# als244/ResNet

Hardware: AMD Instinct MI355X
Metric: images/sec ResNet-50 fp32 224x224 batch256 (higher is better)
Workload: dtype f32

## Files before the change

include/resnet_mi.h:

```cpp
#ifndef RESNET_MI_H
#define RESNET_MI_H
#include <stddef.h>
#include <stdint.h>

#ifdef __cplusplus
extern "C" {
#endif

typedef struct {
    char **labels;
    char **synsets;
    int *counts;
    int n_classes;
} Class_Metadata;

typedef struct {
    int input;
    int init_kernel_dim;
    int init_conv_filters;
    int init_conv_stride;
    int init_maxpool_dim;
    int init_maxpool_stride;
    int n_conv_blocks;
    int *is_block_spatial_reduction;
// ... 88 lines not shown
    float *pred_cpu;
} Forward_Buffer;

typedef struct {
    float *output_layer_deriv;
    Params *param_derivs;
    Params *prev_means;
    Params *prev_vars;
    Activations *activation_derivs;
} Backprop_Buffer;

typedef struct {
    int image_dim;
    int image_size;
    int n_images;
    int cur_shard_id;
    int cur_batch_in_shard;
    int shard_n_images;
    float *full_shard_images;
    int *full_shard_correct_classes;
    float *images_float_cpu;
    float *images;
    int *correct_classes_cpu;
    int *correct_classes;
} Batch;

typedef struct {
    ResNet *model;
    Batch *cur_batch;
    Forward_Buffer *forward_buffer;
    Backprop_Buffer *backprop_buffer;
    float learning_rate;
    float weight_decay;
    float base_mean_decay;
    float base_var_decay;
    float cur_mean_decay;
    float cur_var_decay;
    float eps;
    int batch_size;
    int n_epochs;
    int cur_dump_id;
    int cur_epoch;
    float *loss_per_epoch;
    float *accuracy_per_epoch;
    int init_loaded;
    void *backend_ctx;
    const char *dump_dir;
} Train_ResNet;

typedef struct MiRng MiRng;

Dims *init_dimensions(int input, int init_kernel_dim, int init_conv_filters, int init_conv_stride,
                      int init_maxpool_dim, int init_maxpool_stride, int n_conv_blocks,
                      int *is_block_spatial_reduction, int final_depth, int output);
MiRng *mi_rng_create(uint64_t seed);
void mi_rng_destroy(MiRng *);
ResNet *init_resnet(Dims *dims, MiRng *gen);
Batch *init_general_batch(int n_images, int image_size, int image_dim, int shard_n_images);
Train_ResNet *init_trainer(ResNet *model, Batch *cur_batch, int batch_size, float learning_rate, float weight_decay,
                           float mean_decay, float var_decay, float eps, int n_epochs, const char *dump_dir);
Train_ResNet *init_trainer_cudnn_abi(ResNet *model, Batch *cur_batch, int batch_size, float learning_rate,
                                     float weight_decay, float mean_decay, float var_decay, float eps, int n_epochs,
                                     void *handle, const char *dump_dir);
Class_Metadata *populate_class_info(char *label_filename, char *synset_filename, char *class_size_filename,
                                    int n_classes);
void load_new_batch(Train_ResNet *trainer, Class_Metadata *class_metadata, Batch *batch_buffer);
void forward_pass(Train_ResNet *trainer);
void backwards_pass(Train_ResNet *trainer);
void update_parameters(Train_ResNet *trainer);
void dump_trainer(int dump_id, Train_ResNet *trainer, const char *special_dir);
void overwrite_trainer_hyperparams(Train_ResNet *trainer, int dump_id, const char *special_dir);
void overwrite_model_params(Train_ResNet *trainer, int dump_id, const char *special_dir);

int mi_device_count(void);
int mi_set_device(int device);
const char *mi_last_error(void);
void mi_device_synchronize(void);
void destroy_trainer(Train_ResNet *trainer);

enum { MI_SRC_SHARDS = 0, MI_SRC_BUFFER = 1, MI_SRC_SYNTHETIC = 2, MI_SRC_HOST = 3 };
enum { MI_LAYOUT_NHWC = 0, MI_LAYOUT_NCHW = 1 };
void mi_batch_source_shards(Batch *b, const char *shard_dir, int layout);
void mi_batch_set_prefetch(Batch *b, int on);
void mi_batch_source_buffer(Batch *b, const char *images_path, const char *labels_path, int layout);
void mi_batch_source_synthetic(Batch *b, uint64_t seed_images, uint64_t seed_labels, int n_classes, int pool_batches);
void mi_batch_source_host(Batch *b, int layout);
int mi_batch_last_status(const Batch *b);

void mi_trainer_set_full_store(Train_ResNet *t, int on);
void mi_trainer_set_dump_root(Train_ResNet *t, const char *root);
void mi_trainer_set_dump_every(Train_ResNet *t, int every);
void mi_trainer_set_input_reset(Train_ResNet *t, int on);
void mi_trainer_set_overlap(Train_ResNet *t, int mode);
float mi_host_loss(Train_ResNet *t, int *n_wrong);

void mi_copy_to_device(void *dst_dev, const void *src_host, size_t bytes);
void mi_copy_to_host(void *dst_host, const void *src_dev, size_t bytes);

int mi_dp_unique_id_bytes(void);
int mi_dp_get_unique_id(void *out, int bytes);
int mi_dp_init(Train_ResNet *t, int rank, int world, const void *unique_id, int bytes);
void mi_dp_set_bucket_bytes(Train_ResNet *t, size_t bytes);
int mi_dp_world(const Train_ResNet *t);
int mi_dp_enable_sync_bn(Train_ResNet *t, const void *unique_id, int bytes);

void mi_trainer_last_timings(Train_ResNet *t, float out_ms[5]);

void mi_prof_enable(int on);
void mi_prof_reset(void);
void mi_prof_get(int family, long *launches, double *ms, double *flops, double *bytes);

typedef void *mi_stream_t;
void *mi_malloc(size_t bytes);
void mi_free(void *p);
int mi_op_conv_fwd(const float *x, const float *w_kcrs, float *y, int N, int C, int H, int K, int k, int stride);
int mi_op_conv_dgrad(const float *w_kcrs, const float *dy, float *dx, int N, int C, int H, int K, int k, int stride,
                     int to_add);
int mi_op_conv_wgrad(const float *x, const float *dy, float *dw_kcrs, int N, int C, int H, int K, int k, int stride);
int mi_op_bn_fwd(const float *x, const float *gamma, const float *beta, float *means, float *vars, float *y, int N,
                 int C, int H, float eps, int relu);
int mi_op_bn_fwd_add_relu(const float *x, const float *gamma, const float *beta, const float *residual, float *means,
                          float *vars, float *y, int N, int C, int H, float eps);
int mi_op_bn_bwd(const float *x, const float *gamma, const float *beta, const float *means, const float *vars,
                 const float *dy, const float *mask_src, float *dx, float *dgamma, float *dbeta, int N, int C, int H,
                 float eps, int mask_mode);
int mi_op_bn_bwd_gate(const float *x, const float *gamma, const float *beta, const float *means, const float *vars,
                      const float *dy, const float *mask_src, float *gated_out, float *dx, float *dgamma, float *dbeta, int N,
                      int C, int H, float eps);
int mi_op_maxpool_fwd(const float *x, float *y, int *max_inds, int N, int C, int H, int k, int stride);
int mi_op_maxpool_bwd(const int *max_inds, const float *dy, float *dx, int N, int C, int H, int k, int stride);
int mi_op_avgpool_fwd(const float *x, float *y, int N, int C, int H);
int mi_op_avgpool_bwd(const float *dy, float *dx, int N, int C, int H);
int mi_op_relu_deriv(const float *x, const float *up, float *out, size_t n);
int mi_op_matmul(const float *A, const float *B, float *out, int m, int k, int n);
int mi_op_matmul_lt(const float *A_kxm, const float *B, float *out, int m, int k, int n);
int mi_op_matmul_rt(const float *A, const float *B_nxk, float *out, int m, int k, int n);
int mi_op_softmax(const float *x, float *out, int N, int L);
int mi_op_ce_deriv(const float *pred, const int *labels, float *d, int N, int L);
int mi_op_adam(float *p, const float *g, float *m, float *v, size_t n, float lr, float wd, float b1, float b2,
               float cur_b1, float cur_b2, float eps, int *nan_flag_dev);
int mi_op_nhwc_to_nchw(const float *in, float *out, int N, int H, int W, int C);
int mi_debug_poison_lds(void);
int mi_debug_conv_plan(int op, int N, int C, int H, int K, int k, int stride, int out[9]);
int mi_op_fill_uniform(float *out, size_t n, uint64_t seed, float lo, float hi);


enum { MI_DTYPE_F32 = 0, MI_DTYPE_BF16 = 1 };
int mi_trainer_set_dtype(Train_ResNet *t, int dtype);
int mi_trainer_get_dtype(const Train_ResNet *t);
enum { MI_STORE_FAST = 0, MI_STORE_RECOMPUTE_BN = 1, MI_STORE_FULL = 2 };
int mi_trainer_set_store_policy(Train_ResNet *t, int policy);
size_t mi_trainer_activation_bytes(const Train_ResNet *t);
size_t mi_trainer_device_bytes(const Train_ResNet *t);
void mi_clear_error(void);
int mi_trainer_check_errors(Train_ResNet *t);
int mi_trainer_stem_dtype(Train_ResNet *t);
int mi_trainer_nan_location(const Train_ResNet *t);
void mi_trainer_set_nan_exit(Train_ResNet *t, int on);
int mi_debug_bn_merge(int R, int C, float *means, float *vars, float *dgamma, float *dbeta, float *sums_out);
void mi_trainer_end_epoch(Train_ResNet *t, float epoch_loss, float epoch_n_wrong, float total_images_per_epoch);
int mi_debug_dp_plan(const Dims *d, size_t bucket_bytes, size_t *from, size_t *to, int max);
size_t mi_debug_arena_floats(const Dims *d);
int mi_debug_last_buckets(const Train_ResNet *t, size_t *from, size_t *to, int max);

int mi_build_shard(const char *partition_csv, const char *class_dir, const char *out_dir, int shard_id, int image_dim_in,
                   int image_dim_out, int layout);
void mi_batch_set_rank_slice(Batch *b, int rank, int world);

int mi_op_convert(const void *in, int in_dt, void *out, int out_dt, size_t n);
int mi_bf16_conv_supported(int op, int N, int C, int H, int K, int k, int stride);
int mi_bf16_pw_wgrad_supported(int N, int C, int H, int K);
int mi_op_conv_fwd_bf16(const void *x_bf16, const float *w_kcrs, void *y_bf16, int N, int C, int H, int K, int k, int stride);
int mi_op_conv_dgrad_bf16(const float *w_kcrs, const void *dy_bf16, void *dx_bf16, int N, int C, int H, int K, int k, int stride,
                          int to_add);
int mi_op_conv_wgrad_bf16(const void *x_bf16, const void *dy_bf16, float *dw_kcrs, int N, int C, int H, int K, int k, int stride);
int mi_op_conv_dgrad_bn_bwd_bf16(const float *w_kcrs, const void *dy, const void *addend, void *gated, int N, int C, int H, int K, int k,
                                 int stride, const void *bn_x, const void *mask, const float *gamma, const float *beta, const float *means,
                                 const float *vars, float eps, void *bn_dx, float *dgamma, float *dbeta);
int mi_op_conv_fwd_bf16_cl(const void *x_bf16, const float *w_kcrs, void *y_bf16, int N, int C, int H, int K, int stride);
int mi_op_conv_wgrad_bf16_cl(const void *x_bf16, const void *dy_bf16, float *dw_kcrs, int N, int C, int H, int K, int stride);
int mi_op_bn_fwd_cl_bf16(const void *x_bf16, const float *gamma, const float *beta, const void *residual_bf16, float *means, float *vars, void *y_bf16, void *y_cl, int N, int C, int H, float eps, int par);
int mi_op_conv1x1_fwd_bf16_cl(const void *x_bf16, const float *w_kc, void *y_bf16, int N, int C, int H, int K);
int mi_op_conv_wgrad_bf16_cl2(const void *x, const void *dy, float *dw, int N, int C, int H, int K, int stride);
int mi_op_conv_dgrad_bf16_cl(const float *w_kcrs, const void *dy_bf16, void *dx_bf16, int N, int C, int H, int K, int stride, int to_add);
int mi_op_conv_dgrad_bn_bwd_f32(const float *w_kcrs, const float *dy, const float *addend, float *gated, int N, int C, int H, int K, int k,
                                int stride, const float *bn_x, const float *mask, const float *gamma, const float *beta, const float *means,
                                const float *vars, float eps, float *bn_dx, float *dgamma, float *dbeta);
int mi_op_stem_fwd_bf16(const float *x, const float *w_kcrs, float *y, int N, int H);
int mi_op_stem_wgrad_bf16(const float *x, const float *w_kcrs, const float *dy, float *dw_kcrs, int N, int H);
int mi_op_stem_fwd_f32(const float *x, const float *w_kcrs, float *y, int N, int H);
int mi_op_stem_wgrad_f32(const float *x, const float *w_kcrs, const float *dy, float *dw_kcrs, int N, int H);
int mi_op_conv_bn_fwd_t(const void *x, const float *w_kcrs, void *conv_out, int dt, const float *gamma, const float *beta,
                        float *means, float *vars, void *y, int N, int C, int H, int K, int k, int stride, float eps, int relu);
int mi_op_bn_fwd_t(const void *x, int x_dt, const float *gamma, const float *beta, const void *residual, float *means, float *vars,
                   void *y, int a_dt, int N, int C, int H, float eps, int relu);
int mi_op_bn_apply_t(const void *x, int x_dt, const float *gamma, const float *beta, const void *residual, const float *means,
                     const float *vars, void *y, int a_dt, int N, int C, int H, float eps, int relu);
int mi_op_bn_bwd_t(const void *x, int x_dt, const float *gamma, const float *beta, const float *means, const float *vars,
                   const void *dy, const void *mask_src, void *gated_out, int a_dt, void *dx, float *dgamma, float *dbeta, int N, int C,
                   int H, float eps, int mask_mode);
int mi_op_maxpool_fwd_t(const void *x, void *y, int dt, int *max_inds, int N, int C, int H, int k, int stride);
int mi_op_maxpool_bwd_t(const int *max_inds, const void *dy, void *dx, int dt, int N, int C, int H, int k, int stride);
int mi_op_avgpool_fwd_t(const void *x, int dt, float *y, int N, int C, int H);
int mi_op_avgpool_bwd_t(const float *dy, void *dx, int dt, int N, int C, int H);

#ifdef __cplusplus
}
#endif
#endif
```

resnet_amd/binding.py:

```python
import ctypes as C
import os

_HERE = os.path.dirname(os.path.abspath(__file__))
LIB_PATH = os.environ.get("RESNET_MI_LIB") or os.path.join(_HERE, "libresnet_mi.so")

_fp = C.POINTER(C.c_float)
_ip = C.POINTER(C.c_int)


class Dims(C.Structure):
    _fields_ = [("input", C.c_int), ("init_kernel_dim", C.c_int), ("init_conv_filters", C.c_int),
                ("init_conv_stride", C.c_int), ("init_maxpool_dim", C.c_int), ("init_maxpool_stride", C.c_int),
                ("n_conv_blocks", C.c_int), ("is_block_spatial_reduction", _ip), ("final_depth", C.c_int),
                ("output", C.c_int)]


class BatchNorm(C.Structure):
    _fields_ = [("spatial_dim", C.c_int), ("depth", C.c_int), ("gamma", _fp), ("beta", _fp)]


class ConvBlock(C.Structure):
    _fields_ = [("incoming_filters", C.c_int), ("incoming_spatial_dim", C.c_int), ("reduced_depth", C.c_int),
                ("expanded_depth", C.c_int), ("stride", C.c_int), ("depth_reduction", _fp),
                ("norm_depth_reduction", C.POINTER(BatchNorm)), ("spatial", _fp), ("norm_spatial", C.POINTER(BatchNorm)),
                ("depth_expansion", _fp), ("norm_expansion", C.POINTER(BatchNorm)), ("projection", _fp),
                ("norm_projection", C.POINTER(BatchNorm))]


class Params(C.Structure):
    _fields_ = [("init_conv_layer", _fp), ("norm_init_conv", C.POINTER(BatchNorm)),
                ("conv_blocks", C.POINTER(C.POINTER(ConvBlock))), ("fully_connected", _fp),
                ("locations", C.POINTER(_fp)), ("sizes", _ip), ("n_locations", C.c_int)]


class Cache_BatchNorm(C.Structure):
    _fields_ = [("input_size", C.c_int), ("feature_size", C.c_int), ("means", _fp), ("vars", _fp),
                ("normalized_temp", _fp), ("normalized", _fp)]


_cbp = C.POINTER(Cache_BatchNorm)


class Activation_ConvBlock(C.Structure):
    _fields_ = [("incoming_filters", C.c_int), ("incoming_spatial_dim", C.c_int), ("reduced_depth", C.c_int),
                ("expanded_depth", C.c_int), ("stride", C.c_int),
                ("post_reduced", _fp), ("norm_post_reduced", _cbp), ("post_reduced_activated", _fp),
                ("post_spatial", _fp), ("norm_post_spatial", _cbp), ("post_spatial_activated", _fp),
                ("post_expanded", _fp), ("norm_post_expanded", _cbp), ("post_expanded_norm_vals", _fp),
                ("transformed_residual", _fp), ("norm_post_projection", _cbp), ("post_projection_norm_vals", _fp),
                ("output", _fp), ("output_activated", _fp)]


class Activations(C.Structure):
    _fields_ = [("init_conv_applied", _fp), ("norm_init_conv", _cbp), ("init_conv_activated", _fp),
                ("max_inds", _ip), ("init_convblock_input", _fp),
                ("activation_conv_blocks", C.POINTER(C.POINTER(Activation_ConvBlock))), ("n_conv_blocks", C.c_int),
                ("final_conv_output_pooled", _fp), ("linear_output", _fp)]


class ResNet(C.Structure):
    _fields_ = [("dims", C.POINTER(Dims)), ("params", C.POINTER(Params))]


class Forward_Buffer(C.Structure):
    _fields_ = [("activations", C.POINTER(Activations)), ("pred", _fp), ("pred_cpu", _fp)]


class Backprop_Buffer(C.Structure):
    _fields_ = [("output_layer_deriv", _fp), ("param_derivs", C.POINTER(Params)), ("prev_means", C.POINTER(Params)),
                ("prev_vars", C.POINTER(Params)), ("activation_derivs", C.POINTER(Activations))]


class Batch(C.Structure):
    _fields_ = [("image_dim", C.c_int), ("image_size", C.c_int), ("n_images", C.c_int), ("cur_shard_id", C.c_int),
                ("cur_batch_in_shard", C.c_int), ("shard_n_images", C.c_int), ("full_shard_images", _fp),
                ("full_shard_correct_classes", _ip), ("images_float_cpu", _fp), ("images", _fp),
                ("correct_classes_cpu", _ip), ("correct_classes", _ip)]


class Train_ResNet(C.Structure):
    _fields_ = [("model", C.POINTER(ResNet)), ("cur_batch", C.POINTER(Batch)),
                ("forward_buffer", C.POINTER(Forward_Buffer)), ("backprop_buffer", C.POINTER(Backprop_Buffer)),
                ("learning_rate", C.c_float), ("weight_decay", C.c_float), ("base_mean_decay", C.c_float),
                ("base_var_decay", C.c_float), ("cur_mean_decay", C.c_float), ("cur_var_decay", C.c_float),
                ("eps", C.c_float), ("batch_size", C.c_int), ("n_epochs", C.c_int), ("cur_dump_id", C.c_int),
                ("cur_epoch", C.c_int), ("loss_per_epoch", _fp), ("accuracy_per_epoch", _fp),
                ("init_loaded", C.c_int), ("backend_ctx", C.c_void_p), ("dump_dir", C.c_char_p)]


MI_SRC_SHARDS, MI_SRC_BUFFER, MI_SRC_SYNTHETIC, MI_SRC_HOST = 0, 1, 2, 3
MI_LAYOUT_NHWC, MI_LAYOUT_NCHW = 0, 1
MI_DTYPE_F32, MI_DTYPE_BF16 = 0, 1
MI_STORE_FAST, MI_STORE_RECOMPUTE_BN, MI_STORE_FULL = 0, 1, 2

_i, _f, _vp, _sz, _u64, _cp = C.c_int, C.c_float, C.c_void_p, C.c_size_t, C.c_uint64, C.c_char_p
_T = C.POINTER(Train_ResNet)
_B = C.POINTER(Batch)
PROTOTYPES = {
    "init_dimensions": (C.POINTER(Dims), [_i] * 7 + [_ip, _i, _i]),
    "mi_rng_create": (_vp, [_u64]),
    "mi_rng_destroy": (None, [_vp]),
    "init_resnet": (C.POINTER(ResNet), [C.POINTER(Dims), _vp]),
    "init_general_batch": (_B, [_i, _i, _i, _i]),
    "init_trainer": (_T, [C.POINTER(ResNet), _B, _i, _f, _f, _f, _f, _f, _i, _cp]),
    "init_trainer_cudnn_abi": (_T, [C.POINTER(ResNet), _B, _i, _f, _f, _f, _f, _f, _i, _vp, _cp]),
    "populate_class_info": (_vp, [_cp, _cp, _cp, _i]),
    "load_new_batch": (None, [_T, _vp, _B]),
    "forward_pass": (None, [_T]),
    "backwards_pass": (None, [_T]),
    "update_parameters": (None, [_T]),
    "dump_trainer": (None, [_i, _T, _cp]),
    "overwrite_trainer_hyperparams": (None, [_T, _i, _cp]),
    "overwrite_model_params": (None, [_T, _i, _cp]),
    "mi_device_count": (_i, []),
    "mi_set_device": (_i, [_i]),
    "mi_last_error": (_cp, []),
    "mi_device_synchronize": (None, []),
    "destroy_trainer": (None, [_T]),
    "mi_batch_source_shards": (None, [_B, _cp, _i]),
    "mi_batch_set_prefetch": (None, [_B, _i]),
    "mi_batch_source_buffer": (None, [_B, _cp, _cp, _i]),
    "mi_batch_source_synthetic": (None, [_B, _u64, _u64, _i, _i]),
    "mi_batch_source_host": (None, [_B, _i]),
    "mi_batch_last_status": (_i, [_B]),
    "mi_trainer_set_full_store": (None, [_T, _i]),
    "mi_trainer_set_dump_root": (None, [_T, _cp]),
    "mi_trainer_set_dump_every": (None, [_T, _i]),
    "mi_trainer_set_input_reset": (None, [_T, _i]),
    "mi_trainer_set_overlap": (None, [_T, _i]),
    "mi_host_loss": (_f, [_T, _ip]),
    "mi_copy_to_device": (None, [_vp, _vp, _sz]),
    "mi_copy_to_host": (None, [_vp, _vp, _sz]),
    "mi_dp_unique_id_bytes": (_i, []),
    "mi_dp_get_unique_id": (_i, [_vp, _i]),
    "mi_dp_init": (_i, [_T, _i, _i, _vp, _i]),
    "mi_dp_set_bucket_bytes": (None, [_T, _sz]),
    "mi_dp_world": (_i, [_T]),
    "mi_dp_enable_sync_bn": (_i, [_T, _vp, _i]),
    "mi_trainer_last_timings": (None, [_T, C.POINTER(C.c_float * 5)]),
    "mi_prof_enable": (None, [_i]),
    "mi_prof_reset": (None, []),
    "mi_prof_get": (None, [_i, C.POINTER(C.c_long), C.POINTER(C.c_double), C.POINTER(C.c_double), C.POINTER(C.c_double)]),
    "mi_malloc": (_vp, [_sz]),
    "mi_free": (None, [_vp]),
    "mi_op_conv_fwd": (_i, [_vp, _vp, _vp, _i, _i, _i, _i, _i, _i]),
    "mi_op_conv_dgrad": (_i, [_vp, _vp, _vp, _i, _i, _i, _i, _i, _i, _i]),
    "mi_op_conv_wgrad": (_i, [_vp, _vp, _vp, _i, _i, _i, _i, _i, _i]),
    "mi_op_bn_fwd": (_i, [_vp, _vp, _vp, _vp, _vp, _vp, _i, _i, _i, _f, _i]),
    "mi_op_bn_fwd_add_relu": (_i, [_vp, _vp, _vp, _vp, _vp, _vp, _vp, _i, _i, _i, _f]),
    "mi_op_bn_bwd": (_i, [_vp] * 10 + [_i, _i, _i, _f, _i]),
    "mi_op_bn_bwd_gate": (_i, [_vp] * 11 + [_i, _i, _i, _f]),
    "mi_op_maxpool_fwd": (_i, [_vp, _vp, _vp, _i, _i, _i, _i, _i]),
    "mi_op_maxpool_bwd": (_i, [_vp, _vp, _vp, _i, _i, _i, _i, _i]),
    "mi_op_avgpool_fwd": (_i, [_vp, _vp, _i, _i, _i]),
    "mi_op_avgpool_bwd": (_i, [_vp, _vp, _i, _i, _i]),
    "mi_op_relu_deriv": (_i, [_vp, _vp, _vp, _sz]),
    "mi_op_matmul": (_i, [_vp, _vp, _vp, _i, _i, _i]),
    "mi_op_matmul_lt": (_i, [_vp, _vp, _vp, _i, _i, _i]),
    "mi_op_matmul_rt": (_i, [_vp, _vp, _vp, _i, _i, _i]),
    "mi_op_softmax": (_i, [_vp, _vp, _i, _i]),
    "mi_op_ce_deriv": (_i, [_vp, _vp, _vp, _i, _i]),
    "mi_op_adam": (_i, [_vp, _vp, _vp, _vp, _sz, _f, _f, _f, _f, _f, _f, _f, _vp]),
    "mi_op_nhwc_to_nchw": (_i, [_vp, _vp, _i, _i, _i, _i]),
    "mi_op_fill_uniform": (_i, [_vp, _sz, _u64, _f, _f]),
    "mi_debug_poison_lds": (_i, []),
    "mi_debug_conv_plan": (_i, [_i] * 7 + [_vp]),
    "mi_trainer_set_dtype": (_i, [_T, _i]),
    "mi_trainer_get_dtype": (_i, [_T]),
    "mi_trainer_set_store_policy": (_i, [_T, _i]),
    "mi_trainer_activation_bytes": (_sz, [_T]),
    "mi_trainer_device_bytes": (_sz, [_T]),
    "mi_clear_error": (None, []),
    "mi_trainer_check_errors": (_i, [_T]),
    "mi_trainer_end_epoch": (None, [_T, _f, _f, _f]),
    "mi_trainer_nan_location": (_i, [_T]),
    "mi_trainer_stem_dtype": (_i, [_T]),
    "mi_trainer_set_nan_exit": (None, [_T, _i]),
    "mi_debug_bn_merge": (_i, [_i, _i, _vp, _vp, _vp, _vp, _vp]),
    "mi_debug_dp_plan": (_i, [C.POINTER(Dims), _sz, _vp, _vp, _i]),
    "mi_debug_arena_floats": (_sz, [C.POINTER(Dims)]),
    "mi_debug_last_buckets": (_i, [_T, _vp, _vp, _i]),
    "mi_build_shard": (_i, [_cp, _cp, _cp, _i, _i, _i, _i]),
    "mi_batch_set_rank_slice": (None, [_B, _i, _i]),
    "mi_op_convert": (_i, [_vp, _i, _vp, _i, _sz]),
    "mi_bf16_conv_supported": (_i, [_i] * 7),
    "mi_bf16_pw_wgrad_supported": (_i, [_i] * 4),
    "mi_op_conv_fwd_bf16": (_i, [_vp, _vp, _vp, _i, _i, _i, _i, _i, _i]),
    "mi_op_conv_dgrad_bf16": (_i, [_vp, _vp, _vp, _i, _i, _i, _i, _i, _i, _i]),
    "mi_op_conv_wgrad_bf16": (_i, [_vp, _vp, _vp, _i, _i, _i, _i, _i, _i]),
    "mi_op_conv_dgrad_bn_bwd_bf16": (_i, [_vp, _vp, _vp, _vp, _i, _i, _i, _i, _i, _i, _vp, _vp, _vp, _vp, _vp, _vp, _f, _vp, _vp, _vp]),
    "mi_op_conv_fwd_bf16_cl": (_i, [_vp, _vp, _vp, _i, _i, _i, _i, _i]),
    "mi_op_conv_wgrad_bf16_cl": (_i, [_vp, _vp, _vp, _i, _i, _i, _i, _i]),
    "mi_op_conv_wgrad_bf16_cl2": (_i, [_vp, _vp, _vp, _i, _i, _i, _i, _i]),
    "mi_op_conv1x1_fwd_bf16_cl": (_i, [_vp, _vp, _vp, _i, _i, _i, _i]),
    "mi_op_bn_fwd_cl_bf16": (_i, [_vp, _vp, _vp, _vp, _vp, _vp, _vp, _vp, _i, _i, _i, C.c_float, _i]),
    "mi_op_conv_dgrad_bf16_cl": (_i, [_vp, _vp, _vp, _i, _i, _i, _i, _i, _i]),
    "mi_op_conv_dgrad_bn_bwd_f32": (_i, [_vp, _vp, _vp, _vp, _i, _i, _i, _i, _i, _i, _vp, _vp, _vp, _vp, _vp, _vp, _f, _vp, _vp, _vp]),
    "mi_op_stem_fwd_f32": (_i, [_vp, _vp, _vp, _i, _i]),
    "mi_op_stem_wgrad_f32": (_i, [_vp, _vp, _vp, _vp, _i, _i]),
    "mi_op_stem_fwd_bf16": (_i, [_vp, _vp, _vp, _i, _i]),
    "mi_op_stem_wgrad_bf16": (_i, [_vp, _vp, _vp, _vp, _i, _i]),
    "mi_op_conv_bn_fwd_t": (_i, [_vp, _vp, _vp, _i, _vp, _vp, _vp, _vp, _vp, _i, _i, _i, _i, _i, _i, _f, _i]),
    "mi_op_bn_fwd_t": (_i, [_vp, _i, _vp, _vp, _vp, _vp, _vp, _vp, _i, _i, _i, _i, _f, _i]),
    "mi_op_bn_apply_t": (_i, [_vp, _i, _vp, _vp, _vp, _vp, _vp, _vp, _i, _i, _i, _i, _f, _i]),
    "mi_op_bn_bwd_t": (_i, [_vp, _i, _vp, _vp, _vp, _vp, _vp, _vp, _vp, _i, _vp, _vp, _vp, _i, _i, _i, _f, _i]),
    "mi_op_maxpool_fwd_t": (_i, [_vp, _vp, _i, _vp, _i, _i, _i, _i, _i]),
    "mi_op_maxpool_bwd_t": (_i, [_vp, _vp, _vp, _i, _i, _i, _i, _i, _i]),
    "mi_op_avgpool_fwd_t": (_i, [_vp, _i, _vp, _i, _i, _i]),
    "mi_op_avgpool_bwd_t": (_i, [_vp, _vp, _i, _i, _i, _i]),
}

_lib = None


def load():
    global _lib
    if _lib is not None:
        return _lib
    if not os.path.exists(LIB_PATH):
        raise RuntimeError("libresnet_mi.so is not built (run __graft_entry__.build() or make -C resnet_amd/csrc); "
                           "there is no CPU fallback")
    lib = C.CDLL(LIB_PATH, mode=C.RTLD_GLOBAL)
    for name, (res, args) in PROTOTYPES.items():
        fn = getattr(lib, name)
        fn.restype = res
        fn.argtypes = args
    _lib = lib
    return lib
```

resnet_amd/csrc/dump.c:

```c
#define _GNU_SOURCE
#include <errno.h>
#include <stdio.h>
#include <stdlib.h>
#include <string.h>
#include <sys/stat.h>
#include "mi_host.h"

static const char *root_of(Train_ResNet *t) {
    MiCtx *c = (MiCtx *)t->backend_ctx;
    return c->dump_root ? c->dump_root : "/mnt/storage/data/vision/imagenet/training_dumps";
}
static int mkdir_p(const char *path) {
    char *tmp = strdup(path);
    for (char *p = tmp + 1; *p; p++)
        if (*p == '/') { *p = 0; if (mkdir(tmp, 0777) && errno != EEXIST) { free(tmp); return -1; } *p = '/'; }
    int rc = mkdir(tmp, 0777);
    free(tmp);
    return (rc && errno != EEXIST) ? -1 : 0;
}
static int write_dev(const char *dir, const char *name, const void *dev, size_t elems) {
    if (!dev) return 0;
    char *path = NULL;
    if (mkdir_p(dir) || asprintf(&path, "%s/%s", dir, name) < 0) return -1;
    void *host = malloc(elems * 4);
    mi_copy_to_host(host, dev, elems * 4);
    FILE *f = fopen(path, "wb");
    int rc = -1;
    if (f) { rc = fwrite(host, 4, elems, f) == elems ? 0 : -1; fclose(f); }
    free(host); free(path);
    return rc;
}
static float *g_widen = NULL;
static int write_img_t(const char *dir, const char *name, const float *dev, int N, int C, int H, float *scratch, int dt) {
    if (!dev) return 0;
    if (dt == MID_BF16) {
        mid_bf16_to_f32(mi_global()->compute, dev, g_widen, (size_t)N * C * H * H);
        dev = g_widen;
    }
    mid_nchw_to_nhwc(mi_global()->compute, dev, scratch, N, C, H, H);
    return write_dev(dir, name, scratch, (size_t)N * C * H * H);
}
static int write_img(const char *dir, const char *name, const float *dev, int N, int C, int H, float *scratch) {
    return write_img_t(dir, name, dev, N, C, H, scratch, MID_F32);
}

static int dump_parameters(int dump_id, Train_ResNet *t, const char *special_dir) {
    const Params *sets[4] = {t->model->params, t->backprop_buffer->param_derivs, t->backprop_buffer->prev_means, t->backprop_buffer->prev_vars};
    const char *names[4] = {"model_params", "gradients", "means", "vars"};
    int rc = 0;
    for (int s = 0; s < 4; s++) {
        char *dir = NULL;
        if (asprintf(&dir, "%s/%s/%08d/%s", root_of(t), special_dir, dump_id, names[s]) < 0) return -1;
        for (int i = sets[s]->n_locations - 1; i >= 0 && !rc; i--) {
            char nm[32];
            snprintf(nm, sizeof nm, "%03d.buffer", i);
            rc = write_dev(dir, nm, sets[s]->locations[i], sets[s]->sizes[i]);
        }
        free(dir);
    }
    return rc;
}
static void dump_cache(const char *dir, const Cache_BatchNorm *k) {
    if (!k) return;
    write_dev(dir, "means.buffer", k->means, k->feature_size);
    write_dev(dir, "vars.buffer", k->vars, k->feature_size);
}
static void dump_activations(int dump_id, Train_ResNet *t, Activations *a, int is_deriv, const char *special_dir) {
    const Dims *d = t->model->dims;
    const int N = t->batch_size, f = d->init_conv_filters, Hs = d->input / d->init_conv_stride, Hp = Hs / d->init_maxpool_stride;
    char *base = NULL, *dir = NULL;
    if (asprintf(&base, "%s/%s/%08d/%s", root_of(t), special_dir, dump_id, is_deriv ? "activation_derivs" : "activations") < 0) return;
    size_t maxe = (size_t)N * f * Hs * Hs;
    if ((size_t)N * t->cur_batch->image_size > maxe) maxe = (size_t)N * t->cur_batch->image_size;
    const MiCtx *ctx = (const MiCtx *)t->backend_ctx;
    const int adt = ctx->dtype;
    const int imgs = !is_deriv || ctx->policy == MI_STORE_FULL;
    const int rc = !is_deriv && ctx->policy == MI_STORE_RECOMPUTE_BN;
    float *scratch = (float *)mid_malloc(maxe * sizeof(float));
    g_widen = adt == MID_BF16 ? (float *)mid_malloc(maxe * sizeof(float)) : NULL;
    if (!is_deriv) {
        write_img(base, "input.buffer", t->cur_batch->images, N, 3, d->input, scratch);
        write_dev(base, "max_inds.buffer", a->max_inds, (size_t)N * f * Hp * Hp);
        write_dev(base, "correct_classes.buffer", t->cur_batch->correct_classes, N);
        write_dev(base, "softmax.buffer", t->forward_buffer->pred, (size_t)N * d->output);
    } else {
        write_dev(base, "fc_output.buffer", t->backprop_buffer->output_layer_deriv, (size_t)N * d->output);
    }
    if (imgs) {
        write_img_t(base, "init_conv_applied.buffer", a->init_conv_applied, N, f, Hs, scratch, adt == MID_BF16 && ctx->stem_bf16 ? MID_BF16 : MID_F32);
        if (!rc) write_img_t(base, "init_conv_activated.buffer", a->init_conv_activated, N, f, Hs, scratch, adt);
        write_img_t(base, "init_convblock_input.buffer", a->init_convblock_input, N, f, Hp, scratch, adt);
    }
    if (asprintf(&dir, "%s/batch_norms/init", base) >= 0) { dump_cache(dir, a->norm_init_conv); free(dir); }
    for (int i = 0; i < a->n_conv_blocks; i++) {
        const Activation_ConvBlock *k = a->activation_conv_blocks[i];
        const int H = k->incoming_spatial_dim, Ho = H / k->stride, R = k->reduced_depth, X = k->expanded_depth;
        if (asprintf(&dir, "%s/conv_blocks/%02d", base, i) < 0) break;
        if (imgs) {
            write_img_t(dir, "reduction_applied.buffer", k->post_reduced, N, R, H, scratch, adt);
            if (!rc) write_img_t(dir, "reduction_activated.buffer", k->post_reduced_activated, N, R, H, scratch, adt);
            write_img_t(dir, "spatial_applied.buffer", k->post_spatial, N, R, Ho, scratch, adt);
            if (!rc) write_img_t(dir, "spatial_activated.buffer", k->post_spatial_activated, N, R, Ho, scratch, adt);
            write_img_t(dir, "expanded_applied.buffer", k->post_expanded, N, X, Ho, scratch, adt);
            write_img(dir, "expanded_post_norm.buffer", k->post_expanded_norm_vals, N, X, Ho, scratch);
            write_img_t(dir, "transformed_residual.buffer", k->transformed_residual, N, X, Ho, scratch, adt);
            if (k->output != k->output_activated) write_img_t(dir, "combined_output.buffer", k->output, N, X, Ho, scratch, is_deriv ? adt : MID_F32);
            write_img_t(dir, "output_activated.buffer", k->output_activated, N, X, Ho, scratch, adt);
        }
        free(dir);
        const char *bn[4] = {"reduced", "spatial", "expanded", "projected"};
        const Cache_BatchNorm *kc[4] = {k->norm_post_reduced, k->norm_post_spatial, k->norm_post_expanded, k->norm_post_projection};
        for (int j = 0; j < 4; j++)
            if (kc[j] && asprintf(&dir, "%s/batch_norms/%02d/%s", base, i, bn[j]) >= 0) { dump_cache(dir, kc[j]); free(dir); }
    }
    write_dev(base, "final_avg_pool.buffer", a->final_conv_output_pooled, (size_t)N * d->final_depth);
    if (!is_deriv) write_dev(base, "fc_output.buffer", a->linear_output, (size_t)N * d->output);
    mid_free(scratch);
    mid_free(g_widen); g_widen = NULL;
    free(base);
}
static void dump_meta_and_checkpoint(int dump_id, Train_ResNet *t, const char *special_dir) {
    char *dir = NULL, *path = NULL;
    if (asprintf(&dir, "%s/%s/%08d", root_of(t), special_dir, dump_id) < 0 || mkdir_p(dir)) { free(dir); return; }
    if (asprintf(&path, "%s/trainer_metadata.txt", dir) >= 0) {
        FILE *fp = fopen(path, "w");
        if (fp) {
            fprintf(fp, "%d\n%d\n%d\n%d\n", t->batch_size, t->cur_batch->image_size, t->cur_batch->image_dim, t->cur_batch->shard_n_images);
            fprintf(fp, "%f\n%f\n%f\n%f\n%f\n%f\n%f\n", t->learning_rate, t->weight_decay, t->base_mean_decay, t->base_var_decay,
                    t->cur_mean_decay, t->cur_var_decay, t->eps);
            fprintf(fp, "%d\n%d\n%d\n", t->n_epochs, t->cur_dump_id, t->cur_epoch);
            for (int i = 0; i < t->cur_epoch; i++) fprintf(fp, i ? ",%f" : "%f", t->loss_per_epoch[i]);
            fprintf(fp, "\n");
            for (int i = 0; i < t->cur_epoch; i++) fprintf(fp, i ? ",%f" : "%f", t->accuracy_per_epoch[i]);
            fprintf(fp, "\n");
            fclose(fp);
        }
        free(path);
    }
    if (asprintf(&path, "%s/trainer_checkpoint.txt", dir) >= 0) {
        FILE *fp = fopen(path, "w");
        if (fp) {
            fprintf(fp, "%d\n%d\n%f\n%f\n%d\n%d\n", t->cur_batch->cur_shard_id, t->cur_batch->cur_batch_in_shard,
                    t->cur_mean_decay, t->cur_var_decay, t->cur_dump_id, t->cur_epoch);
            fclose(fp);
        }
        free(path);
    }
    free(dir);
}

void dump_trainer(int dump_id, Train_ResNet *t, const char *special_dir) {
    if (!special_dir) special_dir = "default";
    if (dump_parameters(dump_id, t, special_dir)) {
        fprintf(stderr, "resnet_mi: cannot write dump %d under %s/%s (skipped)\n", dump_id, root_of(t), special_dir);
        return;
    }
    dump_activations(dump_id, t, t->forward_buffer->activations, 0, special_dir);
    dump_activations(dump_id, t, t->backprop_buffer->activation_derivs, 1, special_dir);
    dump_meta_and_checkpoint(dump_id, t, special_dir);
}

void overwrite_trainer_hyperparams(Train_ResNet *t, int dump_id, const char *special_dir) {
    char *path = NULL;
    if (asprintf(&path, "%s/%s/%08d/trainer_checkpoint.txt", root_of(t), special_dir, dump_id) < 0) return;
    FILE *fp = fopen(path, "r");
    free(path);
    if (!fp) { fprintf(stderr, "resnet_mi: no checkpoint %d\n", dump_id); return; }
    int a, b, e, f;
    float c, d;
    if (fscanf(fp, "%d %d %f %f %d %d", &a, &b, &c, &d, &e, &f) == 6) {
        t->cur_batch->cur_shard_id = a; t->cur_batch->cur_batch_in_shard = b;
        t->cur_mean_decay = c; t->cur_var_decay = d; t->cur_dump_id = e; t->cur_epoch = f;
        t->init_loaded = 1;
    }
    fclose(fp);
}
void overwrite_model_params(Train_ResNet *t, int dump_id, const char *special_dir) {
    const Params *sets[3] = {t->model->params, t->backprop_buffer->prev_means, t->backprop_buffer->prev_vars};
    const char *names[3] = {"model_params", "means", "vars"};
    for (int i = sets[0]->n_locations - 1; i >= 0; i--) {
        const size_t sz = sets[0]->sizes[i];
        float *host = (float *)malloc(sz * sizeof(float));
        for (int s = 0; s < 3; s++) {
            char *path = NULL;
            if (asprintf(&path, "%s/%s/%08d/%s/%03d.buffer", root_of(t), special_dir, dump_id, names[s], i) < 0) continue;
            FILE *fp = fopen(path, "rb");
            if (fp) {
                if (fread(host, sizeof(float), sz, fp) == sz) mi_copy_to_device(sets[s]->locations[i], host, sz * sizeof(float));
                fclose(fp);
            } else fprintf(stderr, "resnet_mi: missing %s\n", path);
            free(path);
        }
        free(host);
    }
}
```

resnet_amd/csrc/kernels_bn.hip:

```cpp
#include "mi_common.hpp"
#include "mi_device.h"

#define BN_SPLIT_MAX 64

struct Wel { float n, mean, m2; };
__device__ __forceinline__ Wel wel_merge(Wel a, Wel b) {
    Wel r;
    r.n = a.n + b.n;
    if (r.n == 0.f) { r.mean = 0.f; r.m2 = 0.f; return r; }
    const float d = b.mean - a.mean, f = b.n / r.n;
    r.mean = a.mean + d * f;
    r.m2 = a.m2 + b.m2 + d * d * a.n * f;
    return r;
}
__device__ __forceinline__ Wel wel_wave(Wel w) {
#pragma unroll
    for (int o = 32; o > 0; o >>= 1) {
        Wel b;
        b.n = __shfl_xor(w.n, o, 64); b.mean = __shfl_xor(w.mean, o, 64); b.m2 = __shfl_xor(w.m2, o, 64);
        w = wel_merge(w, b);
    }
    return w;
}
__device__ __forceinline__ void wel_add4(Wel &w, float a, float b, float c, float d) {
    const float bm = ((a + b) + (c + d)) * 0.25f;
    const float da = a - bm, db = b - bm, dc = c - bm, dd = d - bm;
    Wel t; t.n = 4.f; t.mean = bm; t.m2 = (da * da + db * db) + (dc * dc + dd * dd);
    w = wel_merge(w, t);
}
__device__ __forceinline__ void wel_add1(Wel &w, float a) {
    Wel t; t.n = 1.f; t.mean = a; t.m2 = 0.f;
    w = wel_merge(w, t);
}

__device__ __forceinline__ void wel_add_batch(Wel &w, float nb, float bmean, float bm2) {
    Wel t; t.n = nb; t.mean = bmean; t.m2 = bm2;
    w = wel_merge(w, t);
}

template <typename TX, int V>
__global__ void __launch_bounds__(256)
bn_stats_kernel(const TX *__restrict__ x, float *__restrict__ partial, int N, int C, int P, FastDiv fdPV) {
    const int c = blockIdx.x, split = blockIdx.y, nsplit = gridDim.y;
    const int cnt = (N - split + nsplit - 1) / nsplit;
    const uint32_t PV = (uint32_t)P / V;
    const uint32_t total = (uint32_t)cnt * PV;
    const size_t img_stride = (size_t)nsplit * C * P;
    const TX *base = x + ((size_t)split * C + c) * P;
    Wel w = {0.f, 0.f, 0.f};
    auto addr = [&](uint32_t idx) -> const TX * {
        const uint32_t j = fd_div(idx, fdPV), i = idx - j * PV;
        return base + (size_t)j * img_stride + (size_t)i * V;
    };
    uint32_t idx = threadIdx.x;
    for (; idx + 3 * 256 < total; idx += 4 * 256) {
        float v[4][V];
#pragma unroll
        for (int u = 0; u < 4; u++) VecIO<TX, V>::load(addr(idx + u * 256), v[u]);
        if (V == 1) {
            const float bm = ((v[0][0] + v[1][0]) + (v[2][0] + v[3][0])) * 0.25f;
            const float a = v[0][0] - bm, b = v[1][0] - bm, cc = v[2][0] - bm, d = v[3][0] - bm;
            wel_add_batch(w, 4.f, bm, (a * a + b * b) + (cc * cc + d * d));
        } else {
            float s = 0.f;
#pragma unroll
            for (int u = 0; u < 4; u++)
#pragma unroll
                for (int q = 0; q < V; q += 4) s += (v[u][q] + v[u][q + 1]) + (v[u][q + 2] + v[u][q + 3]);
            const float bm = s * (1.0f / (4.0f * V));
            float m2 = 0.f;
#pragma unroll
            for (int u = 0; u < 4; u++)
#pragma unroll
                for (int q = 0; q < V; q += 4) {
                    const float a = v[u][q] - bm, b = v[u][q + 1] - bm, cc = v[u][q + 2] - bm, d = v[u][q + 3] - bm;
                    m2 += (a * a + b * b) + (cc * cc + d * d);
                }
            wel_add_batch(w, 4.f * V, bm, m2);
        }
    }
    for (; idx < total; idx += 256) {
        float v[V];
        VecIO<TX, V>::load(addr(idx), v);
        if (V == 1) wel_add1(w, v[0]);
        else {
#pragma unroll
            for (int q = 0; q < V; q += 4) wel_add4(w, v[q], v[q + 1], v[q + 2], v[q + 3]);
        }
    }
    w = wel_wave(w);
    __shared__ Wel sh[4];
    const int lane = threadIdx.x & 63, wv = threadIdx.x >> 6;
    if (lane == 0) sh[wv] = w;
    __syncthreads();
    if (threadIdx.x == 0) {
        Wel r = sh[0];
        for (int i = 1; i < (int)(blockDim.x >> 6); i++) r = wel_merge(r, sh[i]);
        float *o = partial + ((size_t)c * BN_SPLIT_MAX + split) * 3;
        o[0] = r.n; o[1] = r.mean; o[2] = r.m2;
    }
}

__global__ void __launch_bounds__(256)
bn_parts_merge_kernel(const float *__restrict__ parts, int np, int C, float *__restrict__ partial) {
    const int cx = threadIdx.x & 63, sg = threadIdx.x >> 6;
    const int c = blockIdx.x * 64 + cx;
    const int chunk = (np + gridDim.y - 1) / gridDim.y;
    const int p0 = blockIdx.y * chunk, p1 = min(np, p0 + chunk);
    const size_t plane = (size_t)np * C;
    Wel w = {0.f, 0.f, 0.f};
    if (c < C) {
        int p = p0 + sg;
        for (; p + 7 * 4 < p1; p += 8 * 4) {
            Wel b[8];
#pragma unroll
            for (int u = 0; u < 8; u++) {
                const size_t o = (size_t)(p + 4 * u) * C + c;
                b[u].n = parts[o]; b[u].mean = parts[plane + o]; b[u].m2 = parts[2 * plane + o];
            }
#pragma unroll
            for (int u = 0; u < 8; u++) w = wel_merge(w, b[u]);
        }
        for (; p < p1; p += 4) {
            const size_t o = (size_t)p * C + c;
            Wel b = {parts[o], parts[plane + o], parts[2 * plane + o]};
            w = wel_merge(w, b);
        }
    }
    __shared__ Wel sh[4][64];
    sh[sg][cx] = w;
    __syncthreads();
    if (sg == 0 && c < C) {
        Wel r = sh[0][cx];
        for (int i = 1; i < 4; i++) r = wel_merge(r, sh[i][cx]);
        float *o = partial + ((size_t)c * BN_SPLIT_MAX + blockIdx.y) * 3;
        o[0] = r.n; o[1] = r.mean; o[2] = r.m2;
    }
}

__global__ void __launch_bounds__(256)
bn_finalize_kernel(const float *__restrict__ partial, int nsplit, int C, float *__restrict__ means, float *__restrict__ vars) {
    const int c = blockIdx.x * 4 + (threadIdx.x >> 6), lane = threadIdx.x & 63;
    if (c >= C) return;
    const float *p = partial + (size_t)c * BN_SPLIT_MAX * 3;
    Wel w = {0.f, 0.f, 0.f};
    if (lane < nsplit) { w.n = p[lane * 3]; w.mean = p[lane * 3 + 1]; w.m2 = p[lane * 3 + 2]; }
    w = wel_wave(w);
    if (lane == 0) { means[c] = w.mean; vars[c] = w.m2 / w.n; }
}

__device__ __forceinline__ float bn_xhat(float x, float mean, float sd) { return (x - mean) / sd; }
__device__ __forceinline__ float bn_y(float xh, float g, float b) { return fmaf(g, xh, b); }

template <typename TX, typename TA, int V, bool STR>
__global__ void __launch_bounds__(256)
bn_apply_kernel(const TX *__restrict__ x, const float *__restrict__ gamma, const float *__restrict__ beta,
                const float *__restrict__ means, const float *__restrict__ vars, const TA *__restrict__ residual,
                TA *__restrict__ y, float *__restrict__ xhat_out, float *__restrict__ norm_out, int C, int P,
                FastDiv fdP, FastDiv fdC, size_t total, float eps, int relu) {
    const size_t nvec = total / V;
    for (size_t i = (size_t)blockIdx.x * blockDim.x + threadIdx.x; i < nvec; i += (size_t)gridDim.x * blockDim.x) {
        const size_t e = i * V;
        const uint32_t plane = fd_div((uint32_t)e, fdP);
        const uint32_t c = plane - fd_div(plane, fdC) * C;
        const float mean0 = means[c], sd0 = sqrtf(vars[c] + eps), g0 = gamma[c], b0 = beta[c];
        int nfirst = V;
        float mean1 = mean0, sd1 = sd0, g1 = g0, b1 = b0;
        if (STR) {
            nfirst = min(V, P - (int)((uint32_t)e - plane * (uint32_t)P));
            const uint32_t c1 = c + 1 == (uint32_t)C ? 0u : c + 1;
            mean1 = means[c1]; sd1 = sqrtf(vars[c1] + eps); g1 = gamma[c1]; b1 = beta[c1];
        }
        float v[V], r[V], xh[V], nv[V];
        VecIO<TX, V>::load(x + e, v);
        if (residual) VecIO<TA, V>::load(residual + e, r);
#pragma unroll
        for (int q = 0; q < V; q++) {
            const bool nx = STR && q >= nfirst;
            const float mean = nx ? mean1 : mean0, sd = nx ? sd1 : sd0, g = nx ? g1 : g0, b = nx ? b1 : b0;
            xh[q] = bn_xhat(v[q], mean, sd);
            nv[q] = bn_y(xh[q], g, b);
            float o = nv[q];
            if (residual) o = fmaxf(o + r[q], 0.f);
            else if (relu) o = fmaxf(o, 0.f);
            v[q] = o;
        }
        VecIO<TA, V>::store(y + e, v);
        if (xhat_out) VecIO<float, V>::store(xhat_out + e, xh);
        if (norm_out) VecIO<float, V>::store(norm_out + e, nv);
    }
}

typedef uint32_t bn_u32x4 __attribute__((ext_vector_type(4)));
typedef bn_u32x4 __attribute__((aligned(2))) bn_u32x4_u2;
__global__ void __launch_bounds__(256)
bn_apply_cl_kernel(const bf16_t *__restrict__ x, const float *__restrict__ gamma, const float *__restrict__ beta, const float *__restrict__ means,
                   const float *__restrict__ vars, const bf16_t *__restrict__ residual, bf16_t *__restrict__ y, bf16_t *__restrict__ ycl, int C, int P, int W,
                   float eps, FastDiv fdW, int par) {
    __shared__ __attribute__((aligned(16))) bf16_t tile[64 * 72];
    const int c0 = blockIdx.x * 64, p0 = blockIdx.y * 64, n = blockIdx.z;
#pragma unroll
    for (int u = 0; u < 2; u++) {
        const int idx = threadIdx.x + 256 * u, cc = idx >> 3, part = idx & 7;
        const int c = c0 + cc, pp = p0 + part * 8;
        const float mean = means[c], sd = sqrtf(vars[c] + eps), g = gamma[c], b = beta[c];
        const size_t e = ((size_t)n * C + c) * P + pp;
        const int nv = min(8, P - pp);
        float v[8], r[8];
        if (nv >= 8) {
            const bn_u32x4 t = *(const bn_u32x4_u2 *)(x + e);
#pragma unroll
            for (int q = 0; q < 4; q++) { v[2 * q] = __uint_as_float(t[q] << 16); v[2 * q + 1] = __uint_as_float(t[q] & 0xffff0000u); }
            if (residual) {
                const bn_u32x4 t2 = *(const bn_u32x4_u2 *)(residual + e);
#pragma unroll
                for (int q = 0; q < 4; q++) { r[2 * q] = __uint_as_float(t2[q] << 16); r[2 * q + 1] = __uint_as_float(t2[q] & 0xffff0000u); }
            }
        } else {
#pragma unroll
            for (int q = 0; q < 8; q++) { v[q] = q < nv ? mi_bf2f(x[e + q]) : 0.f; r[q] = (residual && q < nv) ? mi_bf2f(residual[e + q]) : 0.f; }
        }
#pragma unroll
        for (int q = 0; q < 8; q++) {
            const float nvq = bn_y(bn_xhat(v[q], mean, sd), g, b);
            v[q] = residual ? fmaxf(nvq + r[q], 0.f) : fmaxf(nvq, 0.f);
        }
        const bn_u32x4 o = {mi_pack_bf2(v[0], v[1]), mi_pack_bf2(v[2], v[3]), mi_pack_bf2(v[4], v[5]), mi_pack_bf2(v[6], v[7])};
        if (nv >= 8) *(bn_u32x4_u2 *)(y + e) = o;
        else {
#pragma unroll
            for (int q = 0; q < 8; q++) if (q < nv) y[e + q] = (bf16_t)((q & 1) ? o[q >> 1] >> 16 : o[q >> 1] & 0xffffu);
        }
#pragma unroll
        for (int q = 0; q < 4; q++) {
            tile[(part * 8 + 2 * q) * 72 + cc] = (bf16_t)(o[q] & 0xffffu);
            tile[(part * 8 + 2 * q + 1) * 72 + cc] = (bf16_t)(o[q] >> 16);
        }
    }
    __syncthreads();
    const int H = W;
#pragma unroll
    for (int u = 0; u < 2; u++) {
        const int idx = threadIdx.x + 256 * u, px = idx >> 3, piece = idx & 7;
        const int p = p0 + px;
        if (p < P) {
            const uint32_t yy = fd_div((uint32_t)p, fdW), xx = (uint32_t)p - yy * W;
            const int Hp = H / 2 + 1;
            const size_t o = par ? ((((size_t)n * 4 + 2 * (yy & 1) + (xx & 1)) * Hp + (yy >> 1) + 1) * Hp + (xx >> 1) + 1) * C
                                 : (((size_t)n * (H + 2) + yy + 1) * (W + 2) + xx + 1) * C;
            *(bn_u32x4 *)(ycl + o + c0 + piece * 8) = *(const bn_u32x4 *)(tile + px * 72 + piece * 8);
        }
    }
}

template <int MASK, typename TX, typename TA, int V>
__global__ void __launch_bounds__(256)
bn_bwd_reduce_kernel(const TX *__restrict__ x, const TA *__restrict__ dy, const TA *__restrict__ mask_src,
                     const float *__restrict__ gamma, const float *__restrict__ beta, const float *__restrict__ means,
                     const float *__restrict__ vars, float *__restrict__ partial, TA *__restrict__ gated, int N, int C, int P,
                     float eps, FastDiv fdPV) {
    const int c = blockIdx.x, split = blockIdx.y, nsplit = gridDim.y;
    const float mean = means[c], sd = sqrtf(vars[c] + eps), g = gamma[c], b = beta[c];
    const int cnt = (N - split + nsplit - 1) / nsplit;
    constexpr bool EXT = MASK == 2 || MASK == 3;
    const uint32_t PV = (uint32_t)P / V;
    const uint32_t total = (uint32_t)cnt * PV;
    const size_t img_stride = (size_t)nsplit * C * P;
    const size_t base = ((size_t)split * C + c) * P;
    float s1 = 0.f, s2 = 0.f;
    auto one = [&](float xv, float d, float m) -> float {
        const float xh = bn_xhat(xv, mean, sd);
        bool on = true;
        if (MASK == 1) on = bn_y(xh, g, b) > 0.f;
        if (EXT) on = m > 0.f;
        if (on) { s1 += d; s2 = fmaf(d, xh, s2); }
        return on ? d : 0.f;
    };
    auto off = [&](uint32_t idx) -> size_t {
        const uint32_t j = fd_div(idx, fdPV), i = idx - j * PV;
        return base + (size_t)j * img_stride + (size_t)i * V;
    };
    constexpr int U = (EXT ? 2 : 4) * (V == 8 ? 1 : 1);
    uint32_t idx = threadIdx.x;
    for (; idx + (U - 1) * 256 < total; idx += U * 256) {
        float xv[U][V], dv[U][V], mv[U][V];
        size_t o[U];
#pragma unroll
        for (int u = 0; u < U; u++) {
            o[u] = off(idx + u * 256);
            VecIO<TX, V>::load(x + o[u], xv[u]);
            VecIO<TA, V>::load(dy + o[u], dv[u]);
            if (EXT) VecIO<TA, V>::load(mask_src + o[u], mv[u]);
            else {
#pragma unroll
                for (int q = 0; q < V; q++) mv[u][q] = 1.f;
            }
        }
#pragma unroll
        for (int u = 0; u < U; u++) {
            float gq[V];
#pragma unroll
            for (int q = 0; q < V; q++) gq[q] = one(xv[u][q], dv[u][q], mv[u][q]);
            if (MASK == 3) VecIO<TA, V>::store(gated + o[u], gq);
        }
    }
    for (; idx < total; idx += 256) {
        const size_t o = off(idx);
        float xv[V], dv[V], mv[V], gq[V];
        VecIO<TX, V>::load(x + o, xv);
        VecIO<TA, V>::load(dy + o, dv);
        if (EXT) VecIO<TA, V>::load(mask_src + o, mv);
        else {
#pragma unroll
            for (int q = 0; q < V; q++) mv[q] = 1.f;
        }
#pragma unroll
        for (int q = 0; q < V; q++) gq[q] = one(xv[q], dv[q], mv[q]);
        if (MASK == 3) VecIO<TA, V>::store(gated + o, gq);
    }
    s1 = wave_sum(s1); s2 = wave_sum(s2);
    __shared__ float sh[8];
    const int lane = threadIdx.x & 63, wv = threadIdx.x >> 6;
    if (lane == 0) { sh[wv * 2] = s1; sh[wv * 2 + 1] = s2; }
    __syncthreads();
    if (threadIdx.x == 0) {
        float a = 0.f, bsum = 0.f;
        for (int i = 0; i < (int)(blockDim.x >> 6); i++) { a += sh[i * 2]; bsum += sh[i * 2 + 1]; }
        float *o = partial + ((size_t)c * BN_SPLIT_MAX + split) * 3;
// ... 48 lines not shown
    if (lane == 0) { dbeta[c] = s1; dgamma[c] = s2; }
}

template <int MASK, typename TX, typename TA, int V, bool STR>
__global__ void __launch_bounds__(256)
bn_bwd_apply_kernel(const TX *__restrict__ x, const TA *__restrict__ dy, const TA *__restrict__ mask_src,
                    const float *__restrict__ gamma, const float *__restrict__ beta, const float *__restrict__ means,
                    const float *__restrict__ vars, const float *__restrict__ dgamma, const float *__restrict__ dbeta,
                    TX *__restrict__ dx, int C, int P, FastDiv fdP, FastDiv fdC, size_t total, float inv_m, float eps) {
    const size_t nvec = total / V;
    for (size_t i = (size_t)blockIdx.x * blockDim.x + threadIdx.x; i < nvec; i += (size_t)gridDim.x * blockDim.x) {
        const size_t e = i * V;
        const uint32_t plane = fd_div((uint32_t)e, fdP);
        const uint32_t c = plane - fd_div(plane, fdC) * C;
        const float mean0 = means[c], sd0 = sqrtf(vars[c] + eps), g0 = gamma[c], b0 = beta[c];
        const float k10 = dbeta[c] * inv_m, k20 = dgamma[c] * inv_m, scale0 = g0 / sd0;
        int nfirst = V;
        float mean1 = mean0, sd1 = sd0, g1 = g0, b1 = b0, k11 = k10, k21 = k20, scale1 = scale0;
        if (STR) {
            nfirst = min(V, P - (int)((uint32_t)e - plane * (uint32_t)P));
            const uint32_t c1 = c + 1 == (uint32_t)C ? 0u : c + 1;
            mean1 = means[c1]; sd1 = sqrtf(vars[c1] + eps); g1 = gamma[c1]; b1 = beta[c1];
            k11 = dbeta[c1] * inv_m; k21 = dgamma[c1] * inv_m; scale1 = g1 / sd1;
        }
        float xv[V], dv[V], mv[V];
        VecIO<TX, V>::load(x + e, xv);
        VecIO<TA, V>::load(dy + e, dv);
        if (MASK == 2) VecIO<TA, V>::load(mask_src + e, mv);
#pragma unroll
        for (int q = 0; q < V; q++) {
            const bool nx = STR && q >= nfirst;
            const float mean = nx ? mean1 : mean0, sd = nx ? sd1 : sd0, g = nx ? g1 : g0, b = nx ? b1 : b0;
            const float k1 = nx ? k11 : k10, k2 = nx ? k21 : k20, scale = nx ? scale1 : scale0;
            const float xh = bn_xhat(xv[q], mean, sd);
            bool on = true;
            if (MASK == 1) on = bn_y(xh, g, b) > 0.f;
            if (MASK == 2) on = mv[q] > 0.f;
            const float gq = on ? dv[q] : 0.f;
            xv[q] = scale * (gq - k1 - xh * k2);
        }
        VecIO<TX, V>::store(dx + e, xv);
    }
}

static int bn_nsplit(int N, int C) {
    int ns = mi_cdiv(2048, C);
    if (ns > N) ns = N;
    if (ns > BN_SPLIT_MAX) ns = BN_SPLIT_MAX;
    if (ns < 1) ns = 1;
    return ns;
}
static int ew_blocks(size_t nvec) {
    size_t b = (nvec + 255) / 256;
    if (b > (1u << 22)) b = 1u << 22;
    if (b < 1) b = 1;
    return (int)b;
}

__global__ void bn_sync_k2(const float *__restrict__ sum_means, float *__restrict__ means, const float *__restrict__ vars,
                           float *__restrict__ tmp, int C, float inv_world) {
    const int c = blockIdx.x * blockDim.x + threadIdx.x;
    if (c >= C) return;
    const float mg = sum_means[c] * inv_world, d = means[c] - mg;
    tmp[c] = vars[c] + d * d;
    means[c] = mg;
}
__global__ void bn_sync_k3(const float *__restrict__ tmp, float *__restrict__ vars, int C, float inv_world) {
    const int c = blockIdx.x * blockDim.x + threadIdx.x;
    if (c < C) vars[c] = tmp[c] * inv_world;
}
__global__ void bn_sync_pack(const float *__restrict__ a, const float *__restrict__ b, float *__restrict__ out, int C) {
    const int c = blockIdx.x * blockDim.x + threadIdx.x;
    if (c < C) { out[c] = a[c]; out[C + c] = b[c]; }
}
__global__ void bn_sync_unpack(const float *__restrict__ in, float *__restrict__ a, float *__restrict__ b, int C, float inv_world) {
    const int c = blockIdx.x * blockDim.x + threadIdx.x;
    if (c < C) { a[c] = in[c] * inv_world; b[c] = in[C + c] * inv_world; }
}

__global__ void bn_sync_emul_allreduce(float *__restrict__ bufs, int R, size_t stride, int n) {
    const int i = blockIdx.x * blockDim.x + threadIdx.x;
    if (i >= n) return;
    float s = 0.f;
    for (int r = 0; r < R; r++) s += bufs[(size_t)r * stride + i];
    for (int r = 0; r < R; r++) bufs[(size_t)r * stride + i] = s;
}

static int bn_vec(int x_dt, int a_dt, int P) {
    if (x_dt == MID_F32 && a_dt == MID_F32) return (P & 3) == 0 ? 4 : 1;
    return (P & 7) == 0 ? 8 : (P & 3) == 0 ? 4 : 1;
}
static bool bn_pair_ok(int x_dt, int a_dt) {
    return (x_dt == MID_F32 && a_dt == MID_F32) || (x_dt == MID_BF16 && a_dt == MID_BF16) || (x_dt == MID_F32 && a_dt == MID_BF16);
}
#define BN_DISPATCH(BODY)                                                                            \
    do {                                                                                             \
        if (x_dt == MID_F32 && a_dt == MID_F32) { if (vec == 4) { BODY(float, float, 4); } else { BODY(float, float, 1); } } \
        else if (x_dt == MID_BF16) { if (vec == 8) { BODY(bf16_t, bf16_t, 8); } else if (vec == 4) { BODY(bf16_t, bf16_t, 4); } else { BODY(bf16_t, bf16_t, 1); } } \
        else { if (vec == 8) { BODY(float, bf16_t, 8); } else if (vec == 4) { BODY(float, bf16_t, 4); } else { BODY(float, bf16_t, 1); } } \
    } while (0)

static int bn_vec_ew(int x_dt, int a_dt, int P, size_t total, bool *str) {
    int vec = bn_vec(x_dt, a_dt, P);
    *str = false;
    const int vmax = (x_dt == MID_F32 && a_dt == MID_F32) ? 4 : 8;
    static int on = -1;
    if (on < 0) { const char *e = getenv("RESNET_MI_BN_STRADDLE"); on = e ? atoi(e) : 1; }
    if (on && vec == 1 && P >= vmax && total % vmax == 0) { vec = vmax; *str = true; }
    return vec;
}
#define BN_DISPATCH_EW(BODY)                                                                         \
    do {                                                                                             \
        if (x_dt == MID_F32 && a_dt == MID_F32) { if (str) { BODY(float, float, 4, true); } else if (vec == 4) { BODY(float, float, 4, false); } else { BODY(float, float, 1, false); } } \
        else if (x_dt == MID_BF16) { if (str) { BODY(bf16_t, bf16_t, 8, true); } else if (vec == 8) { BODY(bf16_t, bf16_t, 8, false); } else if (vec == 4) { BODY(bf16_t, bf16_t, 4, false); } else { BODY(bf16_t, bf16_t, 1, false); } } \
        else { if (str) { BODY(float, bf16_t, 8, true); } else if (vec == 8) { BODY(float, bf16_t, 8, false); } else if (vec == 4) { BODY(float, bf16_t, 4, false); } else { BODY(float, bf16_t, 1, false); } } \
    } while (0)

static size_t dt_bytes(int dt) { return dt == MID_BF16 ? 2 : 4; }
static struct { void *comm; int world, force; float *tmp; size_t tmp_floats; } g_bn_sync;

extern "C" {
void mid_bn_set_sync(void *comm, int world, float *tmp, size_t tmp_floats, int force) {
    g_bn_sync.comm = comm; g_bn_sync.world = world; g_bn_sync.tmp = tmp; g_bn_sync.tmp_floats = tmp_floats; g_bn_sync.force = force ? 1 : 0;
}
size_t mid_bn_ws_floats(int C) { return (size_t)C * BN_SPLIT_MAX * 3; }

int mid_bn_debug_merge(mid_stream s, int R, int C, float *means, float *vars, float *dgamma, float *dbeta, float *sums_out, float *tmp) {
    hipStream_t st = (hipStream_t)s;
    if (R < 1 || C < 1) return -2;
    const float iw = 1.0f / (float)R;
    const size_t T = (size_t)2 * C;
    const dim3 gc(mi_cdiv(C, 256)), g2c(mi_cdiv(2 * C, 256)), b(256);
    if (means && vars) {
        for (int r = 0; r < R; r++) (void)hipMemcpyAsync(tmp + r * T, means + (size_t)r * C, sizeof(float) * C, hipMemcpyDeviceToDevice, st);
        hipLaunchKernelGGL(bn_sync_emul_allreduce, gc, b, 0, st, tmp, R, T, C);
        for (int r = 0; r < R; r++) hipLaunchKernelGGL(bn_sync_k2, gc, b, 0, st, tmp + r * T, means + (size_t)r * C, vars + (size_t)r * C, tmp + r * T + C, C, iw);
        hipLaunchKernelGGL(bn_sync_emul_allreduce, gc, b, 0, st, tmp + C, R, T, C);
        for (int r = 0; r < R; r++) hipLaunchKernelGGL(bn_sync_k3, gc, b, 0, st, tmp + r * T + C, vars + (size_t)r * C, C, iw);
    }
    if (dgamma && dbeta) {
        for (int r = 0; r < R; r++) hipLaunchKernelGGL(bn_sync_pack, gc, b, 0, st, dgamma + (size_t)r * C, dbeta + (size_t)r * C, tmp + r * T, C);
        hipLaunchKernelGGL(bn_sync_emul_allreduce, g2c, b, 0, st, tmp, R, T, 2 * C);
        if (sums_out) (void)hipMemcpyAsync(sums_out, tmp, sizeof(float) * R * T, hipMemcpyDeviceToDevice, st);
        for (int r = 0; r < R; r++) hipLaunchKernelGGL(bn_sync_unpack, gc, b, 0, st, tmp + r * T, dgamma + (size_t)r * C, dbeta + (size_t)r * C, C, iw);
    }
    MI_LAUNCH_CHECK("mid_bn_debug_merge");
    return 0;
}

size_t mid_bn_parts_floats(int N, int K, int Ho) { return (size_t)3 * (size_t)mi_cdiv((long)N * ((Ho * Ho + 7) / 8 * 8), 128) * 4 * K; }

static int bn_fwd_apply(hipStream_t st, const void *x, int x_dt, const float *gamma, const float *beta, const void *residual,
                        const float *means, const float *vars, void *y, int a_dt, float *xhat_out, float *norm_out, int N, int C,
                        int P, float eps, int relu, void *ycl, int Hcl) {
    const int Hab = Hcl < 0 ? -Hcl : Hcl;
    if (ycl && x_dt == MID_BF16 && a_dt == MID_BF16 && (residual || relu) && !xhat_out && !norm_out && C % 64 == 0 && Hab * Hab == P && !(Hcl < 0 && (Hab & 1))) {
        hipLaunchKernelGGL(bn_apply_cl_kernel, dim3(C / 64, mi_cdiv(P, 64), N), dim3(256), 0, st, (const bf16_t *)x, gamma, beta, means, vars,
                           (const bf16_t *)residual, (bf16_t *)y, (bf16_t *)ycl, C, P, Hab, eps, make_fastdiv(Hab), Hcl < 0);
        MI_LAUNCH_CHECK("bn_apply_cl_kernel");
        return 0;
    }
    if (ycl) { mi_record_error("bn_fwd_apply", "channel-last side output requested for a form that has none"); return -2; }
    const size_t total = (size_t)N * C * P;
    const FastDiv fdP = make_fastdiv(P), fdC = make_fastdiv(C);
    bool str;
    const int vec = bn_vec_ew(x_dt, a_dt, P, total, &str);
#define APPLY(TX, TA, V, STR)                                                                                              \
    hipLaunchKernelGGL((bn_apply_kernel<TX, TA, V, STR>), dim3(ew_blocks(total / V)), dim3(256), 0, st, (const TX *)x, gamma, beta, \
                       means, vars, (const TA *)residual, (TA *)y, xhat_out, norm_out, C, P, fdP, fdC, total, eps, relu)
    BN_DISPATCH_EW(APPLY);
#undef APPLY
    MI_LAUNCH_CHECK("bn_apply_kernel");
    return 0;
}

static int bn_stats_launch(hipStream_t st, float *ws, const void *x, int x_dt, int N, int C, int P, int ns) {
    if (x_dt == MID_F32) {
        if ((P & 3) == 0) hipLaunchKernelGGL((bn_stats_kernel<float, 4>), dim3(C, ns), dim3(256), 0, st, (const float *)x, ws, N, C, P, make_fastdiv(P / 4));
        else hipLaunchKernelGGL((bn_stats_kernel<float, 1>), dim3(C, ns), dim3(256), 0, st, (const float *)x, ws, N, C, P, make_fastdiv(P));
    } else {
        if ((P & 7) == 0) hipLaunchKernelGGL((bn_stats_kernel<bf16_t, 8>), dim3(C, ns), dim3(256), 0, st, (const bf16_t *)x, ws, N, C, P, make_fastdiv(P / 8));
        else if ((P & 3) == 0) hipLaunchKernelGGL((bn_stats_kernel<bf16_t, 4>), dim3(C, ns), dim3(256), 0, st, (const bf16_t *)x, ws, N, C, P, make_fastdiv(P / 4));
        else hipLaunchKernelGGL((bn_stats_kernel<bf16_t, 1>), dim3(C, ns), dim3(256), 0, st, (const bf16_t *)x, ws, N, C, P, make_fastdiv(P));
    }
    MI_LAUNCH_CHECK("bn_stats_kernel");
    return 0;
}

int mid_bn_stats_t(mid_stream s, float *ws, const void *x, int x_dt, float *means, float *vars, int N, int C, int P) {
    hipStream_t st = (hipStream_t)s;
    const int ns = bn_nsplit(N, C);
    if (bn_stats_launch(st, ws, x, x_dt, N, C, P, ns)) return -1;
    hipLaunchKernelGGL(bn_finalize_kernel, dim3(mi_cdiv(C, 4)), dim3(256), 0, st, ws, ns, C, means, vars);
    MI_LAUNCH_CHECK("bn_finalize_kernel");
    return 0;
}

int mid_bn_apply_t(mid_stream s, const void *x, int x_dt, const float *gamma, const float *beta, const void *residual,
                   const float *means, const float *vars, void *y, int a_dt, int N, int C, int P, float eps, int relu, void *ycl, int Hcl) {
    if (!bn_pair_ok(x_dt, a_dt)) { mi_record_error("mid_bn_apply_t", "unsupported storage types"); return -2; }
    hipStream_t st = (hipStream_t)s;
    mi_prof_begin(st, MI_FAM_BN, 0.0, (double)N * C * P * (dt_bytes(x_dt) + dt_bytes(a_dt) * (residual ? 2 : 1)));
    const int rc = bn_fwd_apply(st, x, x_dt, gamma, beta, residual, means, vars, y, a_dt, nullptr, nullptr, N, C, P, eps, relu, ycl, Hcl);
    mi_prof_end(st);
    return rc;
}

int mid_bn_fwd_t(mid_stream s, float *ws, const mid_bn_parts *parts, const void *x, int x_dt, const float *gamma, const float *beta,
                 const void *residual, float *means, float *vars, void *y, int a_dt, float *xhat_out, float *norm_out, int N, int C,
                 int P, float eps, int relu, void *ycl, int Hcl) {
    if (!bn_pair_ok(x_dt, a_dt)) { mi_record_error("mid_bn_fwd_t", "unsupported storage types"); return -2; }
    if ((xhat_out || norm_out) && !(x_dt == MID_F32 && a_dt == MID_F32)) { mi_record_error("mid_bn_fwd_t", "full-store tensors exist in fp32 only"); return -2; }
    hipStream_t st = (hipStream_t)s;
    const double xb = (double)N * C * P * dt_bytes(x_dt), ab = (double)N * C * P * dt_bytes(a_dt);
    if (!parts || parts->nparts <= 0) {
        const int ns = bn_nsplit(N, C);
        mi_prof_begin(st, MI_FAM_BN, 0.0, 2 * xb + ab * (residual ? 2 : 1));
        if (bn_stats_launch(st, ws, x, x_dt, N, C, P, ns)) return -1;
        hipLaunchKernelGGL(bn_finalize_kernel, dim3(mi_cdiv(C, 4)), dim3(256), 0, st, ws, ns, C, means, vars);
        MI_LAUNCH_CHECK("bn_finalize_kernel");
    } else {
        int G = parts->nparts / 64;
        if (G < 1) G = 1;
        if (G > BN_SPLIT_MAX) G = BN_SPLIT_MAX;
        mi_prof_begin(st, MI_FAM_BN, 0.0, xb + ab * (residual ? 2 : 1));
        hipLaunchKernelGGL(bn_parts_merge_kernel, dim3(mi_cdiv(C, 64), G), dim3(256), 0, st, parts->buf, parts->nparts, C, ws);
        MI_LAUNCH_CHECK("bn_parts_merge_kernel");
        hipLaunchKernelGGL(bn_finalize_kernel, dim3(mi_cdiv(C, 4)), dim3(256), 0, st, ws, G, C, means, vars);
        MI_LAUNCH_CHECK("bn_finalize_kernel");
    }
    if (g_bn_sync.comm && g_bn_sync.world > 1 - g_bn_sync.force) {
        const float iw = 1.0f / (float)g_bn_sync.world;
        float *tmp = g_bn_sync.tmp;
        if (C > g_bn_sync.tmp_floats / 2) { mi_record_error("sync BN", "scratch too small"); return -3; }
        (void)hipMemcpyAsync(tmp, means, sizeof(float) * C, hipMemcpyDeviceToDevice, st);
        if (mid_rccl_allreduce_sum(g_bn_sync.comm, tmp, (size_t)C, (mid_stream)st)) return -1;
        hipLaunchKernelGGL(bn_sync_k2, dim3(mi_cdiv(C, 256)), dim3(256), 0, st, tmp, means, vars, tmp + C, C, iw);
        if (mid_rccl_allreduce_sum(g_bn_sync.comm, tmp + C, (size_t)C, (mid_stream)st)) return -1;
        hipLaunchKernelGGL(bn_sync_k3, dim3(mi_cdiv(C, 256)), dim3(256), 0, st, tmp + C, vars, C, iw);
        MI_LAUNCH_CHECK("bn_sync");
    }
    const int rc = bn_fwd_apply(st, x, x_dt, gamma, beta, residual, means, vars, y, a_dt, xhat_out, norm_out, N, C, P, eps, relu, ycl, Hcl);
    mi_prof_end(st);
    return rc;
}

int mid_bn_fwd(mid_stream s, float *ws, const float *x, const float *gamma, const float *beta, const float *residual,
               float *means, float *vars, float *y, float *xhat_out, float *norm_out, int N, int C, int P, float eps,
               int relu) {
    return mid_bn_fwd_t(s, ws, nullptr, x, MID_F32, gamma, beta, residual, means, vars, y, MID_F32, xhat_out, norm_out, N, C, P, eps, relu, nullptr, 0);
}

int mid_bn_fwd_parts(mid_stream s, float *ws, const mid_bn_parts *parts, const float *x, const float *gamma, const float *beta,
                     const float *residual, float *means, float *vars, float *y, float *xhat_out, float *norm_out, int N,
                     int C, int P, float eps, int relu) {
    return mid_bn_fwd_t(s, ws, parts, x, MID_F32, gamma, beta, residual, means, vars, y, MID_F32, xhat_out, norm_out, N, C, P, eps, relu, nullptr, 0);
}

static int bn_bwd_impl(hipStream_t st, float *ws, const void *x, int x_dt, const float *gamma, const float *beta, const float *means,
                       const float *vars, const void *dy, const void *mask_src, void *gated_out, int a_dt, void *dx, float *dgamma,
                       float *dbeta, int N, int C, int P, float eps, int mask_mode, const mid_bn_bwd_parts *bparts = nullptr) {
    if (!bn_pair_ok(x_dt, a_dt)) { mi_record_error("mid_bn_bwd", "unsupported storage types"); return -2; }
    int ns = bn_nsplit(N, C);
    dim3 grid(C, ns), block(256);
    if (mask_mode >= 2 && !mask_src) { mi_record_error("mid_bn_bwd", "mask_src missing"); return -2; }
    if (mask_mode == 3 && !gated_out) { mi_record_error("mid_bn_bwd_gate", "gated_out missing"); return -2; }
    const double xb = (double)N * C * P * dt_bytes(x_dt), ab = (double)N * C * P * dt_bytes(a_dt);
    mi_prof_begin(st, MI_FAM_BN, 0.0, bparts ? 2 * xb + ab : 3 * xb + ab * (mask_mode >= 2 ? 4 : 2));
    const int vec = bn_vec(x_dt, a_dt, P);
    const FastDiv fdPV = make_fastdiv(P / vec);
    if (bparts) {
        ns = bparts->nparts >= 64 * 8 ? 64 : bparts->nparts >= 64 ? 8 : 1;
        hipLaunchKernelGGL(bn_bwd_parts_merge_kernel, dim3(mi_cdiv(C, 64), ns), dim3(256), 0, st, bparts->buf, bparts->nparts, C, vars, eps, ws);
        MI_LAUNCH_CHECK("bn_bwd_parts_merge_kernel");
    } else {
#define BWD_REDUCE_M(M_, TX, TA, V)                                                                                         \
    hipLaunchKernelGGL((bn_bwd_reduce_kernel<M_, TX, TA, V>), grid, block, 0, st, (const TX *)x, (const TA *)dy, (const TA *)mask_src, \
                       gamma, beta, means, vars, ws, (TA *)gated_out, N, C, P, eps, fdPV)
#define BWD_R0(TX, TA, V) BWD_REDUCE_M(0, TX, TA, V)
#define BWD_R1(TX, TA, V) BWD_REDUCE_M(1, TX, TA, V)
#define BWD_R2(TX, TA, V) BWD_REDUCE_M(2, TX, TA, V)
#define BWD_R3(TX, TA, V) BWD_REDUCE_M(3, TX, TA, V)
    if (mask_mode == 0) BN_DISPATCH(BWD_R0);
    else if (mask_mode == 1) BN_DISPATCH(BWD_R1);
    else if (mask_mode == 2) BN_DISPATCH(BWD_R2);
    else BN_DISPATCH(BWD_R3);
#undef BWD_R0
#undef BWD_R1
#undef BWD_R2
#undef BWD_R3
#undef BWD_REDUCE_M
    MI_LAUNCH_CHECK("bn_bwd_reduce_kernel");
    }
    hipLaunchKernelGGL(bn_bwd_finalize_kernel, dim3(mi_cdiv(C, 4)), dim3(256), 0, st, ws, ns, C, dgamma, dbeta);
    MI_LAUNCH_CHECK("bn_bwd_finalize_kernel");
    const size_t total = (size_t)N * C * P;
    const FastDiv fdP = make_fastdiv(P), fdC = make_fastdiv(C);
    float inv_m = 1.0f / (float)((size_t)N * P);
    const float *dg_apply = dgamma, *db_apply = dbeta;
    const bool sync = g_bn_sync.comm && g_bn_sync.world > 1 - g_bn_sync.force;
    if (sync) {
        if (2 * C > g_bn_sync.tmp_floats) { mi_record_error("sync BN", "scratch too small"); return -3; }
        float *tmp = g_bn_sync.tmp;
        hipLaunchKernelGGL(bn_sync_pack, dim3(mi_cdiv(C, 256)), dim3(256), 0, st, dgamma, dbeta, tmp, C);
        if (mid_rccl_allreduce_sum(g_bn_sync.comm, tmp, (size_t)2 * C, (mid_stream)st)) return -1;
        dg_apply = tmp; db_apply = tmp + C;
        inv_m = 1.0f / ((float)g_bn_sync.world * (float)((size_t)N * P));
    }
    const void *dy_apply = mask_mode == 3 ? gated_out : dy;
    {
    bool str;
    const int vec = bn_vec_ew(x_dt, a_dt, P, total, &str);
    dim3 g2(ew_blocks(total / vec));
#define BWD_APPLY_M(M_, TX, TA, V, STR)                                                                                        \
    hipLaunchKernelGGL((bn_bwd_apply_kernel<M_, TX, TA, V, STR>), g2, block, 0, st, (const TX *)x, (const TA *)dy_apply, (const TA *)mask_src, \
                       gamma, beta, means, vars, dg_apply, db_apply, (TX *)dx, C, P, fdP, fdC, total, inv_m, eps)
#define BWD_A0(TX, TA, V, STR) BWD_APPLY_M(0, TX, TA, V, STR)
#define BWD_A1(TX, TA, V, STR) BWD_APPLY_M(1, TX, TA, V, STR)
#define BWD_A2(TX, TA, V, STR) BWD_APPLY_M(2, TX, TA, V, STR)
    if (mask_mode == 0 || mask_mode == 3) BN_DISPATCH_EW(BWD_A0);
    else if (mask_mode == 1) BN_DISPATCH_EW(BWD_A1);
    else BN_DISPATCH_EW(BWD_A2);
    }
#undef BWD_A0
#undef BWD_A1
#undef BWD_A2
#undef BWD_APPLY_M
    if (sync) hipLaunchKernelGGL(bn_sync_unpack, dim3(mi_cdiv(C, 256)), dim3(256), 0, st, g_bn_sync.tmp, dgamma, dbeta, C, 1.0f / (float)g_bn_sync.world);
    mi_prof_end(st);
    MI_LAUNCH_CHECK("bn_bwd_apply_kernel");
    return 0;
}

int mid_bn_bwd_t(mid_stream s, float *ws, const void *x, int x_dt, const float *gamma, const float *beta, const float *means,
                 const float *vars, const void *dy, const void *mask_src, void *gated_out, int a_dt, void *dx, float *dgamma,
                 float *dbeta, int N, int C, int P, float eps, int mask_mode) {
    if (mask_mode < 0 || mask_mode > 3) { mi_record_error("mid_bn_bwd", "mask_mode"); return -2; }
    return bn_bwd_impl((hipStream_t)s, ws, x, x_dt, gamma, beta, means, vars, dy, mask_src, gated_out, a_dt, dx, dgamma, dbeta, N, C, P, eps, mask_mode);
}
int mid_bn_bwd_parts_t(mid_stream s, float *ws, const mid_bn_bwd_parts *parts, const void *x, int x_dt, const float *gamma, const float *beta,
                       const float *means, const float *vars, const void *dy_gated, int a_dt, void *dx, float *dgamma, float *dbeta, int N,
                       int C, int P, float eps) {
    if (!parts || parts->nparts <= 0) { mi_record_error("mid_bn_bwd_parts_t", "no partials"); return -2; }
    return bn_bwd_impl((hipStream_t)s, ws, x, x_dt, gamma, beta, means, vars, dy_gated, nullptr, nullptr, a_dt, dx, dgamma, dbeta, N, C, P, eps, 0, parts);
}
int mid_bn_bwd(mid_stream s, float *ws, const float *x, const float *gamma, const float *beta, const float *means,
               const float *vars, const float *dy, const float *mask_src, float *dx, float *dgamma, float *dbeta, int N,
               int C, int P, float eps, int mask_mode) {
    if (mask_mode < 0 || mask_mode > 2) { mi_record_error("mid_bn_bwd", "mask_mode"); return -2; }
    return bn_bwd_impl((hipStream_t)s, ws, x, MID_F32, gamma, beta, means, vars, dy, mask_src, nullptr, MID_F32, dx, dgamma, dbeta, N, C, P, eps, mask_mode);
}
int mid_bn_bwd_gate(mid_stream s, float *ws, const float *x, const float *gamma, const float *beta, const float *means,
                    const float *vars, const float *dy, const float *mask_src, float *gated_out, float *dx, float *dgamma,
                    float *dbeta, int N, int C, int P, float eps) {
    return bn_bwd_impl((hipStream_t)s, ws, x, MID_F32, gamma, beta, means, vars, dy, mask_src, gated_out, MID_F32, dx, dgamma, dbeta, N, C, P, eps, 3);
}
}
```

resnet_amd/csrc/mi_device.h:

```cpp
#ifndef MI_DEVICE_H
#define MI_DEVICE_H
#include <stddef.h>
#include <stdint.h>
#ifdef __cplusplus
extern "C" {
#endif

typedef void *mid_stream;
typedef void *mid_event;

enum { MID_F32 = 0, MID_BF16 = 1 };

int mid_device_count(void);
int mid_set_device(int dev);
const char *mid_last_error(void);
void mid_clear_error(void);
void *mid_malloc(size_t bytes);
void mid_free(void *p);
void *mid_malloc_host(size_t bytes);
void mid_free_host(void *p);
void mid_memcpy_h2d(void *dst, const void *src, size_t bytes, mid_stream s);
void mid_memcpy_d2h(void *dst, const void *src, size_t bytes, mid_stream s);
void mid_memcpy_d2d(void *dst, const void *src, size_t bytes, mid_stream s);
void mid_memset(void *dst, int byte, size_t bytes, mid_stream s);
mid_stream mid_stream_create(void);
mid_stream mid_stream_create_low_priority(void);
void mid_stream_destroy(mid_stream s);
void mid_stream_sync(mid_stream s);
void mid_device_sync(void);
mid_event mid_event_create(void);
void mid_event_destroy(mid_event e);
void mid_event_record(mid_event e, mid_stream s);
void mid_stream_wait_event(mid_stream s, mid_event e);
float mid_event_elapsed_ms(mid_event a, mid_event b);
void mid_event_sync(mid_event e);

void mid_prof_enable(int on);
void mid_prof_reset(void);
void mid_prof_get(int family, long *launches, double *ms, double *flops, double *bytes);

typedef struct {
    float *wt;
    size_t wt_floats;
    float *part;
    size_t part_floats;
    const float *pre_fwd, *pre_dgrad;
    void *s2d;
    size_t s2d_bytes;
    int s2d_valid;
} mid_workspace;

typedef struct {
    const float *w;
    float *fwd, *dgrad;
    int K, C, T, tile0;
} mid_wt_entry;
int mid_conv_prelayout_all(mid_stream s, const mid_wt_entry *entries_dev, const int *tile_entry_dev, int ntiles);
void mid_conv_prelayout_needs(int N, int C, int H, int K, int k, int stride, int *need_fwd, int *need_dgrad);

int mid_conv_fwd(mid_stream s, mid_workspace *ws, const float *x, const float *w, float *y, int N, int C, int H, int K,
                 int k, int stride);
typedef struct {
    float *buf;
    size_t floats;
    int nparts;
} mid_bn_parts;
size_t mid_bn_parts_floats(int N, int K, int Ho);
int mid_conv_fwd_stats(mid_stream s, mid_workspace *ws, const float *x, const float *w, float *y, int N, int C, int H, int K,
                       int k, int stride, mid_bn_parts *parts);
int mid_conv_dgrad(mid_stream s, mid_workspace *ws, const float *w, const float *dy, float *dx, const float *addend,
                   int N, int C, int H, int K, int k, int stride);
int mid_conv_wgrad(mid_stream s, mid_workspace *ws, const float *x, const float *dy, float *dw, int N, int C, int H,
                   int K, int k, int stride);
size_t mid_conv_ws_wt_floats(int C, int K, int k);
size_t mid_conv_ws_part_floats(int N, int C, int H, int K, int k, int stride);

int mid_bf16_supported(int op, int N, int C, int H, int K, int k, int stride);
size_t mid_bf16_part_floats(int N, int C, int H, int K, int k, int stride);
int mid_conv_prelayout_all_bf16(mid_stream s, const mid_wt_entry *entries_dev, const int *tile_entry_dev, int ntiles);
int mid_conv_fwd_bf16(mid_stream s, mid_workspace *ws, const void *x, const float *w, void *y, int N, int C, int H, int K, int k,
                      int stride, mid_bn_parts *parts);
typedef struct {
    const void *x;
    const void *mask;
    const float *means;
    float *buf;
    size_t floats;
    int nparts;
} mid_bn_bwd_parts;
int mid_conv_dgrad_bn_bf16(mid_stream s, mid_workspace *ws, const float *w, const void *dy, void *dx, const void *addend, int N, int C,
                           int H, int K, int k, int stride, mid_bn_bwd_parts *fz);
int mid_conv_dgrad_bn_f32(mid_stream s, mid_workspace *ws, const float *w, const float *dy, float *dx, const float *addend, int N, int C,
                          int H, int K, int k, int stride, mid_bn_bwd_parts *fz);
int mid_bn_bwd_parts_t(mid_stream s, float *stats_ws, const mid_bn_bwd_parts *parts, const void *x, int x_dt, const float *gamma,
                       const float *beta, const float *means, const float *vars, const void *dy_gated, int a_dt, void *dx, float *dgamma,
                       float *dbeta, int N, int C, int P, float eps);
int mid_conv_dgrad_bf16(mid_stream s, mid_workspace *ws, const float *w, const void *dy, void *dx, const void *addend, int N, int C,
                        int H, int K, int k, int stride);
int mid_conv_wgrad_bf16(mid_stream s, mid_workspace *ws, const void *x, const void *dy, float *dw, int N, int C, int H, int K, int k,
                        int stride);
int mid_bf16_prelayout_fwd(mid_stream s, const float *w, void *out, int K, int C, int k);
int mid_bf16_prelayout_dgrad(mid_stream s, const float *w, void *out, int K, int C, int k);
int mid_cl_supported(int op, int N, int C, int H, int K, int stride);
size_t mid_cl_operand_bytes(int op, int N, int C, int H, int K, int stride);
int mid_cl_relayout(mid_stream s, const void *x, void *xp, int N, int C, int H, int parity);
int mid_cl_fwd(mid_stream s, const void *xp, const void *a_tiles, void *y, int N, int C, int H, int K, int stride, mid_bn_parts *parts);
int mid_cl_dgrad(mid_stream s, const void *dyp, const void *a_tiles, void *dx, const void *addend, int N, int C, int H, int K);
int mid_cl_wgrad_supported(int N, int C, int H, int K, int stride);
size_t mid_cl_wgrad_part_floats(int N, int C, int H, int K, int stride);
int mid_cl_pw_supported(int N, int C, int H, int K);
int mid_cl_relayout_dense(mid_stream s, const void *x, void *xp, int N, int C, int H);
int mid_cl_pw_fwd(mid_stream s, const void *xc, const void *a_tiles, void *y, int N, int C, int H, int K, mid_bn_parts *parts);
int mid_cl_wgrad2_supported(int N, int C, int H, int K, int stride);
size_t mid_cl_wgrad2_part_floats(int N, int C, int H, int K, int stride);
int mid_cl_wgrad2(mid_stream s, const void *xp, const void *dyp, float *dw, float *part, size_t part_floats, int N, int C, int H, int K, int stride);
int mid_pw_wgrad_supported(int N, int C, int H, int K);
size_t mid_pw_wgrad_part_floats(int N, int C, int H, int K);
int mid_pw_wgrad(mid_stream s, const void *x, const void *dy, float *dw, float *part, size_t part_floats, int N, int C, int H, int K);
int mid_cl_wgrad(mid_stream s, const void *xp, const void *dy, float *dw, float *part, size_t part_floats, int N, int C, int H, int K, int stride);
int mid_cl_dgrad2_supported(int N, int C, int H, int K);
size_t mid_cl_dgrad2_operand_bytes(int N, int K, int Ho);
int mid_cl_relayout_end(mid_stream s, const void *dy, void *dyp, int N, int K, int Ho);
int mid_cl_dgrad2(mid_stream s, const void *dyp, const void *a_tiles, void *dx, int N, int C, int H, int K);
int mid_igemm_mode(void);
size_t mid_stem_f32_xp_bytes(int N, int H);
int mid_stem_fwd_f32(mid_stream s, const float *x, const float *w, float *y, void *xp, size_t xp_bytes, float *scratch, size_t scratch_floats,
                     int N, int H, mid_bn_parts *parts);
int mid_stem_wgrad_f32(mid_stream s, const void *xp, const float *dy, float *dw, float *scratch, size_t scratch_floats, int N, int H);
int mid_stem_bf16_supported(int C, int H, int K, int k, int stride);
size_t mid_stem_bf16_xp_bytes(int N, int H);
size_t mid_stem_bf16_part_floats(int N, int H);
int mid_stem_fwd_bf16(mid_stream s, const float *x, const float *w, void *y, int y_dt, void *xp, size_t xp_bytes, float *scratch, size_t scratch_floats,
                      int N, int H, mid_bn_parts *parts);
int mid_stem_wgrad_bf16(mid_stream s, const void *xp, const void *dy, int dy_dt, float *dw, float *scratch, size_t scratch_floats, int N, int H);
int mid_f32_to_bf16(mid_stream s, const float *in, void *out, size_t n);
int mid_bf16_to_f32(mid_stream s, const void *in, float *out, size_t n);

int mid_igemm_plan(int op, int N, int C, int H, int K, int k, int stride, int out[9]);

int mid_gemm_nn(mid_stream s, const float *A, const float *B, float *out, int m, int k, int n);
int mid_gemm_tn(mid_stream s, const float *At, const float *B, float *out, int m, int k, int n);
int mid_gemm_nt(mid_stream s, const float *A, const float *Bt, float *out, int m, int k, int n);

size_t mid_bn_ws_floats(int C);
int mid_bn_fwd(mid_stream s, float *stats_ws, const float *x, const float *gamma, const float *beta,
               const float *residual, float *means, float *vars, float *y, float *xhat_out, float *norm_out, int N,
               int C, int P, float eps, int relu);
int mid_bn_fwd_parts(mid_stream s, float *stats_ws, const mid_bn_parts *parts, const float *x, const float *gamma,
                     const float *beta, const float *residual, float *means, float *vars, float *y, float *xhat_out,
                     float *norm_out, int N, int C, int P, float eps, int relu);
int mid_bn_bwd(mid_stream s, float *stats_ws, const float *x, const float *gamma, const float *beta,
               const float *means, const float *vars, const float *dy, const float *mask_src, float *dx,
               float *dgamma, float *dbeta, int N, int C, int P, float eps, int mask_mode);

int mid_bn_bwd_gate(mid_stream s, float *stats_ws, const float *x, const float *gamma, const float *beta,
                    const float *means, const float *vars, const float *dy, const float *mask_src, float *gated_out,
                    float *dx, float *dgamma, float *dbeta, int N, int C, int P, float eps);

int mid_bn_fwd_t(mid_stream s, float *stats_ws, const mid_bn_parts *parts, const void *x, int x_dt, const float *gamma,
                 const float *beta, const void *residual, float *means, float *vars, void *y, int a_dt, float *xhat_out,
                 float *norm_out, int N, int C, int P, float eps, int relu, void *ycl, int Hcl);
void mid_bn_set_sync(void *comm, int world, float *tmp, size_t tmp_floats, int force);
int mid_bn_debug_merge(mid_stream s, int R, int C, float *means, float *vars, float *dgamma, float *dbeta, float *sums_out, float *tmp);
int mid_bn_stats_t(mid_stream s, float *stats_ws, const void *x, int x_dt, float *means, float *vars, int N, int C, int P);
int mid_bn_apply_t(mid_stream s, const void *x, int x_dt, const float *gamma, const float *beta, const void *residual,
                   const float *means, const float *vars, void *y, int a_dt, int N, int C, int P, float eps, int relu, void *ycl, int Hcl);
int mid_bn_bwd_t(mid_stream s, float *stats_ws, const void *x, int x_dt, const float *gamma, const float *beta, const float *means,
                 const float *vars, const void *dy, const void *mask_src, void *gated_out, int a_dt, void *dx, float *dgamma,
                 float *dbeta, int N, int C, int P, float eps, int mask_mode);
int mid_maxpool_fwd_t(mid_stream s, const void *x, void *y, int dt, int *max_inds, int N, int C, int H, int k, int stride);
int mid_maxpool_bwd_t(mid_stream s, const int *max_inds, const void *dy, void *dx, int dt, int N, int C, int H, int k, int stride);
int mid_avgpool_fwd_t(mid_stream s, const void *x, int dt, float *y, int N, int C, int P);
int mid_avgpool_bwd_t(mid_stream s, const float *dy, void *dx, int dt, int N, int C, int P);

int mid_maxpool_fwd(mid_stream s, const float *x, float *y, int *max_inds, int N, int C, int H, int k, int stride);
int mid_maxpool_bwd(mid_stream s, const int *max_inds, const float *dy, float *dx, int N, int C, int H, int k,
                    int stride);
int mid_avgpool_fwd(mid_stream s, const float *x, float *y, int N, int C, int P);
int mid_avgpool_bwd(mid_stream s, const float *dy, float *dx, int N, int C, int P);
int mid_relu_deriv(mid_stream s, const float *x, const float *up, float *out, size_t n);
int mid_add_relu(mid_stream s, const float *a, const float *b, float *sum_out, float *act_out, size_t n);
int mid_softmax(mid_stream s, const float *x, float *out, int N, int L);
int mid_ce_deriv(mid_stream s, const float *pred, const int *labels, float *d, int N, int L);
int mid_adam(mid_stream s, float *p, float *g, float *m, float *v, size_t n, float lr, float wd, float b1,
             float b2, float cur_b1, float cur_b2, float eps, int *nan_flag, int zero_grads, const size_t *loc_off_dev, int n_loc,
             size_t base);
int mid_nhwc_to_nchw(mid_stream s, const float *in, float *out, int N, int H, int W, int C);
int mid_nchw_to_nhwc(mid_stream s, const float *in, float *out, int N, int C, int H, int W);
int mid_fill_uniform(mid_stream s, float *out, size_t n, uint64_t seed, uint64_t offset, float lo, float hi);
int mid_lds_poison(mid_stream s);
int mid_fill_labels(mid_stream s, int *out, size_t n, uint64_t seed, uint64_t offset, int n_classes);

int mid_rccl_unique_id_bytes(void);
int mid_rccl_get_unique_id(void *out, int bytes);
void *mid_rccl_comm_init(int rank, int world, const void *unique_id, int bytes);
int mid_rccl_allreduce_sum(void *comm, float *buf, size_t count, mid_stream s);
void mid_rccl_comm_destroy(void *comm);
void mid_rccl_comm_abort(void *comm);

#ifdef __cplusplus
}
#endif
#endif
```

resnet_amd/csrc/mi_host.h:

```cpp
#ifndef MI_HOST_H
#define MI_HOST_H
#include "mi_device.h"
#include "resnet_mi.h"

struct MiRng { uint64_t seed; uint64_t counter; };

uint64_t mi_splitmix64_at(uint64_t seed, uint64_t i);
void mi_synth_uniform(float *out, size_t n, uint64_t seed, uint64_t offset, float lo, float hi);
void mi_synth_normal(float *out, size_t n, uint64_t seed, uint64_t offset, double var);
void mi_synth_labels(int *out, size_t n, uint64_t seed, uint64_t offset, int n_classes);

typedef struct {
    int ready;
    mid_stream compute, comm, copy, aux;
} MiGlobal;
MiGlobal *mi_global(void);

typedef struct BatchExt {
    Batch *batch;
    int source, layout, status;
    int rank, world;
    char *shard_dir, *images_path, *labels_path;
    uint64_t seed_images, seed_labels;
    int n_classes, pool_batches, pool_next;
    float *pool_images;
    int *pool_labels;
    int *pool_labels_host;
    float *stage_dev;
    int prefetch, have_next, next_shard_id, next_batch_in_shard;
    float *images_next, *stage_next, *pinned_next;
    int *labels_next, *labels_next_host;
    mid_event ev_next, ev_compute;
    uint64_t synth_step;
    struct BatchExt *next;
} BatchExt;
BatchExt *mi_batch_ext(Batch *b);
void mi_batch_ext_free(Batch *b);

typedef struct {
    int cl_s1, cl_s1_dgrad;
    int cl_s2, cl_dgrad2;
    int stem_mfma, bf16_stem;
    int stem_tensors_f32;
    int bnfuse_bwd;
    int bnfuse_bwd_f32;
    int overlap, overlap_given;
    int bnfuse;
    int prelayout;
} MiOptions;

enum { MI_FWD_F32, MI_FWD_BF16, MI_FWD_CL, MI_FWD_STEM_F32, MI_FWD_STEM_BF16 };
enum { MI_DG_F32, MI_DG_BF16, MI_DG_CL, MI_DG_CL2 };
enum { MI_WG_F32, MI_WG_BF16, MI_WG_CL, MI_WG_CL2, MI_WG_STEM_F32, MI_WG_STEM_BF16 };
typedef struct {
    const float *w;
    int C, H, K, k, stride;
    const mid_wt_entry *we;
    int fwd, dgrad, wgrad;
    int fz;
    void *cl; int cl_by_bn;
    void *dye;
    void *par; size_t par_bytes; int par_valid;
    void *xp; size_t xp_bytes; float *scratch; size_t scratch_floats;
} MiLayer;
typedef struct { MiLayer red, spa, exp, proj; } MiBlockLayers;

typedef struct MiCtx {
    mid_workspace ws;
    float *bn_ws;
    mid_bn_parts bn_parts;
    mid_wt_entry *wt_tab;
    int wt_n, wt_tiles;
    mid_wt_entry *wt_tab_dev;
    int *wt_tile_entry_dev;
    MiOptions opt;
    MiLayer stem;
    MiBlockLayers *blk;
    int *nan_flag_dev, *nan_flag_host;
    int nan_check_pending;
    mid_event ev_nan;
    size_t *loc_off_dev; int n_loc;
    int nan_location, nan_no_exit;
    struct MiCtx *next_live;
    int full_store, dump_every, input_reset;
    int dtype;
    int policy;
    int n_persist;
    size_t act_bytes, dev_bytes;
    size_t *alloc_bytes;
    float *rc_buf[2];
    int stem_bf16;
    float *stem_dx;
    int counting_act;
    int overlap_set;
    int params_dirty;
    unsigned long host_epoch_seen;
    char *dump_root;
    void **allocs;
    int n_allocs, cap_allocs;
    size_t arena_floats;
    float *g_arena, *m_arena, *v_arena;
    void *comm;
    int rank, world;
    size_t bucket_bytes;
    size_t dp_cursor;
    mid_event ev_grads, ev_reduced;
    int dp_pending;
#define MI_MAX_BUCKETS 64
    size_t bk_from[MI_MAX_BUCKETS], bk_to[MI_MAX_BUCKETS];
    mid_event bk_ev[MI_MAX_BUCKETS];
    int n_buckets;
    int sync_bn;
    void *sync_bn_comm;
    float *sync_bn_tmp;
    int overlap_wgrad, wgrad_pending;
    mid_event ev_bn_done, ev_wgrad_done;
#define MI_RING 10
    float *ring_buf[MI_RING];
    mid_event ring_ev[MI_RING];
    int ring_busy[MI_RING], ring_next;
    float *dpool[6];
    mid_event ev_t[6];
    float last_ms[5];
} MiCtx;

#define MI_GUARD 256
void *mi_ctx_alloc(MiCtx *c, size_t bytes);
void mi_params_mark_dirty(void);
int mi_dp_plan_buckets(const Dims *d, size_t bucket_bytes, size_t *from, size_t *to, int max);
size_t mi_params_arena_floats(const Params *p);
float *mi_params_arena_base(const Params *p);
void mi_dp_reduce_ready(Train_ResNet *t, size_t from_float_offset, int force);
void mi_trainer_poll_errors(Train_ResNet *t);

#endif
```

resnet_amd/csrc/ops.c:

```c
#include <stdlib.h>
#include "mi_host.h"

void *mi_malloc(size_t bytes) {
    char *p = (char *)mid_malloc(bytes + 2 * MI_GUARD);
    return p ? p + MI_GUARD : NULL;
}
void mi_free(void *p) { if (p) mid_free((char *)p - MI_GUARD); }

static int finish(int rc) {
    mid_stream_sync(mi_global()->compute);
    if (rc) return rc;
    return mid_last_error()[0] ? -1 : 0;
}
static int ws_make(mid_workspace *ws, size_t wt, size_t part) {
    ws->wt_floats = wt; ws->part_floats = part;
    ws->pre_fwd = ws->pre_dgrad = NULL;
    ws->s2d = NULL; ws->s2d_bytes = 0; ws->s2d_valid = 0;
    ws->wt = wt ? (float *)mid_malloc(wt * sizeof(float)) : NULL;
    ws->part = part ? (float *)mid_malloc(part * sizeof(float)) : NULL;
    return (wt && !ws->wt) || (part && !ws->part);
}
static void ws_free(mid_workspace *ws) { mid_free(ws->wt); mid_free(ws->part); }

int mi_op_conv_fwd(const float *x, const float *w, float *y, int N, int C, int H, int K, int k, int stride) {
// ... 105 lines not shown
}
int mi_op_conv_dgrad_bn_bwd_bf16(const float *w, const void *dy, const void *addend, void *gated, int N, int C, int H, int K, int k, int stride,
                                 const void *bn_x, const void *mask, const float *gamma, const float *beta, const float *means,
                                 const float *vars, float eps, void *bn_dx, float *dgamma, float *dbeta) {
    mid_workspace ws;
    if (ws_make(&ws, (size_t)k * k * C * K, 0)) return -3;
    mid_bn_bwd_parts fz = {bn_x, mask, means, NULL, mid_bn_parts_floats(N, C, H), 0};
    fz.buf = (float *)mid_malloc(fz.floats * sizeof(float));
    float *bws = (float *)mid_malloc(mid_bn_ws_floats(C) * sizeof(float));
    if (addend) mid_memcpy_d2d(gated, addend, (size_t)N * C * H * H * 2, mi_global()->compute);
    int rc = mid_conv_dgrad_bn_bf16(mi_global()->compute, &ws, w, dy, gated, addend ? gated : NULL, N, C, H, K, k, stride, &fz);
    if (!rc) {
        if (fz.nparts > 0)
            rc = mid_bn_bwd_parts_t(mi_global()->compute, bws, &fz, bn_x, MID_BF16, gamma, beta, means, vars, gated, MID_BF16, bn_dx, dgamma, dbeta, N, C, H * H, eps);
        else {
            void *tmp = mi_malloc((size_t)N * C * H * H * 2);
            rc = mid_bn_bwd_t(mi_global()->compute, bws, bn_x, MID_BF16, gamma, beta, means, vars, gated, mask, tmp, MID_BF16, bn_dx, dgamma, dbeta, N, C, H * H, eps, 3);
            if (!rc) mid_memcpy_d2d(gated, tmp, (size_t)N * C * H * H * 2, mi_global()->compute);
            rc = finish(rc);
            mi_free(tmp);
        }
    }
    rc = finish(rc);
    mid_free(bws);
    mid_free(fz.buf);
    ws_free(&ws);
    return rc < 0 ? rc : fz.nparts;
}
int mi_op_conv_dgrad_bn_bwd_f32(const float *w, const float *dy, const float *addend, float *gated, int N, int C, int H, int K, int k, int stride,
                                const float *bn_x, const float *mask, const float *gamma, const float *beta, const float *means,
                                const float *vars, float eps, float *bn_dx, float *dgamma, float *dbeta) {
    mid_workspace ws;
    if (ws_make(&ws, mid_conv_ws_wt_floats(C, K, k), 0)) return -3;
    mid_bn_bwd_parts fz = {bn_x, mask, means, NULL, mid_bn_parts_floats(N, C, H), 0};
    fz.buf = (float *)mid_malloc(fz.floats * sizeof(float));
    float *bws = (float *)mid_malloc(mid_bn_ws_floats(C) * sizeof(float));
    const size_t bytes = (size_t)N * C * H * H * 4;
    if (addend) mid_memcpy_d2d(gated, addend, bytes, mi_global()->compute);
    int rc = mid_conv_dgrad_bn_f32(mi_global()->compute, &ws, w, dy, gated, addend ? gated : NULL, N, C, H, K, k, stride, &fz);
    if (!rc) {
        if (fz.nparts > 0)
            rc = mid_bn_bwd_parts_t(mi_global()->compute, bws, &fz, bn_x, MID_F32, gamma, beta, means, vars, gated, MID_F32, bn_dx, dgamma, dbeta, N, C, H * H, eps);
        else {
            float *tmp = (float *)mid_malloc(bytes);
            rc = mid_bn_bwd_t(mi_global()->compute, bws, bn_x, MID_F32, gamma, beta, means, vars, gated, mask, tmp, MID_F32, bn_dx, dgamma, dbeta, N, C, H * H, eps, 3);
            if (!rc) mid_memcpy_d2d(gated, tmp, bytes, mi_global()->compute);
            rc = finish(rc);
            mid_free(tmp);
        }
    }
    rc = finish(rc);
    mid_free(bws);
    mid_free(fz.buf);
    ws_free(&ws);
    return rc < 0 ? rc : fz.nparts;
}
int mi_op_stem_fwd_bf16(const float *x, const float *w, float *y, int N, int H) {
    if (!mid_stem_bf16_supported(3, H, 64, 7, 2)) return -2;
    const size_t xb = mid_stem_bf16_xp_bytes(N, H), sf = mid_stem_bf16_part_floats(N, H);
    void *xp = mi_malloc(xb);
    float *sc = (float *)mid_malloc(sf * sizeof(float));
    int rc = (!xp || !sc) ? -3 : finish(mid_stem_fwd_bf16(mi_global()->compute, x, w, y, MID_F32, xp, xb, sc, sf, N, H, NULL));
    mid_free(sc);
    mi_free(xp);
    return rc;
}
int mi_op_stem_wgrad_bf16(const float *x, const float *w, const float *dy, float *dw, int N, int H) {
    if (!mid_stem_bf16_supported(3, H, 64, 7, 2)) return -2;
    const size_t xb = mid_stem_bf16_xp_bytes(N, H), sf = mid_stem_bf16_part_floats(N, H);
    void *xp = mi_malloc(xb);
    float *sc = (float *)mid_malloc(sf * sizeof(float));
    float *y = (float *)mid_malloc((size_t)N * 64 * (H / 2) * (H / 2) * sizeof(float));
    int rc = (!xp || !sc || !y) ? -3 : mid_stem_fwd_bf16(mi_global()->compute, x, w, y, MID_F32, xp, xb, sc, sf, N, H, NULL);
    if (!rc) rc = mid_stem_wgrad_bf16(mi_global()->compute, xp, dy, MID_F32, dw, sc, sf, N, H);
    rc = finish(rc);
    mid_free(y);
    mid_free(sc);
    mi_free(xp);
    return rc;
}
int mi_op_stem_fwd_f32(const float *x, const float *w, float *y, int N, int H) {
    if (!mid_stem_bf16_supported(3, H, 64, 7, 2)) return -2;
    const size_t xb = mid_stem_f32_xp_bytes(N, H), sf = mid_stem_bf16_part_floats(N, H);
    void *xp = mi_malloc(xb);
    float *sc = (float *)mid_malloc(sf * sizeof(float));
    int rc = (!xp || !sc) ? -3 : finish(mid_stem_fwd_f32(mi_global()->compute, x, w, y, xp, xb, sc, sf, N, H, NULL));
    mid_free(sc);
    mi_free(xp);
    return rc;
}
int mi_op_stem_wgrad_f32(const float *x, const float *w, const float *dy, float *dw, int N, int H) {
    if (!mid_stem_bf16_supported(3, H, 64, 7, 2)) return -2;
    const size_t xb = mid_stem_f32_xp_bytes(N, H), sf = mid_stem_bf16_part_floats(N, H);
    void *xp = mi_malloc(xb);
    float *sc = (float *)mid_malloc(sf * sizeof(float));
    float *y = (float *)mid_malloc((size_t)N * 64 * (H / 2) * (H / 2) * sizeof(float));
    int rc = (!xp || !sc || !y) ? -3 : mid_stem_fwd_f32(mi_global()->compute, x, w, y, xp, xb, sc, sf, N, H, NULL);
    if (!rc) rc = mid_stem_wgrad_f32(mi_global()->compute, xp, dy, dw, sc, sf, N, H);
    rc = finish(rc);
    mid_free(y);
    mid_free(sc);
    mi_free(xp);
    return rc;
}
int mi_op_conv_bn_fwd_t(const void *x, const float *w, void *conv_out, int dt, const float *gamma, const float *beta, float *means,
                        float *vars, void *y, int N, int C, int H, int K, int k, int stride, float eps, int relu) {
    mid_workspace ws;
    const int Ho = H / stride;
    if (ws_make(&ws, dt == MID_BF16 ? (size_t)k * k * C * K : mid_conv_ws_wt_floats(C, K, k), 0)) return -3;
    mid_bn_parts parts = {NULL, mid_bn_parts_floats(N, K, Ho), 0};
    parts.buf = (float *)mid_malloc(parts.floats * sizeof(float));
    float *bws = (float *)mid_malloc(mid_bn_ws_floats(K) * sizeof(float));
    void *par = NULL;
    int rc;
    if (dt == MID_BF16) {
        if (stride == 2) { ws.s2d_bytes = (size_t)N * C * H * H * 2; par = mi_malloc(ws.s2d_bytes); ws.s2d = par; }
        rc = mid_conv_fwd_bf16(mi_global()->compute, &ws, x, w, conv_out, N, C, H, K, k, stride, &parts);
    } else rc = mid_conv_fwd_stats(mi_global()->compute, &ws, (const float *)x, w, (float *)conv_out, N, C, H, K, k, stride, &parts);
    if (!rc) rc = mid_bn_fwd_t(mi_global()->compute, bws, &parts, conv_out, dt, gamma, beta, NULL, means, vars, y, dt, NULL, NULL, N, K, Ho * Ho, eps, relu, NULL, 0);
    rc = finish(rc);
    mi_free(par);
    mid_free(bws);
    mid_free(parts.buf);
    ws_free(&ws);
    return rc < 0 ? rc : parts.nparts;
}
int mi_op_bn_fwd_t(const void *x, int x_dt, const float *gamma, const float *beta, const void *residual, float *means, float *vars,
                   void *y, int a_dt, int N, int C, int H, float eps, int relu) {
    float *ws = (float *)mid_malloc(mid_bn_ws_floats(C) * sizeof(float));
    int rc = finish(mid_bn_fwd_t(mi_global()->compute, ws, NULL, x, x_dt, gamma, beta, residual, means, vars, y, a_dt, NULL, NULL, N, C, H * H, eps, relu, NULL, 0));
    mid_free(ws);
    return rc;
}
int mi_op_bn_fwd_cl_bf16(const void *x, const float *gamma, const float *beta, const void *residual, float *means, float *vars, void *y, void *ycl,
                         int N, int C, int H, float eps, int par) {
    float *ws = (float *)mid_malloc(mid_bn_ws_floats(C) * sizeof(float));
    int rc = finish(mid_bn_fwd_t(mi_global()->compute, ws, NULL, x, MID_BF16, gamma, beta, residual, means, vars, y, MID_BF16, NULL, NULL, N, C, H * H, eps,
                                 residual ? 0 : 1, ycl, par ? -H : H));
    mid_free(ws);
    return rc;
}
int mi_op_bn_bwd_t(const void *x, int x_dt, const float *gamma, const float *beta, const float *means, const float *vars,
                   const void *dy, const void *mask_src, void *gated_out, int a_dt, void *dx, float *dgamma, float *dbeta, int N, int C,
                   int H, float eps, int mask_mode) {
    float *ws = (float *)mid_malloc(mid_bn_ws_floats(C) * sizeof(float));
    int rc = finish(mid_bn_bwd_t(mi_global()->compute, ws, x, x_dt, gamma, beta, means, vars, dy, mask_src, gated_out, a_dt, dx, dgamma, dbeta, N, C, H * H, eps, mask_mode));
    mid_free(ws);
    return rc;
}
int mi_op_bn_apply_t(const void *x, int x_dt, const float *gamma, const float *beta, const void *residual, const float *means,
                     const float *vars, void *y, int a_dt, int N, int C, int H, float eps, int relu) {
    return finish(mid_bn_apply_t(mi_global()->compute, x, x_dt, gamma, beta, residual, means, vars, y, a_dt, N, C, H * H, eps, relu, NULL, 0));
}
int mi_op_maxpool_fwd_t(const void *x, void *y, int dt, int *max_inds, int N, int C, int H, int k, int stride) {
    return finish(mid_maxpool_fwd_t(mi_global()->compute, x, y, dt, max_inds, N, C, H, k, stride));
}
int mi_op_maxpool_bwd_t(const int *max_inds, const void *dy, void *dx, int dt, int N, int C, int H, int k, int stride) {
    return finish(mid_maxpool_bwd_t(mi_global()->compute, max_inds, dy, dx, dt, N, C, H, k, stride));
}
int mi_op_avgpool_fwd_t(const void *x, int dt, float *y, int N, int C, int H) { return finish(mid_avgpool_fwd_t(mi_global()->compute, x, dt, y, N, C, H * H)); }
int mi_op_avgpool_bwd_t(const float *dy, void *dx, int dt, int N, int C, int H) { return finish(mid_avgpool_bwd_t(mi_global()->compute, dy, dx, dt, N, C, H * H)); }
int mi_bf16_conv_supported(int op, int N, int C, int H, int K, int k, int stride) { return mid_bf16_supported(op, N, C, H, K, k, stride); }
int mi_bf16_pw_wgrad_supported(int N, int C, int H, int K) { return mid_pw_wgrad_supported(N, C, H, K); }
void mi_clear_error(void) { mid_clear_error(); }

int mi_debug_bn_merge(int R, int C, float *means, float *vars, float *dgamma, float *dbeta, float *sums_out) {
    float *tmp = (float *)mid_malloc((size_t)R * 2 * C * sizeof(float));
    if (!tmp) return -3;
    int rc = finish(mid_bn_debug_merge(mi_global()->compute, R, C, means, vars, dgamma, dbeta, sums_out, tmp));
    mid_free(tmp);
    return rc;
}

int mi_op_conv_fwd_bf16_cl(const void *x, const float *w, void *y, int N, int C, int H, int K, int stride) {
    if (!mid_cl_supported(0, N, C, H, K, stride)) return -2;
    mid_stream st = mi_global()->compute;
    const size_t xb = mid_cl_operand_bytes(0, N, C, H, K, stride);
    void *xp = mid_malloc(xb), *at = mid_malloc((size_t)9 * C * K * 2);
    if (!xp || !at) { mid_free(xp); mid_free(at); return -3; }
    mid_memset(xp, 0, xb, st);
    int rc = mid_bf16_prelayout_fwd(st, w, at, K, C, 3);
    if (!rc) rc = mid_cl_relayout(st, x, xp, N, C, H, stride == 2);
    if (!rc) rc = mid_cl_fwd(st, xp, at, y, N, C, H, K, stride, NULL);
    rc = finish(rc);
    mid_free(xp); mid_free(at);
    return rc;
}
int mi_op_conv1x1_fwd_bf16_cl(const void *x, const float *w, void *y, int N, int C, int H, int K) {
    if (!mid_cl_pw_supported(N, C, H, K)) return -2;
    mid_stream st = mi_global()->compute;
    const size_t xb = (size_t)N * H * H * C * 2 + 4096;
    void *xp = mid_malloc(xb), *at = mid_malloc((size_t)C * K * 2);
    if (!xp || !at) { mid_free(xp); mid_free(at); return -3; }
    int rc = mid_bf16_prelayout_fwd(st, w, at, K, C, 1);
    if (!rc) rc = mid_cl_relayout_dense(st, x, xp, N, C, H);
    if (!rc) rc = mid_cl_pw_fwd(st, xp, at, y, N, C, H, K, NULL);
    rc = finish(rc);
    mid_free(xp); mid_free(at);
    return rc;
}
int mi_op_conv_dgrad_bf16_cl(const float *w, const void *dy, void *dx, int N, int C, int H, int K, int stride, int to_add) {
    if (stride == 2) {
        if (to_add || !mid_cl_dgrad2_supported(N, C, H, K)) return -2;
        mid_stream st2 = mi_global()->compute;
        const size_t yb2 = mid_cl_dgrad2_operand_bytes(N, K, H / 2);
        void *dyp2 = mid_malloc(yb2), *at2 = mid_malloc((size_t)9 * C * K * 2);
        if (!dyp2 || !at2) { mid_free(dyp2); mid_free(at2); return -3; }
        mid_memset(dyp2, 0, yb2, st2);
        int rc2 = mid_bf16_prelayout_dgrad(st2, w, at2, K, C, 3);
        if (!rc2) rc2 = mid_cl_relayout_end(st2, dy, dyp2, N, K, H / 2);
        if (!rc2) rc2 = mid_cl_dgrad2(st2, dyp2, at2, dx, N, C, H, K);
        rc2 = finish(rc2);
        mid_free(dyp2); mid_free(at2);
        return rc2;
    }
    if (!mid_cl_supported(1, N, C, H, K, 1)) return -2;
    mid_stream st = mi_global()->compute;
    const size_t yb = mid_cl_operand_bytes(1, N, C, H, K, 1);
    void *dyp = mid_malloc(yb), *at = mid_malloc((size_t)9 * C * K * 2);
    if (!dyp || !at) { mid_free(dyp); mid_free(at); return -3; }
    mid_memset(dyp, 0, yb, st);
    int rc = mid_bf16_prelayout_dgrad(st, w, at, K, C, 3);
    if (!rc) rc = mid_cl_relayout(st, dy, dyp, N, K, H, 0);
    if (!rc) rc = mid_cl_dgrad(st, dyp, at, dx, to_add ? dx : NULL, N, C, H, K);
    rc = finish(rc);
    mid_free(dyp); mid_free(at);
    return rc;
}

int mi_op_conv_wgrad_bf16_cl2(const void *x, const void *dy, float *dw, int N, int C, int H, int K, int stride) {
    if (!mid_cl_wgrad2_supported(N, C, H, K, stride)) return -2;
    mid_stream st = mi_global()->compute;
    const int Ho = H / stride;
    const size_t xb = mid_cl_operand_bytes(0, N, C, H, K, stride), yb = stride == 2 ? mid_cl_dgrad2_operand_bytes(N, K, Ho) : mid_cl_operand_bytes(1, N, C, H, K, 1),
                 pf = mid_cl_wgrad2_part_floats(N, C, H, K, stride);
    void *xp = mid_malloc(xb), *dyp = mid_malloc(yb);
    float *part = (float *)mid_malloc(pf * sizeof(float));
    if (!xp || !dyp || !part) { mid_free(xp); mid_free(dyp); mid_free(part); return -3; }
    mid_memset(xp, 0, xb, st);
    mid_memset(dyp, 0, yb, st);
    int rc = mid_cl_relayout(st, x, xp, N, C, H, stride == 2);
    if (!rc) rc = stride == 2 ? mid_cl_relayout_end(st, dy, dyp, N, K, Ho) : mid_cl_relayout(st, dy, dyp, N, K, H, 0);
    if (!rc) rc = mid_cl_wgrad2(st, xp, dyp, dw, part, pf, N, C, H, K, stride);
    rc = finish(rc);
    mid_free(xp); mid_free(dyp); mid_free(part);
    return rc;
}
int mi_op_conv_wgrad_bf16_cl(const void *x, const void *dy, float *dw, int N, int C, int H, int K, int stride) {
    if (!mid_cl_wgrad_supported(N, C, H, K, stride)) return -2;
    mid_stream st = mi_global()->compute;
    const size_t xb = mid_cl_operand_bytes(0, N, C, H, K, stride), pf = mid_cl_wgrad_part_floats(N, C, H, K, stride);
    void *xp = mid_malloc(xb);
    float *part = (float *)mid_malloc(pf * sizeof(float));
    if (!xp || !part) { mid_free(xp); mid_free(part); return -3; }
    mid_memset(xp, 0, xb, st);
    int rc = mid_cl_relayout(st, x, xp, N, C, H, stride == 2);
    if (!rc) rc = mid_cl_wgrad(st, xp, dy, dw, part, pf, N, C, H, K, stride);
    rc = finish(rc);
    mid_free(xp); mid_free(part);
    return rc;
}
```

resnet_amd/csrc/trainer.c:

```c
#include <math.h>
#include <stdio.h>
#include <stdlib.h>
#include <string.h>
#include "mi_host.h"

static MiGlobal G;
MiGlobal *mi_global(void) {
    if (!G.ready) {
        G.compute = mid_stream_create();
        G.comm = mid_stream_create();
        G.copy = mid_stream_create();
        G.aux = mid_stream_create_low_priority();
        G.ready = 1;
    }
    return &G;
}

int mi_device_count(void) { return mid_device_count(); }
int mi_set_device(int device) { return mid_set_device(device); }
const char *mi_last_error(void) { return mid_last_error(); }
void mi_device_synchronize(void) { mid_device_sync(); }
static unsigned long g_host_write_epoch = 0;
void mi_params_mark_dirty(void) { g_host_write_epoch++; }
void mi_copy_to_device(void *d, const void *s, size_t n) { MiGlobal *g = mi_global(); mid_memcpy_h2d(d, s, n, g->compute); mid_stream_sync(g->compute); g_host_write_epoch++; }
// ... 203 lines not shown
    } else {
        a->init_conv_applied = c->dtype == MID_BF16 ? c->stem_dx : pool[3];
        a->norm_init_conv = make_cache(c, (int)stem, f, 0);
        a->init_conv_activated = pool[2];
        a->init_convblock_input = pool[0];
    }
    for (int i = 0; i < d->n_conv_blocks; i++) {
        const ConvBlock *b = blocks[i];
        Activation_ConvBlock *k = (Activation_ConvBlock *)calloc(1, sizeof(Activation_ConvBlock));
        k->incoming_filters = b->incoming_filters; k->incoming_spatial_dim = b->incoming_spatial_dim;
        k->reduced_depth = b->reduced_depth; k->expanded_depth = b->expanded_depth; k->stride = b->stride;
        const int H = b->incoming_spatial_dim, Ho = H / b->stride;
        const size_t rsz = (size_t)N * b->reduced_depth * H * H, ssz = (size_t)N * b->reduced_depth * Ho * Ho,
                     osz = (size_t)N * b->expanded_depth * Ho * Ho;
        const int has_proj = b->projection != NULL;
        k->norm_post_reduced = make_cache(c, (int)rsz, b->reduced_depth, mode == 0);
        k->norm_post_spatial = make_cache(c, (int)ssz, b->reduced_depth, mode == 0);
        k->norm_post_expanded = make_cache(c, (int)osz, b->expanded_depth, mode == 0);
        if (has_proj) k->norm_post_projection = make_cache(c, (int)osz, b->expanded_depth, mode == 0);
        if (mode == 0) {
            k->post_reduced = aalloc(c, rsz); k->post_reduced_activated = rc ? c->rc_buf[0] : aalloc(c, rsz);
            k->post_spatial = aalloc(c, ssz); k->post_spatial_activated = rc ? c->rc_buf[1] : aalloc(c, ssz);
            k->post_expanded = aalloc(c, osz);
            if (has_proj) { k->transformed_residual = aalloc(c, osz); k->post_projection_norm_vals = rc ? c->rc_buf[0] : aalloc(c, osz); }
            k->output_activated = aalloc(c, osz);
            k->output = k->output_activated;
        } else if (mode == 2) {
            k->output_activated = aalloc(c, osz); k->output = aalloc(c, osz);
            k->transformed_residual = has_proj ? aalloc(c, osz) : NULL;
            k->post_expanded = aalloc(c, osz);
            k->post_spatial_activated = aalloc(c, ssz); k->post_spatial = aalloc(c, ssz);
            k->post_reduced_activated = aalloc(c, rsz); k->post_reduced = aalloc(c, rsz);
        } else {
            k->output_activated = pool[(i + 1) & 1];
            k->output = pool[5];
            k->transformed_residual = has_proj ? pool[2] : NULL;
            k->post_expanded = pool[3];
            k->post_spatial_activated = pool[4];
            k->post_spatial = pool[2];
            k->post_reduced_activated = pool[3];
            k->post_reduced = pool[4];
        }
        a->activation_conv_blocks[i] = k;
    }
    if (mode == 0) {
        a->final_conv_output_pooled = falloc(c, (size_t)N * d->final_depth);
        a->linear_output = falloc(c, (size_t)N * d->output);
    } else a->final_conv_output_pooled = falloc(c, (size_t)N * d->final_depth);
    return a;
}

static size_t max_tensor_elems(const Dims *d, ConvBlock **blocks, int N) {
    const int f = d->init_conv_filters, Hs = d->input / d->init_conv_stride;
    size_t m = (size_t)N * f * Hs * Hs;
    for (int i = 0; i < d->n_conv_blocks; i++) {
        const ConvBlock *b = blocks[i];
        const int H = b->incoming_spatial_dim, Ho = H / b->stride;
        size_t v[3] = {(size_t)N * b->reduced_depth * H * H, (size_t)N * b->expanded_depth * Ho * Ho,
                       (size_t)N * b->incoming_filters * H * H};
        for (int j = 0; j < 3; j++) if (v[j] > m) m = v[j];
    }
    return m;
}

static void *zalloc(MiCtx *c, size_t bytes) {
    void *p = mi_ctx_alloc(c, bytes);
    mid_memset(p, 0, bytes, G.compute);
    return p;
}
static void layer_init(MiLayer *L, const float *w, int C, int H, int K, int k, int stride) {
    memset(L, 0, sizeof *L);
    L->w = w; L->C = C; L->H = H; L->K = K; L->k = k; L->stride = stride;
}
static void plan_conv(MiCtx *c, MiLayer *L, int N, int site) {
    const MiOptions *o = &c->opt;
    const int C = L->C, H = L->H, K = L->K, s = L->stride;
    if (c->dtype == MID_BF16) {
        L->fwd = MI_FWD_BF16; L->dgrad = MI_DG_BF16; L->wgrad = MI_WG_BF16;
        if (L->k == 3 && s == 1 && o->cl_s1 && mid_cl_supported(0, N, C, H, K, 1)) {
            L->cl = zalloc(c, mid_cl_operand_bytes(0, N, C, H, K, 1));
            L->fwd = MI_FWD_CL;
            if (o->cl_s1_dgrad && mid_cl_supported(1, N, C, H, K, 1)) {
                L->dye = zalloc(c, mid_cl_operand_bytes(1, N, C, H, K, 1));
                L->dgrad = MI_DG_CL;
            }
        }
        if (s == 2) {
            if (o->cl_s2 && mid_cl_supported(0, N, C, H, K, 2)) {
                L->cl = zalloc(c, mid_cl_operand_bytes(0, N, C, H, K, 2));
                L->fwd = MI_FWD_CL;
            }
            if (o->cl_dgrad2 && mid_cl_dgrad2_supported(N, C, H, K)) {
                L->dye = zalloc(c, mid_cl_dgrad2_operand_bytes(N, K, H / 2));
                L->dgrad = MI_DG_CL2;
            }
        }
        const int P = (H / s) * (H / s);
        const int wg = L->cl && mid_cl_wgrad_supported(N, C, H, K, s), wg2 = L->cl && mid_cl_wgrad2_supported(N, C, H, K, s);
        if (L->dye && wg2 && (P % 64 != 0 || !wg)) L->wgrad = MI_WG_CL2;
        else if (wg) L->wgrad = MI_WG_CL;
        if (s == 2 && (L->fwd == MI_FWD_BF16 || (!wg && !wg2))) {
            const size_t e = (size_t)N * C * H * H;
            L->par_bytes = e * 2;
            L->par = (char *)mi_ctx_alloc(c, e * 2 + 2 * MI_GUARD) + MI_GUARD;
        }
    }
    const int f32_sites = mid_igemm_mode() >= 2 ? o->bnfuse_bwd_f32 : 0;
    L->fz = site && o->bnfuse_bwd &&
            (L->dgrad == MI_DG_BF16 || (L->dgrad == MI_DG_F32 && (f32_sites & site) && c->policy != MI_STORE_FULL));
}
static void plan_layers(MiCtx *c, const Params *p, const Dims *d, int N) {
    const MiOptions *o = &c->opt;
    ConvBlock **blocks = p->conv_blocks;
    const int f = d->init_conv_filters;
    MiLayer *S = &c->stem;
    layer_init(S, p->init_conv_layer, 3, d->input, f, d->init_kernel_dim, d->init_conv_stride);
    c->stem_bf16 = 0;
    const int stem_mc = mid_stem_bf16_supported(3, d->input, f, d->init_kernel_dim, d->init_conv_stride);
    if (c->dtype == MID_F32 && mid_igemm_mode() > 0 && stem_mc && o->stem_mfma) {
        S->xp_bytes = mid_stem_f32_xp_bytes(N, d->input);
        S->scratch_floats = mid_stem_bf16_part_floats(N, d->input);
        S->xp = falloc(c, (S->xp_bytes + 3) / 4);
        S->scratch = falloc(c, S->scratch_floats);
        S->fwd = MI_FWD_STEM_F32; S->wgrad = MI_WG_STEM_F32;
    }
    if (c->dtype == MID_BF16 && stem_mc && o->bf16_stem) {
        S->xp_bytes = mid_stem_bf16_xp_bytes(N, d->input);
        S->scratch_floats = mid_stem_bf16_part_floats(N, d->input);
        S->xp = aalloc(c, (S->xp_bytes + 1) / 2);
        S->scratch = falloc(c, S->scratch_floats);
        S->fwd = MI_FWD_STEM_BF16; S->wgrad = MI_WG_STEM_BF16;
        c->stem_bf16 = !o->stem_tensors_f32;
    }
    free(c->blk);
    c->blk = (MiBlockLayers *)calloc((size_t)(d->n_conv_blocks > 0 ? d->n_conv_blocks : 1), sizeof(MiBlockLayers));
    free(c->wt_tab);
    c->wt_tab = (mid_wt_entry *)calloc((size_t)(4 * d->n_conv_blocks + 1), sizeof(mid_wt_entry));
    c->wt_n = 0; c->wt_tiles = 0;
    for (int i = 0; i < d->n_conv_blocks; i++) {
        const ConvBlock *b = blocks[i];
        MiBlockLayers *B = &c->blk[i];
        const int H = b->incoming_spatial_dim, s = b->stride;
        layer_init(&B->red, b->depth_reduction, b->incoming_filters, H, b->reduced_depth, 1, 1);
        layer_init(&B->spa, b->spatial, b->reduced_depth, H, b->reduced_depth, 3, s);
        layer_init(&B->exp, b->depth_expansion, b->reduced_depth, H / s, b->expanded_depth, 1, 1);
        plan_conv(c, &B->red, N, i > 0 && !blocks[i - 1]->projection ? 4 : 0);
        plan_conv(c, &B->spa, N, 2);
        plan_conv(c, &B->exp, N, 1);
        if (B->spa.cl) B->spa.cl_by_bn = s == 1 || !(H & 1);
        if (b->projection) {
            layer_init(&B->proj, b->projection, b->incoming_filters, H, b->expanded_depth, s == 2 ? 3 : 1, s);
            plan_conv(c, &B->proj, N, 0);
            if (B->proj.cl) B->proj.cl_by_bn = i > 0 && !(H & 1);
        }
        MiLayer *Ls[4] = {&B->red, &B->spa, &B->exp, &B->proj};
        for (int j = 0; j < 4; j++) {
            MiLayer *L = Ls[j];
            int nf = 0, nd = 0;
            if (L->w && c->dtype == MID_BF16) nf = nd = 1;
            else if (L->w && o->prelayout) mid_conv_prelayout_needs(N, L->C, L->H, L->K, L->k, L->stride, &nf, &nd);
            if (!nf && !nd) continue;
            mid_wt_entry *e = &c->wt_tab[c->wt_n++];
            const size_t n = ((size_t)L->k * L->k * L->C * L->K) / (c->dtype == MID_BF16 ? 2 : 1);
            e->w = L->w; e->K = L->K; e->C = L->C; e->T = L->k * L->k;
            e->fwd = nf ? falloc(c, n) : NULL; e->dgrad = nd ? falloc(c, n) : NULL;
            e->tile0 = c->wt_tiles; c->wt_tiles += (L->C / 32) * (L->K / 32);
            L->we = e;
        }
    }
    c->wt_tab_dev = NULL; c->wt_tile_entry_dev = NULL;
    if (c->wt_n) {
        int *te = (int *)malloc((size_t)c->wt_tiles * sizeof(int));
        for (int e = 0; e < c->wt_n; e++) {
            const int nt = (c->wt_tab[e].C / 32) * (c->wt_tab[e].K / 32);
            for (int q = 0; q < nt; q++) te[c->wt_tab[e].tile0 + q] = e;
        }
        c->wt_tab_dev = (mid_wt_entry *)mi_ctx_alloc(c, (size_t)c->wt_n * sizeof(mid_wt_entry));
        c->wt_tile_entry_dev = (int *)mi_ctx_alloc(c, (size_t)c->wt_tiles * sizeof(int));
        mid_memcpy_h2d(c->wt_tab_dev, c->wt_tab, (size_t)c->wt_n * sizeof(mid_wt_entry), G.compute);
        mid_memcpy_h2d(c->wt_tile_entry_dev, te, (size_t)c->wt_tiles * sizeof(int), G.compute);
        mid_stream_sync(G.compute);
        free(te);
    }
}
static void size_layer_ws(const MiCtx *c, const MiLayer *L, int N, size_t *wt, size_t *part, int *maxc) {
    const int C = L->C, H = L->H, K = L->K, k = L->k, s = L->stride;
    size_t a = mid_conv_ws_wt_floats(C, K, k), b = mid_conv_ws_part_floats(N, C, H, K, k, s);
    if (c->dtype == MID_BF16 && k <= 3) { size_t e = mid_bf16_part_floats(N, C, H, K, k, s); if (e > b) b = e; }
    if (c->dtype == MID_BF16 && k == 3 && mid_cl_wgrad_supported(N, C, H, K, s)) { size_t e = mid_cl_wgrad_part_floats(N, C, H, K, s); if (e > b) b = e; }
    if (c->dtype == MID_BF16 && k == 3 && mid_cl_wgrad2_supported(N, C, H, K, s)) { size_t e = mid_cl_wgrad2_part_floats(N, C, H, K, s); if (e > b) b = e; }
    if (a > *wt) *wt = a;
    if (b > *part) *part = b;
    if (K > *maxc) *maxc = K;
}
static void size_workspaces(MiCtx *c, const Dims *d, int N) {
    size_t wt = 0, part = 0, pf = 0;
    int maxc = d->init_conv_filters;
    size_layer_ws(c, &c->stem, N, &wt, &part, &maxc);
    for (int i = 0; i < d->n_conv_blocks; i++) {
        const MiBlockLayers *B = &c->blk[i];
        size_layer_ws(c, &B->red, N, &wt, &part, &maxc);
        size_layer_ws(c, &B->spa, N, &wt, &part, &maxc);
        size_layer_ws(c, &B->exp, N, &wt, &part, &maxc);
        if (B->proj.w) size_layer_ws(c, &B->proj, N, &wt, &part, &maxc);
        const size_t a = mid_bn_parts_floats(N, B->red.K, B->red.H), e = mid_bn_parts_floats(N, B->exp.K, B->exp.H);
        if (a > pf) pf = a;
        if (e > pf) pf = e;
    }
    c->ws.s2d = NULL; c->ws.s2d_bytes = 0; c->ws.s2d_valid = 0;
    c->ws.wt_floats = wt; c->ws.part_floats = part;
    c->ws.wt = wt ? falloc(c, wt) : NULL;
    c->ws.part = part ? falloc(c, part) : NULL;
    c->bn_ws = falloc(c, mid_bn_ws_floats(maxc));
    c->bn_parts.floats = pf;
    c->bn_parts.buf = pf ? falloc(c, pf) : NULL;
    c->bn_parts.nparts = 0;
}

static MiCtx *ctx_of(Train_ResNet *t) { return (MiCtx *)t->backend_ctx; }
static void free_activations_host(Activations *a);
static void add_full_store_extras(Train_ResNet *t);
static void build_buffers(Train_ResNet *t) {
    MiCtx *c = (MiCtx *)t->backend_ctx;
    Dims *d = t->model->dims;
    ConvBlock **blocks = t->model->params->conv_blocks;
    const int N = t->batch_size;
    const size_t maxe = max_tensor_elems(d, blocks, N);
    c->act_bytes = 0;
    c->rc_buf[0] = c->rc_buf[1] = NULL;
    if (c->policy == MI_STORE_RECOMPUTE_BN) { c->rc_buf[0] = aalloc(c, maxe); c->rc_buf[1] = aalloc(c, maxe); }
    c->counting_act = 1;
    t->forward_buffer->activations = build_activations(c, d, blocks, N, NULL, 0);
    c->counting_act = 0;
    c->full_store = 0;
    if (c->policy == MI_STORE_FULL) add_full_store_extras(t);
    const int f = d->init_conv_filters, Hs = d->input / d->init_conv_stride;
    c->stem_dx = c->dtype == MID_BF16 ? falloc(c, (size_t)N * f * Hs * Hs) : NULL;
    float *pool[6];
    for (int i = 0; i < 6; i++) pool[i] = aalloc(c, maxe);
    for (int i = 0; i < 6; i++) c->dpool[i] = pool[i];
    for (int i = 0; i < MI_RING; i++) { c->ring_buf[i] = i < 4 ? pool[2 + i] : aalloc(c, maxe); c->ring_busy[i] = 0; }
    c->ring_next = 0;
    t->backprop_buffer->activation_derivs = build_activations(c, d, blocks, N, pool, c->policy == MI_STORE_FULL ? 2 : 1);
    if ((c->policy != MI_STORE_FAST || c->dtype != MID_F32) && c->overlap_wgrad > 1) c->overlap_wgrad = 1;
    if (c->dtype == MID_BF16 && !c->opt.overlap_given && !c->overlap_set) c->overlap_wgrad = 0;
    plan_layers(c, t->model->params, d, N);
    size_workspaces(c, d, N);
    mid_stream_sync(G.compute);
}
static void drop_buffers(Train_ResNet *t) {
    MiCtx *c = (MiCtx *)t->backend_ctx;
    mid_device_sync();
    ctx_free_from(c, c->n_persist);
    free_activations_host(t->forward_buffer->activations);
    free_activations_host(t->backprop_buffer->activation_derivs);
    t->forward_buffer->activations = NULL; t->backprop_buffer->activation_derivs = NULL;
    c->wt_n = 0; c->wt_tiles = 0; c->wt_tab_dev = NULL; c->wt_tile_entry_dev = NULL;
    c->wgrad_pending = 0;
}

static void read_options(MiOptions *o) {
#define ENV_INT(name_, default_) (getenv(name_) ? atoi(getenv(name_)) : (default_))
    o->cl_s1 = ENV_INT("RESNET_MI_BF16_CL_S1", 1) != 0;
    o->cl_s1_dgrad = ENV_INT("RESNET_MI_BF16_CL_S1_DGRAD", 1) != 0;
    o->cl_s2 = ENV_INT("RESNET_MI_BF16_CL_S2", 1) != 0;
    o->cl_dgrad2 = ENV_INT("RESNET_MI_BF16_CL_DGRAD2", 1) != 0;
    o->stem_mfma = ENV_INT("RESNET_MI_STEM_MFMA", 1) != 0;
    o->bf16_stem = ENV_INT("RESNET_MI_BF16_STEM", 1) != 0;
    o->stem_tensors_f32 = getenv("RESNET_MI_BF16_STEM_TENSORS") && !strcmp(getenv("RESNET_MI_BF16_STEM_TENSORS"), "f32");
    o->bnfuse_bwd = ENV_INT("RESNET_MI_BF16_BNFUSE_BWD", 1) != 0;
    o->bnfuse_bwd_f32 = ENV_INT("RESNET_MI_F32_BNFUSE_BWD", 4);
    o->overlap = ENV_INT("RESNET_MI_OVERLAP", 1);
    o->overlap_given = getenv("RESNET_MI_OVERLAP") != NULL;
    o->bnfuse = ENV_INT("RESNET_MI_BNFUSE", 1);
    o->prelayout = ENV_INT("RESNET_MI_PRELAYOUT", 1);
#undef ENV_INT
}
Train_ResNet *init_trainer(ResNet *model, Batch *cur_batch, int batch_size, float learning_rate, float weight_decay,
                           float mean_decay, float var_decay, float eps, int n_epochs, const char *dump_dir) {
    Train_ResNet *t = (Train_ResNet *)calloc(1, sizeof(Train_ResNet));
    MiCtx *c = (MiCtx *)calloc(1, sizeof(MiCtx));
    Dims *d = model->dims;
    mi_global();
    t->backend_ctx = c;
    t->model = model; t->cur_batch = cur_batch; t->batch_size = batch_size;
    c->dump_every = 1000;
    c->input_reset = 1;
    c->world = 1; c->bucket_bytes = (size_t)32 << 20;
    c->dtype = MID_F32; c->policy = MI_STORE_FAST;
    read_options(&c->opt);
    c->overlap_wgrad = c->opt.overlap;
    c->ev_bn_done = mid_event_create(); c->ev_wgrad_done = mid_event_create();

    Forward_Buffer *fb = (Forward_Buffer *)calloc(1, sizeof(Forward_Buffer));
    fb->pred = falloc(c, (size_t)batch_size * d->output);
    fb->pred_cpu = (float *)mid_malloc_host((size_t)batch_size * d->output * sizeof(float));
    t->forward_buffer = fb;
    Backprop_Buffer *bb = (Backprop_Buffer *)calloc(1, sizeof(Backprop_Buffer));
    bb->output_layer_deriv = falloc(c, (size_t)batch_size * d->output);
    bb->param_derivs = build_params(d, NULL, c);
    bb->prev_means = build_params(d, NULL, c);
    bb->prev_vars = build_params(d, NULL, c);
    t->backprop_buffer = bb;
    c->arena_floats = mi_params_arena_floats(model->params);
    c->g_arena = mi_params_arena_base(bb->param_derivs);
    c->m_arena = mi_params_arena_base(bb->prev_means);
// ... 38 lines not shown
Train_ResNet *init_trainer_cudnn_abi(ResNet *model, Batch *cur_batch, int batch_size, float learning_rate,
                                     float weight_decay, float mean_decay, float var_decay, float eps, int n_epochs,
                                     void *handle, const char *dump_dir) {
    (void)handle;
    return init_trainer(model, cur_batch, batch_size, learning_rate, weight_decay, mean_decay, var_decay, eps, n_epochs, dump_dir);
}

static void add_full_store_extras(Train_ResNet *t) {
    MiCtx *c = ctx_of(t);
    Activations *a = t->forward_buffer->activations;
    c->counting_act = 1;
#define EXTRA(cache) do { (cache)->normalized_temp = falloc(c, (cache)->input_size); (cache)->normalized = falloc(c, (cache)->input_size); } while (0)
    EXTRA(a->norm_init_conv);
    for (int i = 0; i < a->n_conv_blocks; i++) {
        Activation_ConvBlock *k = a->activation_conv_blocks[i];
        EXTRA(k->norm_post_reduced); EXTRA(k->norm_post_spatial); EXTRA(k->norm_post_expanded);
        if (k->norm_post_projection) EXTRA(k->norm_post_projection);
        k->post_expanded_norm_vals = falloc(c, k->norm_post_expanded->input_size);
        k->output = falloc(c, k->norm_post_expanded->input_size);
    }
#undef EXTRA
    c->counting_act = 0;
    c->full_store = 1;
}
static int bf16_net_supported(const Train_ResNet *t, char *why, size_t whylen) {
    const Dims *d = t->model->dims;
    ConvBlock **blocks = t->model->params->conv_blocks;
    const int N = t->batch_size;
    for (int i = 0; i < d->n_conv_blocks; i++) {
        const ConvBlock *b = blocks[i];
        const int H = b->incoming_spatial_dim;
        const int L[4][5] = {{b->incoming_filters, H, b->reduced_depth, 1, 1},
                             {b->reduced_depth, H, b->reduced_depth, 3, b->stride},
                             {b->reduced_depth, H / b->stride, b->expanded_depth, 1, 1},
                             {b->incoming_filters, H, b->expanded_depth, b->stride == 2 ? 3 : 1, b->stride}};
        for (int j = 0; j < (b->projection ? 4 : 3); j++)
            for (int op = 0; op < 3; op++)
                if (!mid_bf16_supported(op, N, L[j][0], L[j][1], L[j][2], L[j][3], L[j][4])) {
                    snprintf(why, whylen, "block %d conv %d (C=%d H=%d K=%d k=%d s=%d) op %d does not tile for the bf16 kernels", i, j,
                             L[j][0], L[j][1], L[j][2], L[j][3], L[j][4], op);
                    return 0;
                }
    }
    return 1;
}
void mi_record_host_error(const char *what, const char *detail);
int mi_trainer_set_store_policy(Train_ResNet *t, int policy) {
    MiCtx *c = ctx_of(t);
    if (policy < MI_STORE_FAST || policy > MI_STORE_FULL) { mi_record_host_error("mi_trainer_set_store_policy", "unknown policy"); return -1; }
    if (policy == MI_STORE_FULL && c->dtype != MID_F32) { mi_record_host_error("mi_trainer_set_store_policy", "the FULL policy (x-hat / BN-out / pre-ReLU sums) exists in fp32 only"); return -1; }
    if (policy == c->policy) return 0;
    drop_buffers(t);
    c->policy = policy;
    build_buffers(t);
    return 0;
}
void mi_trainer_set_full_store(Train_ResNet *t, int on) { (void)mi_trainer_set_store_policy(t, on ? MI_STORE_FULL : MI_STORE_FAST); }
int mi_trainer_set_dtype(Train_ResNet *t, int dtype) {
    MiCtx *c = ctx_of(t);
    if (dtype != MID_F32 && dtype != MID_BF16) { mi_record_host_error("mi_trainer_set_dtype", "unknown dtype"); return -1; }
    if (dtype == c->dtype) return 0;
    if (dtype == MID_BF16) {
        char why[256];
        if (c->policy == MI_STORE_FULL) { mi_record_host_error("mi_trainer_set_dtype", "the FULL store policy exists in fp32 only"); return -1; }
        if (!bf16_net_supported(t, why, sizeof why)) { mi_record_host_error("mi_trainer_set_dtype", why); return -1; }
    }
    drop_buffers(t);
    c->dtype = dtype;
    build_buffers(t);
    return 0;
}
int mi_trainer_get_dtype(const Train_ResNet *t) { return ((MiCtx *)t->backend_ctx)->dtype; }
size_t mi_trainer_activation_bytes(const Train_ResNet *t) { return ((MiCtx *)t->backend_ctx)->act_bytes; }
size_t mi_trainer_device_bytes(const Train_ResNet *t) {
    const MiCtx *c = (MiCtx *)t->backend_ctx;
    return c->dev_bytes + c->arena_floats * sizeof(float);
}
void mi_trainer_set_dump_every(Train_ResNet *t, int every) { ctx_of(t)->dump_every = every; }
void mi_trainer_set_overlap(Train_ResNet *t, int mode) {
    MiCtx *c = ctx_of(t);
    mid_stream_sync(G.aux); mid_stream_sync(G.compute);
    c->overlap_wgrad = mode < 0 ? 0 : mode > 2 ? 2 : mode;
    c->overlap_set = 1;
    if ((c->policy != MI_STORE_FAST || c->dtype != MID_F32) && c->overlap_wgrad > 1) c->overlap_wgrad = 1;
    c->wgrad_pending = 0;
    for (int i = 0; i < MI_RING; i++) c->ring_busy[i] = 0;
    if (c->overlap_wgrad != 2) {
        Activations *da = t->backprop_buffer->activation_derivs;
        float **pool = c->dpool;
        if (c->policy == MI_STORE_FULL) return;
        da->init_conv_applied = c->dtype == MID_BF16 ? c->stem_dx : pool[3]; da->init_conv_activated = pool[2];
        for (int i = 0; i < da->n_conv_blocks; i++) {
            Activation_ConvBlock *k = da->activation_conv_blocks[i];
            k->output = pool[5];
            if (k->transformed_residual) k->transformed_residual = pool[2];
            k->post_expanded = pool[3]; k->post_spatial_activated = pool[4]; k->post_spatial = pool[2];
            k->post_reduced_activated = pool[3]; k->post_reduced = pool[4];
        }
    }
}
void mi_trainer_set_input_reset(Train_ResNet *t, int on) { ctx_of(t)->input_reset = on; }
void mi_trainer_set_dump_root(Train_ResNet *t, const char *root) {
    MiCtx *c = ctx_of(t);
    free(c->dump_root);
    c->dump_root = root ? strdup(root) : NULL;
}
void mi_trainer_last_timings(Train_ResNet *t, float out_ms[5]) {
    MiCtx *c = ctx_of(t);
    mid_stream_sync(G.compute);
    out_ms[0] = 0;
    out_ms[1] = mid_event_elapsed_ms(c->ev_t[0], c->ev_t[1]);
    out_ms[2] = mid_event_elapsed_ms(c->ev_t[2], c->ev_t[3]);
    out_ms[3] = mid_event_elapsed_ms(c->ev_t[4], c->ev_t[5]);
    out_ms[4] = c->last_ms[4];
}

static void relayout_weights(MiCtx *c) {
    if (c->dtype == MID_BF16) ck(mid_conv_prelayout_all_bf16(G.compute, c->wt_tab_dev, c->wt_tile_entry_dev, c->wt_tiles), "weight re-layout (bf16)");
    else ck(mid_conv_prelayout_all(G.compute, c->wt_tab_dev, c->wt_tile_entry_dev, c->wt_tiles), "weight re-layout");
    c->params_dirty = 0;
    c->host_epoch_seen = g_host_write_epoch;
}
static int weights_stale(const MiCtx *c) { return c->params_dirty || c->host_epoch_seen != g_host_write_epoch; }
void dump_trainer(int dump_id, Train_ResNet *trainer, const char *special_dir);
static void poll_nan_flag(Train_ResNet *t) {
    MiCtx *c = ctx_of(t);
    if (!c->nan_check_pending) return;
    c->nan_check_pending = 0;
    if (*c->nan_flag_host) {
        printf("ERROR: nan or inf found at location: %d\n", *c->nan_flag_host - 1);
        printf("Dumping data to id=99999999 and exiting...\n");
        c->nan_location = *c->nan_flag_host - 1;
        if (c->dp_pending) mid_stream_sync(G.comm);
        dump_trainer(99999999, t, t->dump_dir);
        if (c->nan_no_exit) {
            mid_memset(c->nan_flag_dev, 0, sizeof(int), G.compute);
            mid_stream_sync(G.compute);
            *c->nan_flag_host = 0;
            return;
        }
        abort_all_comms();
        exit(1);
    }
}
void mi_trainer_poll_errors(Train_ResNet *t) {
    MiCtx *c = ctx_of(t);
    if (!c || !c->nan_check_pending) return;
    mid_event_sync(c->ev_nan);
    poll_nan_flag(t);
}

static int conv_out_dt(const MiCtx *c, const MiLayer *L) { return L == &c->stem ? (c->stem_bf16 ? MID_BF16 : MID_F32) : c->dtype; }
static void unit_fwd(Train_ResNet *t, MiLayer *L, const float *in, const BatchNorm *bn, Cache_BatchNorm *cache, float *conv_out,
                     float *act_out, const float *residual, int relu, const MiLayer *cl_reader) {
    MiCtx *c = ctx_of(t);
    const int N = t->batch_size, C = L->C, H = L->H, K = L->K, Ho = H / L->stride;
    const int bf_ops = L->fwd == MI_FWD_BF16 || L->fwd == MI_FWD_CL || L->fwd == MI_FWD_STEM_BF16;
    mid_bn_parts *parts = (c->opt.bnfuse || bf_ops) ? &c->bn_parts : NULL;
    c->ws.s2d = L->par; c->ws.s2d_bytes = L->par_bytes; c->ws.s2d_valid = 0;
    c->ws.pre_fwd = L->we ? L->we->fwd : NULL;
    switch (L->fwd) {
    case MI_FWD_STEM_F32:
        ck(mid_stem_fwd_f32(G.compute, in, L->w, conv_out, L->xp, L->xp_bytes, L->scratch, L->scratch_floats, N, H, parts),
           "stem convolution forward (fp32 matrix cores)");
        break;
    case MI_FWD_STEM_BF16:
        ck(mid_stem_fwd_bf16(G.compute, in, L->w, conv_out, conv_out_dt(c, L), L->xp, L->xp_bytes, L->scratch, L->scratch_floats, N, H, parts),
           "stem convolution forward (bf16 operands)");
        break;
    case MI_FWD_CL:
        if (!L->cl_by_bn) ck(mid_cl_relayout(G.compute, in, L->cl, N, C, H, L->stride == 2), "input re-layout (channel-last parity planes)");
        ck(mid_cl_fwd(G.compute, L->cl, L->we->fwd, conv_out, N, C, H, K, L->stride, parts), "convolution forward (bf16, channel-last)");
        L->par_valid = 0;
        break;
    case MI_FWD_BF16:
        ck(mid_conv_fwd_bf16(G.compute, &c->ws, in, L->w, conv_out, N, C, H, K, L->k, L->stride, parts), "convolution forward (bf16)");
        L->par_valid = c->ws.s2d_valid;
        break;
    default: ck(mid_conv_fwd_stats(G.compute, &c->ws, in, L->w, conv_out, N, C, H, K, L->k, L->stride, parts), "convolution forward");
    }
    c->ws.pre_fwd = NULL;
    void *ycl = cl_reader && cl_reader->cl_by_bn ? cl_reader->cl : NULL;
    const int Hcl = ycl ? (cl_reader->stride == 2 ? -cl_reader->H : cl_reader->H) : 0;
    ck(mid_bn_fwd_t(G.compute, c->bn_ws, parts, conv_out, conv_out_dt(c, L), bn->gamma, bn->beta, residual, cache->means, cache->vars,
                    act_out, c->dtype, cache->normalized_temp, cache->normalized, N, K, Ho * Ho, t->eps, relu, ycl, Hcl), "batch norm forward");
}

#define MI_SYNC_BN_TMP_FLOATS (2 * 4096)
static void bind_sync_bn(const MiCtx *c) {
    if (c->sync_bn && c->sync_bn_comm) mid_bn_set_sync(c->sync_bn_comm, c->world, c->sync_bn_tmp, MI_SYNC_BN_TMP_FLOATS, 1);
    else mid_bn_set_sync(NULL, 1, NULL, 0, 0);
}
void forward_pass(Train_ResNet *t) {
    MiCtx *c = ctx_of(t);
    const Dims *d = t->model->dims;
    const Params *p = t->model->params;
    Activations *a = t->forward_buffer->activations;
    const int N = t->batch_size, f = d->init_conv_filters;
    mid_event_record(c->ev_t[0], G.compute);
    bind_sync_bn(c);
    relayout_weights(c);
    unit_fwd(t, &c->stem, t->cur_batch->images, p->norm_init_conv, a->norm_init_conv, a->init_conv_applied, a->init_conv_activated,
             NULL, 1, NULL);
    const int Hs = d->input / d->init_conv_stride;
    ck(mid_maxpool_fwd_t(G.compute, a->init_conv_activated, a->init_convblock_input, c->dtype, a->max_inds, N, f, Hs, d->init_maxpool_dim,
                         d->init_maxpool_stride), "max-pool forward");
    const float *bin = a->init_convblock_input;
    for (int i = 0; i < d->n_conv_blocks; i++) {
        const ConvBlock *b = p->conv_blocks[i];
        MiBlockLayers *B = &c->blk[i];
        Activation_ConvBlock *k = a->activation_conv_blocks[i];
        const int Ho = b->incoming_spatial_dim / b->stride;
        unit_fwd(t, &B->red, bin, b->norm_depth_reduction, k->norm_post_reduced, k->post_reduced, k->post_reduced_activated, NULL, 1, &B->spa);
        unit_fwd(t, &B->spa, k->post_reduced_activated, b->norm_spatial, k->norm_post_spatial, k->post_spatial, k->post_spatial_activated,
                 NULL, 1, NULL);
        const float *res = bin;
        if (b->projection) {
            unit_fwd(t, &B->proj, bin, b->norm_projection, k->norm_post_projection, k->transformed_residual, k->post_projection_norm_vals,
                     NULL, 0, NULL);
            res = k->post_projection_norm_vals;
        }
        if (!c->full_store) {
            unit_fwd(t, &B->exp, k->post_spatial_activated, b->norm_expansion, k->norm_post_expanded, k->post_expanded, k->output_activated,
                     res, 0, i + 1 < d->n_conv_blocks ? &c->blk[i + 1].proj : NULL);
        } else {
            unit_fwd(t, &B->exp, k->post_spatial_activated, b->norm_expansion, k->norm_post_expanded, k->post_expanded,
                     k->post_expanded_norm_vals, NULL, 0, NULL);
            ck(mid_add_relu(G.compute, k->post_expanded_norm_vals, res, k->output, k->output_activated,
                            (size_t)N * b->expanded_depth * Ho * Ho), "add + ReLU");
        }
        bin = k->output_activated;
    }
    const ConvBlock *last = p->conv_blocks[d->n_conv_blocks - 1];
    const int Hl = last->incoming_spatial_dim;
    ck(mid_avgpool_fwd_t(G.compute, bin, c->dtype, a->final_conv_output_pooled, N, d->final_depth, Hl * Hl), "average pool");
    ck(mid_gemm_nn(G.compute, a->final_conv_output_pooled, p->fully_connected, a->linear_output, N, d->final_depth, d->output), "FC forward");
    ck(mid_softmax(G.compute, a->linear_output, t->forward_buffer->pred, N, d->output), "soft-max");
    mid_event_record(c->ev_t[1], G.compute);
    mid_memcpy_d2h(t->forward_buffer->pred_cpu, t->forward_buffer->pred, (size_t)N * d->output * sizeof(float), G.compute);
    mid_stream_sync(G.compute);
    poll_nan_flag(t);
}

float mi_host_loss(Train_ResNet *t, int *n_wrong) {
    const int N = t->batch_size, L = t->model->dims->output;
    const float *pred = t->forward_buffer->pred_cpu;
    const int *lab = t->cur_batch->correct_classes_cpu;
    float loss = 0;
    int wrong = 0;
    for (int s = 0; s < N; s++) loss += -1 * logf(pred[(size_t)s * L + lab[s]]);
    for (int s = 0; s < N; s++) {
        const float pc = pred[(size_t)s * L + lab[s]];
        for (int cc = 0; cc < L; cc++)
            if (cc != lab[s] && pred[(size_t)s * L + cc] >= pc) { wrong++; break; }
    }
    if (n_wrong) *n_wrong = wrong;
    return loss;
}

static void join_wgrad(MiCtx *c) {
    if (c->wgrad_pending) { mid_stream_wait_event(G.compute, c->ev_wgrad_done); c->wgrad_pending = 0; }
}
static float *ring_take(MiCtx *c, int *slot) {
    const int i = c->ring_next;
    c->ring_next = (i + 1) % MI_RING;
    if (c->ring_busy[i]) { mid_stream_wait_event(G.compute, c->ring_ev[i]); c->ring_busy[i] = 0; }
    if (slot) *slot = i;
    return c->ring_buf[i];
}
static void conv_dgrad_t(Train_ResNet *t, const MiLayer *L, const float *dy, float *dx, const float *addend, const mid_bn_bwd_parts *req,
                         mid_bn_bwd_parts *fz) {
    MiCtx *c = ctx_of(t);
    const int N = t->batch_size, C = L->C, H = L->H, K = L->K, k = L->k, s = L->stride;
    if (L->dgrad == MI_DG_CL) {
        ck(mid_cl_dgrad(G.compute, L->dye, L->we->dgrad, dx, addend, N, C, H, K), "convolution dgrad (bf16, channel-last)");
        return;
    }
    if (L->dgrad == MI_DG_CL2) {
        ck(mid_cl_dgrad2(G.compute, L->dye, L->we->dgrad, dx, N, C, H, K), "convolution dgrad (bf16, channel-last, stride 2)");
        return;
    }
    c->ws.pre_dgrad = L->we ? L->we->dgrad : NULL;
    if (req) *fz = *req;
    if (L->dgrad == MI_DG_BF16 && req)
        ck(mid_conv_dgrad_bn_bf16(G.compute, &c->ws, L->w, dy, dx, addend, N, C, H, K, k, s, fz), "convolution dgrad + BN' reduction (bf16)");
    else if (req)
        ck(mid_conv_dgrad_bn_f32(G.compute, &c->ws, L->w, dy, dx, addend, N, C, H, K, k, s, fz), "convolution dgrad + BN' reduction");
    else if (L->dgrad == MI_DG_BF16) ck(mid_conv_dgrad_bf16(G.compute, &c->ws, L->w, dy, dx, addend, N, C, H, K, k, s), "convolution dgrad (bf16)");
    else ck(mid_conv_dgrad(G.compute, &c->ws, L->w, dy, dx, addend, N, C, H, K, k, s), "convolution dgrad");
    c->ws.pre_dgrad = NULL;
}
static void conv_wgrad_t(Train_ResNet *t, const MiLayer *L, mid_stream st, const float *x, const float *dy, float *dw) {
    MiCtx *c = ctx_of(t);
    const int N = t->batch_size, C = L->C, H = L->H, K = L->K, k = L->k, s = L->stride;
    c->ws.s2d = L->par; c->ws.s2d_bytes = L->par_bytes; c->ws.s2d_valid = L->par && L->par_valid;
    switch (L->wgrad) {
    case MI_WG_STEM_F32:
        ck(mid_stem_wgrad_f32(st, L->xp, dy, dw, L->scratch, L->scratch_floats, N, H), "stem convolution wgrad (fp32 matrix cores)");
        break;
    case MI_WG_STEM_BF16:
        ck(mid_stem_wgrad_bf16(st, L->xp, dy, conv_out_dt(c, L), dw, L->scratch, L->scratch_floats, N, H), "stem convolution wgrad (bf16 operands)");
        break;
    case MI_WG_CL2:
        ck(mid_cl_wgrad2(st, L->cl, L->dye, dw, c->ws.part, c->ws.part_floats, N, C, H, K, s), "convolution wgrad (bf16, both operands channel-last)");
        break;
    case MI_WG_CL:
        ck(mid_cl_wgrad(st, L->cl, dy, dw, c->ws.part, c->ws.part_floats, N, C, H, K, s), "convolution wgrad (bf16, channel-last input)");
        break;
    case MI_WG_BF16: ck(mid_conv_wgrad_bf16(st, &c->ws, x, dy, dw, N, C, H, K, k, s), "convolution wgrad (bf16)"); break;
    default: ck(mid_conv_wgrad(st, &c->ws, x, dy, dw, N, C, H, K, k, s), "convolution wgrad");
    }
}
static void unit_bwd(Train_ResNet *t, MiLayer *L, const float *in, const BatchNorm *bn, const Cache_BatchNorm *cache,
                     const BatchNorm *dbn, const float *conv_out, const float *dy, const float *mask_src, int mask_mode,
                     float *gated_out, float *d_conv_out, int d_slot, float *dx, const float *addend, float *dw, mid_bn_bwd_parts *fz,
                     const mid_bn_bwd_parts *fz_req) {
    MiCtx *c = ctx_of(t);
    const int N = t->batch_size, K = L->K, Ho = L->H / L->stride;
    const int x_dt = conv_out_dt(c, L);
    if (fz->nparts > 0) {
        ck(mid_bn_bwd_parts_t(G.compute, c->bn_ws, fz, conv_out, x_dt, bn->gamma, bn->beta, cache->means, cache->vars, dy, c->dtype,
                              d_conv_out, dbn->gamma, dbn->beta, N, K, Ho * Ho, t->eps), "batch norm backward (reduction done by the dgrad)");
        fz->nparts = 0;
    } else
    ck(mid_bn_bwd_t(G.compute, c->bn_ws, conv_out, x_dt, bn->gamma, bn->beta, cache->means, cache->vars, dy, mask_src, gated_out, c->dtype,
                    d_conv_out, dbn->gamma, dbn->beta, N, K, Ho * Ho, t->eps, mask_mode), "batch norm backward");
    if (L->dgrad == MI_DG_CL)
        ck(mid_cl_relayout(G.compute, d_conv_out, L->dye, N, K, Ho, 0), "dY re-layout (channel-last)");
    else if (L->dgrad == MI_DG_CL2)
        ck(mid_cl_relayout_end(G.compute, d_conv_out, L->dye, N, K, Ho), "dY re-layout (channel-last)");
    if (c->overlap_wgrad == 2 && d_slot >= 0) {
        mid_event_record(c->ev_bn_done, G.compute);
        mid_stream_wait_event(G.aux, c->ev_bn_done);
        conv_wgrad_t(t, L, G.aux, in, d_conv_out, dw);
        mid_event_record(c->ring_ev[d_slot], G.aux);
        c->ring_busy[d_slot] = 1;
        mid_event_record(c->ev_wgrad_done, G.aux);
        c->wgrad_pending = 1;
        if (dx) conv_dgrad_t(t, L, d_conv_out, dx, addend, fz_req, fz);
        return;
    }
    join_wgrad(c);
    if (dx) conv_dgrad_t(t, L, d_conv_out, dx, addend, fz_req, fz);
    if (c->overlap_wgrad) {
        mid_event_record(c->ev_bn_done, G.compute);
        mid_stream_wait_event(G.aux, c->ev_bn_done);
        conv_wgrad_t(t, L, G.aux, in, d_conv_out, dw);
        mid_event_record(c->ev_wgrad_done, G.aux);
        c->wgrad_pending = 1;
    } else conv_wgrad_t(t, L, G.compute, in, d_conv_out, dw);
}
static const mid_bn_bwd_parts *fz_request(const MiCtx *c, mid_bn_bwd_parts *r, const MiLayer *L, const void *x, const void *mask,
                                          const float *means) {
    if (!L->fz) return NULL;
    r->x = x; r->mask = mask; r->means = means;
    r->buf = c->bn_parts.buf; r->floats = c->bn_parts.floats; r->nparts = 0;
    return r;
}

void backwards_pass(Train_ResNet *t) {
    MiCtx *c = ctx_of(t);
    const Dims *d = t->model->dims;
    const Params *p = t->model->params;
    Activations *a = t->forward_buffer->activations;
    Backprop_Buffer *bb = t->backprop_buffer;
    const Params *dp = bb->param_derivs;
    Activations *da = bb->activation_derivs;
    const int N = t->batch_size, L = d->output, D = d->final_depth, nb = d->n_conv_blocks;
    const int recompute = c->policy == MI_STORE_RECOMPUTE_BN;
    mid_event_record(c->ev_t[2], G.compute);
    bind_sync_bn(c);
    if (weights_stale(c)) relayout_weights(c);
    c->dp_cursor = c->arena_floats;
    c->n_buckets = 0;
    ck(mid_ce_deriv(G.compute, t->forward_buffer->pred, t->cur_batch->correct_classes, bb->output_layer_deriv, N, L), "cross-entropy derivative");
    ck(mid_gemm_tn(G.compute, a->final_conv_output_pooled, bb->output_layer_deriv, dp->fully_connected, D, N, L), "FC wgrad");
    ck(mid_gemm_nt(G.compute, bb->output_layer_deriv, p->fully_connected, da->final_conv_output_pooled, N, L, D), "FC dgrad");
    mi_dp_reduce_ready(t, (size_t)(dp->fully_connected - c->g_arena), 0);
    const ConvBlock *last = p->conv_blocks[nb - 1];
    const int Hl = last->incoming_spatial_dim;
    ck(mid_avgpool_bwd_t(G.compute, da->final_conv_output_pooled, da->activation_conv_blocks[nb - 1]->output_activated, c->dtype, N, D, Hl * Hl),
       "average pool backward");
    const int ring = c->overlap_wgrad == 2;
    mid_bn_bwd_parts fz = {NULL}, req;
    for (int i = nb - 1; i >= 0; i--) {
        const ConvBlock *b = p->conv_blocks[i];
        const ConvBlock *db = dp->conv_blocks[i];
        MiBlockLayers *B = &c->blk[i];
        const Activation_ConvBlock *k = a->activation_conv_blocks[i];
        const Activation_ConvBlock *kb = i == 0 ? NULL : a->activation_conv_blocks[i - 1];
        Activation_ConvBlock *dk = da->activation_conv_blocks[i];
        const float *bin = i == 0 ? a->init_convblock_input : kb->output_activated;
        float *dbin = i == 0 ? da->init_convblock_input : da->activation_conv_blocks[i - 1]->output_activated;
        const int H = b->incoming_spatial_dim, Ho = H / b->stride;
// ... 244 lines not shown
```

resnet_amd/ops.py:

```python
import ctypes as C

import numpy as np

from . import binding as B


class DeviceArray:
    def __init__(self, lib, arr=None, shape=None, dtype=np.float32):
        self.L = lib
        if arr is not None:
            arr = np.ascontiguousarray(arr)
            shape, dtype = arr.shape, arr.dtype
        self.shape, self.dtype = tuple(shape), np.dtype(dtype)
        self.nbytes = int(np.prod(self.shape)) * self.dtype.itemsize
        self.ptr = lib.mi_malloc(max(self.nbytes, 4))
        if not self.ptr:
            raise MemoryError(lib.mi_last_error().decode())
        if arr is not None:
            lib.mi_copy_to_device(self.ptr, arr.ctypes.data, self.nbytes)

    def get(self):
        out = np.empty(self.shape, self.dtype)
        self.L.mi_copy_to_host(out.ctypes.data, self.ptr, self.nbytes)
        return out
# ... 170 lines not shown
        self._chk(self.L.mi_op_conv_fwd_bf16(dx.ptr, dw.ptr, dy.ptr, N, Cc, H, K, k, stride), "conv_fwd_bf16")
        return self.get_t(dy, BF)

    def conv_fwd_bf16_cl(self, x, w, stride):
        N, Cc, H, _ = x.shape
        K = w.shape[0]
        BF = B.MI_DTYPE_BF16
        dx, dw = self.dev_t(x, BF), self.dev(w)
        dy = self.new_t((N, K, H // stride, H // stride), BF)
        self._chk(self.L.mi_op_conv_fwd_bf16_cl(dx.ptr, dw.ptr, dy.ptr, N, Cc, H, K, stride), "conv_fwd_bf16_cl")
        return self.get_t(dy, BF)

    def conv_wgrad_bf16_cl(self, x, dy, stride):
        N, Cc, H, _ = x.shape
        K = dy.shape[1]
        BF = B.MI_DTYPE_BF16
        dx, ddy = self.dev_t(x, BF), self.dev_t(dy, BF)
        dw = self.dev(shape=(K, Cc, 3, 3))
        self._chk(self.L.mi_op_conv_wgrad_bf16_cl(dx.ptr, ddy.ptr, dw.ptr, N, Cc, H, K, stride), "conv_wgrad_bf16_cl")
        return dw.get()

    def bn_fwd_cl_bf16(self, x, gamma, beta, eps, residual=None, par=False):
        N, Cc, H, _ = x.shape
        BF = B.MI_DTYPE_BF16
        dx, dg, db = self.dev_t(x, BF), self.dev(gamma), self.dev(beta)
        dr = self.dev_t(residual, BF) if residual is not None else None
        dm, dv, dy = self.dev(shape=(Cc,)), self.dev(shape=(Cc,)), self.new_t(x.shape, BF)
        shp = (N, 4, H // 2 + 1, H // 2 + 1, Cc) if par else (N, H + 2, H + 2, Cc)
        ycl = self.dev_t(np.zeros(shp, np.float32), BF)
        self._chk(self.L.mi_op_bn_fwd_cl_bf16(dx.ptr, dg.ptr, db.ptr, dr.ptr if dr else None, dm.ptr, dv.ptr, dy.ptr, ycl.ptr, N, Cc, H, eps, int(par)),
                  "bn_fwd_cl_bf16")
        return dm.get(), dv.get(), self.get_t(dy, BF), self.get_t(ycl, BF)

    def conv1x1_fwd_bf16_cl(self, x, w):
        N, Cc, H, _ = x.shape
        K = w.shape[0]
        BF = B.MI_DTYPE_BF16
        dx, dw = self.dev_t(x, BF), self.dev(w)
        dy = self.new_t((N, K, H, H), BF)
        self._chk(self.L.mi_op_conv1x1_fwd_bf16_cl(dx.ptr, dw.ptr, dy.ptr, N, Cc, H, K), "conv1x1_fwd_bf16_cl")
        return self.get_t(dy, BF)

    def conv_wgrad_bf16_cl2(self, x, dy, stride=2):
        N, Cc, H, _ = x.shape
        K = dy.shape[1]
        BF = B.MI_DTYPE_BF16
        dx, ddy = self.dev_t(x, BF), self.dev_t(dy, BF)
        dw = self.dev(shape=(K, Cc, 3, 3))
        self._chk(self.L.mi_op_conv_wgrad_bf16_cl2(dx.ptr, ddy.ptr, dw.ptr, N, Cc, H, K, stride), "conv_wgrad_bf16_cl2")
        return dw.get()

    def conv_dgrad_bf16_cl(self, w, dy, H, dx_init=None, stride=1):
        K, Cc, k, _ = w.shape
        N = dy.shape[0]
        BF = B.MI_DTYPE_BF16
        dw_, ddy = self.dev(w), self.dev_t(dy, BF)
        ddx = self.dev_t(dx_init, BF) if dx_init is not None else self.new_t((N, Cc, H, H), BF)
        self._chk(self.L.mi_op_conv_dgrad_bf16_cl(dw_.ptr, ddy.ptr, ddx.ptr, N, Cc, H, K, stride, 0 if dx_init is None else 1), "conv_dgrad_bf16_cl")
        return self.get_t(ddx, BF)

    def conv_dgrad_bf16(self, w, dy, H, stride, dx_init=None):
        K, Cc, k, _ = w.shape
        N = dy.shape[0]
        BF = B.MI_DTYPE_BF16
        dw_, ddy = self.dev(w), self.dev_t(dy, BF)
        ddx = self.dev_t(dx_init, BF) if dx_init is not None else self.new_t((N, Cc, H, H), BF)
        self._chk(self.L.mi_op_conv_dgrad_bf16(dw_.ptr, ddy.ptr, ddx.ptr, N, Cc, H, K, k, stride, 0 if dx_init is None else 1), "conv_dgrad_bf16")
        return self.get_t(ddx, BF)

    def conv_wgrad_bf16(self, x, dy, k, stride):
        N, Cc, H, _ = x.shape
        K = dy.shape[1]
        BF = B.MI_DTYPE_BF16
        dx, ddy = self.dev_t(x, BF), self.dev_t(dy, BF)
        dw = self.dev(shape=(K, Cc, k, k))
        self._chk(self.L.mi_op_conv_wgrad_bf16(dx.ptr, ddy.ptr, dw.ptr, N, Cc, H, K, k, stride), "conv_wgrad_bf16")
        return dw.get()

    def bn_fwd_t(self, x, gamma, beta, eps, relu, x_dt, a_dt, residual=None):
        N, Cc, H, _ = x.shape
        dx, dg, db = self.dev_t(x, x_dt), self.dev(gamma), self.dev(beta)
        dm, dv, dy = self.dev(shape=(Cc,)), self.dev(shape=(Cc,)), self.new_t(x.shape, a_dt)
        dr = self.dev_t(residual, a_dt) if residual is not None else None
        self._chk(self.L.mi_op_bn_fwd_t(dx.ptr, x_dt, dg.ptr, db.ptr, dr.ptr if dr else None, dm.ptr, dv.ptr, dy.ptr, a_dt, N, Cc, H, eps,
                                        int(relu)), "bn_fwd_t")
        return dm.get(), dv.get(), self.get_t(dy, a_dt)

    def conv_dgrad_bn_bwd_bf16(self, w, dy, H, stride, bn_x, mask, gamma, beta, means, vars_, eps, addend=None):
        N = dy.shape[0]
        K, Cc, k, _ = w.shape
        BF = B.MI_DTYPE_BF16
        dw, ddy = self.dev(w), self.dev_t(dy, BF)
        dadd = self.dev_t(addend, BF) if addend is not None else None
        dxb, dmask = self.dev_t(bn_x, BF), self.dev_t(mask, BF)
        dg, db, dm, dv = (self.dev(a) for a in (gamma, beta, means, vars_))
        gated, bdx = self.new_t((N, Cc, H, H), BF), self.new_t((N, Cc, H, H), BF)
        og, ob = self.dev(shape=(Cc,)), self.dev(shape=(Cc,))
        rc = self.L.mi_op_conv_dgrad_bn_bwd_bf16(dw.ptr, ddy.ptr, dadd.ptr if dadd else None, gated.ptr, N, Cc, H, K, k, stride, dxb.ptr, dmask.ptr,
                                                 dg.ptr, db.ptr, dm.ptr, dv.ptr, eps, bdx.ptr, og.ptr, ob.ptr)
        if rc < 0:
            self._chk(rc, "conv_dgrad_bn_bwd_bf16")
        return self.get_t(gated, BF), self.get_t(bdx, BF), og.get(), ob.get(), rc > 0

    def conv_dgrad_bn_bwd_f32(self, w, dy, H, stride, bn_x, mask, gamma, beta, means, vars_, eps, addend=None):
        N = dy.shape[0]
        K, Cc, k, _ = w.shape
        dw, ddy = self.dev(w), self.dev(dy)
        dadd = self.dev(addend) if addend is not None else None
        dxb, dmask = self.dev(bn_x), self.dev(mask)
        dg, db, dm, dv = (self.dev(a) for a in (gamma, beta, means, vars_))
        gated, bdx = self.dev(shape=(N, Cc, H, H)), self.dev(shape=(N, Cc, H, H))
        og, ob = self.dev(shape=(Cc,)), self.dev(shape=(Cc,))
        rc = self.L.mi_op_conv_dgrad_bn_bwd_f32(dw.ptr, ddy.ptr, dadd.ptr if dadd else None, gated.ptr, N, Cc, H, K, k, stride, dxb.ptr, dmask.ptr,
                                                dg.ptr, db.ptr, dm.ptr, dv.ptr, eps, bdx.ptr, og.ptr, ob.ptr)
        if rc < 0:
            self._chk(rc, "conv_dgrad_bn_bwd_f32")
        return gated.get(), bdx.get(), og.get(), ob.get(), rc > 0

    def stem_fwd_bf16(self, x, w, exact=False):
        N, _, H, _ = x.shape
        dx, dw, dy = self.dev(x), self.dev(w), self.dev(shape=(N, 64, H // 2, H // 2))
        fn = self.L.mi_op_stem_fwd_f32 if exact else self.L.mi_op_stem_fwd_bf16
        self._chk(fn(dx.ptr, dw.ptr, dy.ptr, N, H), "stem_fwd")
        return dy.get()

    def stem_wgrad_bf16(self, x, w, dy, exact=False):
        N, _, H, _ = x.shape
        dx, dw, ddy, out = self.dev(x), self.dev(w), self.dev(dy), self.dev(shape=w.shape)
        fn = self.L.mi_op_stem_wgrad_f32 if exact else self.L.mi_op_stem_wgrad_bf16
        self._chk(fn(dx.ptr, dw.ptr, ddy.ptr, out.ptr, N, H), "stem_wgrad")
        return out.get()

    def conv_bn_fwd_t(self, x, w, gamma, beta, stride, eps, relu, dt):
        N, Cc, H, _ = x.shape
        K, _, k, _ = w.shape
        Ho = H // stride
        dx, dw, dg, db = self.dev_t(x, dt), self.dev(w), self.dev(gamma), self.dev(beta)
        dc, dy = self.new_t((N, K, Ho, Ho), dt), self.new_t((N, K, Ho, Ho), dt)
        dm, dv = self.dev(shape=(K,)), self.dev(shape=(K,))
        rc = self.L.mi_op_conv_bn_fwd_t(dx.ptr, dw.ptr, dc.ptr, dt, dg.ptr, db.ptr, dm.ptr, dv.ptr, dy.ptr, N, Cc, H, K, k, stride, eps, int(relu))
        if rc < 0:
            self._chk(rc, "conv_bn_fwd_t")
        return self.get_t(dc, dt), dm.get(), dv.get(), self.get_t(dy, dt), rc > 0

    def bn_apply_t(self, x, gamma, beta, means, vars_, eps, relu, x_dt, a_dt, residual=None):
        N, Cc, H, _ = x.shape
        dx, dg, db, dm, dv = self.dev_t(x, x_dt), self.dev(gamma), self.dev(beta), self.dev(means), self.dev(vars_)
        dy = self.new_t(x.shape, a_dt)
        dr = self.dev_t(residual, a_dt) if residual is not None else None
        self._chk(self.L.mi_op_bn_apply_t(dx.ptr, x_dt, dg.ptr, db.ptr, dr.ptr if dr else None, dm.ptr, dv.ptr, dy.ptr, a_dt, N, Cc, H, eps,
                                          int(relu)), "bn_apply_t")
        return self.get_t(dy, a_dt)

    def bn_bwd_t(self, x, gamma, beta, means, vars_, dy, eps, mask_mode, x_dt, a_dt, mask_src=None):
        N, Cc, H, _ = x.shape
        dx, ddy = self.dev_t(x, x_dt), self.dev_t(dy, a_dt)
        dg, db, dm, dv = (self.dev(a) for a in (gamma, beta, means, vars_))
        dmask = self.dev_t(mask_src, a_dt) if mask_src is not None else None
        gated = self.new_t(x.shape, a_dt) if mask_mode == 3 else None
        out, ogam, obet = self.new_t(x.shape, x_dt), self.dev(shape=(Cc,)), self.dev(shape=(Cc,))
        self._chk(self.L.mi_op_bn_bwd_t(dx.ptr, x_dt, dg.ptr, db.ptr, dm.ptr, dv.ptr, ddy.ptr, dmask.ptr if dmask else None,
                                        gated.ptr if gated else None, a_dt, out.ptr, ogam.ptr, obet.ptr, N, Cc, H, eps, mask_mode), "bn_bwd_t")
        res = (self.get_t(out, x_dt), ogam.get(), obet.get())
        return res + (self.get_t(gated, a_dt),) if gated else res

    def maxpool_fwd_t(self, x, k, stride, dt):
        N, Cc, H, _ = x.shape
        Ho = H // stride
        dx, dy, di = self.dev_t(x, dt), self.new_t((N, Cc, Ho, Ho), dt), self.dev(shape=(N, Cc, Ho, Ho), dtype=np.int32)
        self._chk(self.L.mi_op_maxpool_fwd_t(dx.ptr, dy.ptr, dt, di.ptr, N, Cc, H, k, stride), "maxpool_fwd_t")
        return self.get_t(dy, dt), di.get()

    def maxpool_bwd_t(self, idx, dy, H, k, stride, dt):
        N, Cc = dy.shape[:2]
        di, ddy, dx = self.dev(idx.astype(np.int32)), self.dev_t(dy, dt), self.new_t((N, Cc, H, H), dt)
        self._chk(self.L.mi_op_maxpool_bwd_t(di.ptr, ddy.ptr, dx.ptr, dt, N, Cc, H, k, stride), "maxpool_bwd_t")
        return self.get_t(dx, dt)

    def avgpool_fwd_t(self, x, dt):
        N, Cc, H, _ = x.shape
        dx, dy = self.dev_t(x, dt), self.dev(shape=(N, Cc))
        self._chk(self.L.mi_op_avgpool_fwd_t(dx.ptr, dt, dy.ptr, N, Cc, H), "avgpool_fwd_t")
        return dy.get()

    def avgpool_bwd_t(self, dy, H, dt):
        N, Cc = dy.shape
        ddy, dx = self.dev(dy), self.new_t((N, Cc, H, H), dt)
        self._chk(self.L.mi_op_avgpool_bwd_t(ddy.ptr, dx.ptr, dt, N, Cc, H), "avgpool_bwd_t")
        return self.get_t(dx, dt)
```

resnet_amd/trainer.py:

```python
import ctypes as C

import numpy as np

from . import binding as B


def resnet_dims(input=224, n_conv_blocks=16, reductions=(3, 7, 13), final_depth=2048, output=1000,
                init_conv_filters=64):
    return dict(input=input, init_kernel_dim=7, init_conv_filters=init_conv_filters, init_conv_stride=2,
                init_maxpool_dim=3, init_maxpool_stride=2, n_conv_blocks=n_conv_blocks,
                is_block_spatial_reduction=[1 if i in reductions else 0 for i in range(n_conv_blocks)],
                final_depth=final_depth, output=output)


class Trainer:
    def __init__(self, dims, batch, lr=1e-4, wd=0.0, b1=0.9, b2=0.999, eps=1e-7, seed=1234, n_epochs=1,
                 dump_dir="default", shard_n_images=None, device=None):
        self.L = L = B.load()
        if device is not None:
            if L.mi_set_device(int(device)) != 0:
                raise RuntimeError(self.error())
        self.dims, self.batch = dict(dims), batch
        nb = dims["n_conv_blocks"]
        self._flags = (C.c_int * max(nb, 1))(*dims["is_block_spatial_reduction"])
        self.c_dims = L.init_dimensions(dims["input"], dims["init_kernel_dim"], dims["init_conv_filters"],
                                        dims["init_conv_stride"], dims["init_maxpool_dim"], dims["init_maxpool_stride"],
                                        nb, self._flags, dims["final_depth"], dims["output"])
        rng = L.mi_rng_create(seed)
        self.model = L.init_resnet(self.c_dims, rng)
        L.mi_rng_destroy(rng)
        image_size = dims["input"] * dims["input"] * 3
        self.c_batch = L.init_general_batch(batch, image_size, dims["input"], shard_n_images or batch)
        self._dump_dir = dump_dir.encode()
        self.t = L.init_trainer(self.model, self.c_batch, batch, lr, wd, b1, b2, eps, n_epochs, self._dump_dir)
        self.check()
        p = self.t.contents.model.contents.params.contents
        self.n_locations = p.n_locations
        self.sizes = [p.sizes[i] for i in range(p.n_locations)]
        L.mi_trainer_set_dump_every(self.t, 0)
        self.dtype = B.MI_DTYPE_F32

    def set_dtype(self, dtype):
        if self.L.mi_trainer_set_dtype(self.t, int(dtype)) != 0:
            e = self.error()
            self.L.mi_clear_error()
            raise RuntimeError("mi_trainer_set_dtype: " + e)
        self.dtype = int(dtype)

    def set_store_policy(self, policy):
        if self.L.mi_trainer_set_store_policy(self.t, int(policy)) != 0:
            e = self.error()
            self.L.mi_clear_error()
            raise RuntimeError("mi_trainer_set_store_policy: " + e)

    def activation_bytes(self):
        return int(self.L.mi_trainer_activation_bytes(self.t))

    def device_bytes(self):
        return int(self.L.mi_trainer_device_bytes(self.t))

    def check_errors(self):
        return int(self.L.mi_trainer_check_errors(self.t))

    def error(self):
        return self.L.mi_last_error().decode()

    def check(self):
        e = self.error()
        if e:
            raise RuntimeError("libresnet_mi: " + e)

    def close(self):
        if self.t:
            self.L.destroy_trainer(self.t)
            self.t = None

    def _to_host(self, ptr, n, dtype=np.float32):
        out = np.empty(n, dtype)
        self.L.mi_copy_to_host(out.ctypes.data, C.cast(ptr, C.c_void_p), n * 4)
        return out

    def _act_to_host(self, ptr, n):
        if self.dtype == B.MI_DTYPE_F32:
            return self._to_host(ptr, n)
        raw = np.empty(n, np.uint16)
        self.L.mi_copy_to_host(raw.ctypes.data, C.cast(ptr, C.c_void_p), n * 2)
        return (raw.astype(np.uint32) << 16).view(np.float32)

    def _to_dev(self, ptr, arr):
        arr = np.ascontiguousarray(arr)
        self.L.mi_copy_to_device(C.cast(ptr, C.c_void_p), arr.ctypes.data, arr.nbytes)

    def _pset(self, which):
        t = self.t.contents
        if which == "params":
            return t.model.contents.params.contents
        bb = t.backprop_buffer.contents
        return {"grads": bb.param_derivs, "means": bb.prev_means, "vars": bb.prev_vars}[which].contents

    def get(self, which, i):
        p = self._pset(which)
        return self._to_host(p.locations[i], p.sizes[i])

    def set(self, which, i, arr):
        p = self._pset(which)
        assert arr.size == p.sizes[i]
        self._to_dev(p.locations[i], arr.astype(np.float32).ravel())

    def set_params(self, arrays):
        for i, a in enumerate(arrays):
            self.set("params", i, a)

    def source_synthetic(self, seed_images=1234, seed_labels=1235, pool_batches=2):
        self.L.mi_batch_source_synthetic(self.c_batch, seed_images, seed_labels, self.dims["output"], pool_batches)
        self.check()

    def source_host(self, layout=B.MI_LAYOUT_NHWC):
        self.L.mi_batch_source_host(self.c_batch, layout)

    def source_buffer(self, images_path, labels_path, layout=B.MI_LAYOUT_NHWC):
        self.L.mi_batch_source_buffer(self.c_batch, images_path.encode(), labels_path.encode(), layout)

    def source_shards(self, shard_dir, layout=B.MI_LAYOUT_NCHW, prefetch=False):
        self.L.mi_batch_source_shards(self.c_batch, shard_dir.encode(), layout)
        if prefetch:
            self.L.mi_batch_set_prefetch(self.c_batch, 1)

    def fill_host_batch(self, images, labels):
        b = self.c_batch.contents
        n = b.n_images * b.image_size
        np.ctypeslib.as_array(b.images_float_cpu, shape=(n,))[:] = np.ascontiguousarray(images, np.float32).ravel()
        np.ctypeslib.as_array(b.correct_classes_cpu, shape=(b.n_images,))[:] = np.asarray(labels, np.int32)

    def load_new_batch(self):
        self.L.load_new_batch(self.t, None, self.c_batch)

    def forward(self):
        self.L.forward_pass(self.t)

    def loss(self):
        nw = C.c_int(0)
        return float(self.L.mi_host_loss(self.t, C.byref(nw))), nw.value

    def backward(self):
        self.L.backwards_pass(self.t)

    def update(self):
        self.L.update_parameters(self.t)

    def step(self):
        self.load_new_batch()
        self.forward()
        loss = self.loss()
        self.backward()
        self.update()
        return loss

    def pred(self):
        t = self.t.contents
        n = self.batch * self.dims["output"]
        return np.ctypeslib.as_array(t.forward_buffer.contents.pred_cpu, shape=(n,)).reshape(self.batch, -1).copy()

    def stem_dtype(self):
        return self.L.mi_trainer_stem_dtype(self.t)

    def labels(self):
        return np.ctypeslib.as_array(self.c_batch.contents.correct_classes_cpu, shape=(self.batch,)).copy()

    def timings(self):
        out = (C.c_float * 5)()
        self.L.mi_trainer_last_timings(self.t, C.byref(out))
        return list(out)

    def activation(self, name, deriv=False):
        t = self.t.contents
        a = (t.backprop_buffer.contents.activation_derivs if deriv else t.forward_buffer.contents.activations).contents
        d, N = self.dims, self.batch
        f = d["init_conv_filters"]
        Hs = d["input"] // d["init_conv_stride"]
        Hp = Hs // d["init_maxpool_stride"]
        if name == "input":
            return self._to_host(self.c_batch.contents.images, N * 3 * d["input"] ** 2).reshape(N, 3, d["input"], d["input"])
        if name == "init_conv_applied":
            get = self._act_to_host if self.stem_dtype() == B.MI_DTYPE_BF16 else self._to_host
            return get(a.init_conv_applied, N * f * Hs * Hs).reshape(N, f, Hs, Hs)
        if name == "init_conv_activated":
            return self._act_to_host(a.init_conv_activated, N * f * Hs * Hs).reshape(N, f, Hs, Hs)
        if name == "init_convblock_input":
            return self._act_to_host(a.init_convblock_input, N * f * Hp * Hp).reshape(N, f, Hp, Hp)
        if name == "max_inds":
            return self._to_host(a.max_inds, N * f * Hp * Hp, np.int32).reshape(N, f, Hp, Hp)
        if name == "final_avg_pool":
            return self._to_host(a.final_conv_output_pooled, N * d["final_depth"]).reshape(N, -1)
        if name == "fc_output":
            if deriv:
                return self._to_host(t.backprop_buffer.contents.output_layer_deriv, N * d["output"]).reshape(N, -1)
            return self._to_host(a.linear_output, N * d["output"]).reshape(N, -1)
        if name == "softmax":
            return self._to_host(t.forward_buffer.contents.pred, N * d["output"]).reshape(N, -1)
        if name.startswith("conv_blocks/"):
            _, idx, leaf = name.split("/")
            k = a.activation_conv_blocks[int(idx)].contents
            H, Ho, R, X = k.incoming_spatial_dim, k.incoming_spatial_dim // k.stride, k.reduced_depth, k.expanded_depth
            table = {"reduction_applied": ("post_reduced", R, H), "reduction_activated": ("post_reduced_activated", R, H),
                     "spatial_applied": ("post_spatial", R, Ho), "spatial_activated": ("post_spatial_activated", R, Ho),
                     "expanded_applied": ("post_expanded", X, Ho), "expanded_post_norm": ("post_expanded_norm_vals", X, Ho),
                     "transformed_residual": ("transformed_residual", X, Ho),
                     "post_projection_norm_vals": ("post_projection_norm_vals", X, Ho),
                     "combined_output": ("output", X, Ho), "output_activated": ("output_activated", X, Ho)}
            field, ch, hh = table[leaf]
            ptr = getattr(k, field)
            if not ptr:
                raise KeyError(name + " is not stored (fast path); enable full-store")
            return self._act_to_host(ptr, N * ch * hh * hh).reshape(N, ch, hh, hh)
        if name.startswith("batch_norms/"):
            parts = name.split("/")
            if parts[1] == "init":
                cache = a.norm_init_conv.contents
            else:
                k = a.activation_conv_blocks[int(parts[1])].contents
                cache = {"reduced": k.norm_post_reduced, "spatial": k.norm_post_spatial,
                         "expanded": k.norm_post_expanded, "projected": k.norm_post_projection}[parts[2]].contents
            return self._to_host(getattr(cache, parts[-1]), cache.feature_size)
        raise KeyError(name)
```

Baseline: 2452.

## Fold projection batch norm into expansion BN apply with deferred materialisation

For fp32 without full-store, the projection shortcut's batch-norm apply is no longer run as its own pass. Its statistics are still computed, but the normalisation of the raw projection output is fused into the expansion BN apply kernel, which normalises the residual on the fly before the add. This removes one full read and write of the projection activation per downsampling block. A gamma/beta snapshot is saved, and a materialise routine rebuilds the normalised projection tensor on demand for dumps and inspection, which adds bookkeeping and extra per-element sqrt and loads in the fused kernel.

```diff
diff --git a/include/resnet_mi.h b/include/resnet_mi.h
--- a/include/resnet_mi.h
+++ b/include/resnet_mi.h
@@ -264,6 +264,7 @@
 int mi_trainer_set_store_policy(Train_ResNet *t, int policy);
 size_t mi_trainer_activation_bytes(const Train_ResNet *t);
 size_t mi_trainer_device_bytes(const Train_ResNet *t);
+void mi_trainer_materialize_activations(Train_ResNet *t);
 void mi_clear_error(void);
 int mi_trainer_check_errors(Train_ResNet *t);
 int mi_trainer_stem_dtype(Train_ResNet *t);
@@ -308,6 +309,8 @@
                    void *y, int a_dt, int N, int C, int H, float eps, int relu);
 int mi_op_bn_apply_t(const void *x, int x_dt, const float *gamma, const float *beta, const void *residual, const float *means,
                      const float *vars, void *y, int a_dt, int N, int C, int H, float eps, int relu);
+int mi_op_bn_fwd_rbn(const float *x, const float *gamma, const float *beta, const float *r, const float *rgamma, const float *rbeta,
+                     const float *rmeans, const float *rvars, float *snap, float *means, float *vars, float *y, int N, int C, int H, float eps);
 int mi_op_bn_bwd_t(const void *x, int x_dt, const float *gamma, const float *beta, const float *means, const float *vars,
                    const void *dy, const void *mask_src, void *gated_out, int a_dt, void *dx, float *dgamma, float *dbeta, int N, int C,
                    int H, float eps, int mask_mode);
diff --git a/resnet_amd/binding.py b/resnet_amd/binding.py
--- a/resnet_amd/binding.py
+++ b/resnet_amd/binding.py
@@ -170,6 +170,7 @@
     "mi_trainer_set_store_policy": (_i, [_T, _i]),
     "mi_trainer_activation_bytes": (_sz, [_T]),
     "mi_trainer_device_bytes": (_sz, [_T]),
+    "mi_trainer_materialize_activations": (None, [_T]),
     "mi_clear_error": (None, []),
     "mi_trainer_check_errors": (_i, [_T]),
     "mi_trainer_end_epoch": (None, [_T, _f, _f, _f]),
@@ -203,6 +204,7 @@
     "mi_op_conv_bn_fwd_t": (_i, [_vp, _vp, _vp, _i, _vp, _vp, _vp, _vp, _vp, _i, _i, _i, _i, _i, _i, _f, _i]),
     "mi_op_bn_fwd_t": (_i, [_vp, _i, _vp, _vp, _vp, _vp, _vp, _vp, _i, _i, _i, _i, _f, _i]),
     "mi_op_bn_apply_t": (_i, [_vp, _i, _vp, _vp, _vp, _vp, _vp, _vp, _i, _i, _i, _i, _f, _i]),
+    "mi_op_bn_fwd_rbn": (_i, [_vp] * 12 + [_i, _i, _i, _f]),
     "mi_op_bn_bwd_t": (_i, [_vp, _i, _vp, _vp, _vp, _vp, _vp, _vp, _vp, _i, _vp, _vp, _vp, _i, _i, _i, _f, _i]),
     "mi_op_maxpool_fwd_t": (_i, [_vp, _vp, _i, _vp, _i, _i, _i, _i, _i]),
     "mi_op_maxpool_bwd_t": (_i, [_vp, _vp, _vp, _i, _i, _i, _i, _i, _i]),
diff --git a/resnet_amd/csrc/dump.c b/resnet_amd/csrc/dump.c
--- a/resnet_amd/csrc/dump.c
+++ b/resnet_amd/csrc/dump.c
@@ -151,6 +151,7 @@
 
 void dump_trainer(int dump_id, Train_ResNet *t, const char *special_dir) {
     if (!special_dir) special_dir = "default";
+    mi_trainer_materialize_activations(t);
     if (dump_parameters(dump_id, t, special_dir)) {
         fprintf(stderr, "resnet_mi: cannot write dump %d under %s/%s (skipped)\n", dump_id, root_of(t), special_dir);
         return;
diff --git a/resnet_amd/csrc/kernels_bn.hip b/resnet_amd/csrc/kernels_bn.hip
--- a/resnet_amd/csrc/kernels_bn.hip
+++ b/resnet_amd/csrc/kernels_bn.hip
@@ -152,13 +152,15 @@
 __device__ __forceinline__ float bn_xhat(float x, float mean, float sd) { return (x - mean) / sd; }
 __device__ __forceinline__ float bn_y(float xh, float g, float b) { return fmaf(g, xh, b); }
 
-template <typename TX, typename TA, int V, bool STR>
+template <typename TX, typename TA, int V, bool STR, bool RBN = false>
 __global__ void __launch_bounds__(256)
 bn_apply_kernel(const TX *__restrict__ x, const float *__restrict__ gamma, const float *__restrict__ beta,
                 const float *__restrict__ means, const float *__restrict__ vars, const TA *__restrict__ residual,
                 TA *__restrict__ y, float *__restrict__ xhat_out, float *__restrict__ norm_out, int C, int P,
-                FastDiv fdP, FastDiv fdC, size_t total, float eps, int relu) {
+                FastDiv fdP, FastDiv fdC, size_t total, float eps, int relu, const mid_bn_res rb) {
     const size_t nvec = total / V;
+    if (RBN && rb.snap && blockIdx.x == 0)
+        for (int c = threadIdx.x; c < C; c += blockDim.x) { rb.snap[c] = rb.gamma[c]; rb.snap[C + c] = rb.beta[c]; }
     for (size_t i = (size_t)blockIdx.x * blockDim.x + threadIdx.x; i < nvec; i += (size_t)gridDim.x * blockDim.x) {
         const size_t e = i * V;
         const uint32_t plane = fd_div((uint32_t)e, fdP);
@@ -174,6 +176,19 @@
         float v[V], r[V], xh[V], nv[V];
         VecIO<TX, V>::load(x + e, v);
         if (residual) VecIO<TA, V>::load(residual + e, r);
+        if (RBN) {
+            const float rm0 = rb.means[c], rs0 = sqrtf(rb.vars[c] + eps), rg0 = rb.gamma[c], rbb0 = rb.beta[c];
+            float rm1 = rm0, rs1 = rs0, rg1 = rg0, rbb1 = rbb0;
+            if (STR) {
+                const uint32_t c1 = c + 1 == (uint32_t)C ? 0u : c + 1;
+                rm1 = rb.means[c1]; rs1 = sqrtf(rb.vars[c1] + eps); rg1 = rb.gamma[c1]; rbb1 = rb.beta[c1];
+            }
+#pragma unroll
+            for (int q = 0; q < V; q++) {
+                const bool nx = STR && q >= nfirst;
+                r[q] = bn_y(bn_xhat(r[q], nx ? rm1 : rm0, nx ? rs1 : rs0), nx ? rg1 : rg0, nx ? rbb1 : rbb0);
+            }
+        }
 #pragma unroll
         for (int q = 0; q < V; q++) {
             const bool nx = STR && q >= nfirst;
@@ -528,7 +543,7 @@
 
 static int bn_fwd_apply(hipStream_t st, const void *x, int x_dt, const float *gamma, const float *beta, const void *residual,
                         const float *means, const float *vars, void *y, int a_dt, float *xhat_out, float *norm_out, int N, int C,
-                        int P, float eps, int relu, void *ycl, int Hcl) {
+                        int P, float eps, int relu, void *ycl, int Hcl, const mid_bn_res *rb = nullptr) {
     const int Hab = Hcl < 0 ? -Hcl : Hcl;
     if (ycl && x_dt == MID_BF16 && a_dt == MID_BF16 && (residual || relu) && !xhat_out && !norm_out && C % 64 == 0 && Hab * Hab == P && !(Hcl < 0 && (Hab & 1))) {
         hipLaunchKernelGGL(bn_apply_cl_kernel, dim3(C / 64, mi_cdiv(P, 64), N), dim3(256), 0, st, (const bf16_t *)x, gamma, beta, means, vars,
@@ -541,9 +556,23 @@
     const FastDiv fdP = make_fastdiv(P), fdC = make_fastdiv(C);
     bool str;
     const int vec = bn_vec_ew(x_dt, a_dt, P, total, &str);
+    const mid_bn_res rb0 = {nullptr, nullptr, nullptr, nullptr, nullptr};
+    if (rb) {
+        if (!(x_dt == MID_F32 && a_dt == MID_F32) || !residual || relu || xhat_out || norm_out) {
+            mi_record_error("bn_fwd_apply", "a normalised residual needs fp32 tensors, a residual and no full-store output");
+            return -2;
+        }
+#define APPLY_RBN(V, STR)                                                                                                       \
+    hipLaunchKernelGGL((bn_apply_kernel<float, float, V, STR, true>), dim3(ew_blocks(total / V)), dim3(256), 0, st, (const float *)x, \
+                       gamma, beta, means, vars, (const float *)residual, (float *)y, nullptr, nullptr, C, P, fdP, fdC, total, eps, 0, *rb)
+        if (str) { APPLY_RBN(4, true); } else if (vec == 4) { APPLY_RBN(4, false); } else { APPLY_RBN(1, false); }
+#undef APPLY_RBN
+        MI_LAUNCH_CHECK("bn_apply_kernel");
+        return 0;
+    }
 #define APPLY(TX, TA, V, STR)                                                                                              \
     hipLaunchKernelGGL((bn_apply_kernel<TX, TA, V, STR>), dim3(ew_blocks(total / V)), dim3(256), 0, st, (const TX *)x, gamma, beta, \
-                       means, vars, (const TA *)residual, (TA *)y, xhat_out, norm_out, C, P, fdP, fdC, total, eps, relu)
+                       means, vars, (const TA *)residual, (TA *)y, xhat_out, norm_out, C, P, fdP, fdC, total, eps, relu, rb0)
     BN_DISPATCH_EW(APPLY);
 #undef APPLY
     MI_LAUNCH_CHECK("bn_apply_kernel");
@@ -582,16 +611,17 @@
     return rc;
 }
 
-int mid_bn_fwd_t(mid_stream s, float *ws, const mid_bn_parts *parts, const void *x, int x_dt, const float *gamma, const float *beta,
-                 const void *residual, float *means, float *vars, void *y, int a_dt, float *xhat_out, float *norm_out, int N, int C,
-                 int P, float eps, int relu, void *ycl, int Hcl) {
+static int bn_fwd_impl(mid_stream s, float *ws, const mid_bn_parts *parts, const void *x, int x_dt, const float *gamma, const float *beta,
+                       const void *residual, const mid_bn_res *rb, float *means, float *vars, void *y, int a_dt, float *xhat_out,
+                       float *norm_out, int N, int C, int P, float eps, int relu, void *ycl, int Hcl) {
     if (!bn_pair_ok(x_dt, a_dt)) { mi_record_error("mid_bn_fwd_t", "unsupported storage types"); return -2; }
     if ((xhat_out || norm_out) && !(x_dt == MID_F32 && a_dt == MID_F32)) { mi_record_error("mid_bn_fwd_t", "full-store tensors exist in fp32 only"); return -2; }
+    if (!y && (xhat_out || norm_out || ycl || residual)) { mi_record_error("mid_bn_fwd_t", "outputs requested without y"); return -2; }
     hipStream_t st = (hipStream_t)s;
-    const double xb = (double)N * C * P * dt_bytes(x_dt), ab = (double)N * C * P * dt_bytes(a_dt);
+    const double xb = (double)N * C * P * dt_bytes(x_dt), ab = y ? (double)N * C * P * dt_bytes(a_dt) : 0.0;
     if (!parts || parts->nparts <= 0) {
         const int ns = bn_nsplit(N, C);
-        mi_prof_begin(st, MI_FAM_BN, 0.0, 2 * xb + ab * (residual ? 2 : 1));
+        mi_prof_begin(st, MI_FAM_BN, 0.0, (y ? 2 : 1) * xb + ab * (residual ? 2 : 1));
         if (bn_stats_launch(st, ws, x, x_dt, N, C, P, ns)) return -1;
         hipLaunchKernelGGL(bn_finalize_kernel, dim3(mi_cdiv(C, 4)), dim3(256), 0, st, ws, ns, C, means, vars);
         MI_LAUNCH_CHECK("bn_finalize_kernel");
@@ -599,7 +629,7 @@
         int G = parts->nparts / 64;
         if (G < 1) G = 1;
         if (G > BN_SPLIT_MAX) G = BN_SPLIT_MAX;
-        mi_prof_begin(st, MI_FAM_BN, 0.0, xb + ab * (residual ? 2 : 1));
+        mi_prof_begin(st, MI_FAM_BN, 0.0, (y ? xb : 0.0) + ab * (residual ? 2 : 1));
         hipLaunchKernelGGL(bn_parts_merge_kernel, dim3(mi_cdiv(C, 64), G), dim3(256), 0, st, parts->buf, parts->nparts, C, ws);
         MI_LAUNCH_CHECK("bn_parts_merge_kernel");
         hipLaunchKernelGGL(bn_finalize_kernel, dim3(mi_cdiv(C, 4)), dim3(256), 0, st, ws, G, C, means, vars);
@@ -616,9 +646,23 @@
         hipLaunchKernelGGL(bn_sync_k3, dim3(mi_cdiv(C, 256)), dim3(256), 0, st, tmp + C, vars, C, iw);
         MI_LAUNCH_CHECK("bn_sync");
     }
-    const int rc = bn_fwd_apply(st, x, x_dt, gamma, beta, residual, means, vars, y, a_dt, xhat_out, norm_out, N, C, P, eps, relu, ycl, Hcl);
+    const int rc = y ? bn_fwd_apply(st, x, x_dt, gamma, beta, residual, means, vars, y, a_dt, xhat_out, norm_out, N, C, P, eps, relu, ycl, Hcl, rb) : 0;
     mi_prof_end(st);
     return rc;
+}
+
+int mid_bn_fwd_t(mid_stream s, float *ws, const mid_bn_parts *parts, const void *x, int x_dt, const float *gamma, const float *beta,
+                 const void *residual, float *means, float *vars, void *y, int a_dt, float *xhat_out, float *norm_out, int N, int C,
+                 int P, float eps, int relu, void *ycl, int Hcl) {
+    return bn_fwd_impl(s, ws, parts, x, x_dt, gamma, beta, residual, nullptr, means, vars, y, a_dt, xhat_out, norm_out, N, C, P, eps,
+                       relu, ycl, Hcl);
+}
+
+int mid_bn_fwd_rbn_t(mid_stream s, float *ws, const mid_bn_parts *parts, const float *x, const float *gamma, const float *beta,
+                     const float *residual_raw, const mid_bn_res *rb, float *means, float *vars, float *y, int N, int C, int P, float eps) {
+    if (!rb || !residual_raw) { mi_record_error("mid_bn_fwd_rbn_t", "no residual batch norm"); return -2; }
+    return bn_fwd_impl(s, ws, parts, x, MID_F32, gamma, beta, residual_raw, rb, means, vars, y, MID_F32, nullptr, nullptr, N, C, P, eps,
+                       0, nullptr, 0);
 }
 
 int mid_bn_fwd(mid_stream s, float *ws, const float *x, const float *gamma, const float *beta, const float *residual,
diff --git a/resnet_amd/csrc/mi_device.h b/resnet_amd/csrc/mi_device.h
--- a/resnet_amd/csrc/mi_device.h
+++ b/resnet_amd/csrc/mi_device.h
@@ -162,6 +162,9 @@
                  float *norm_out, int N, int C, int P, float eps, int relu, void *ycl, int Hcl);
 void mid_bn_set_sync(void *comm, int world, float *tmp, size_t tmp_floats, int force);
 int mid_bn_debug_merge(mid_stream s, int R, int C, float *means, float *vars, float *dgamma, float *dbeta, float *sums_out, float *tmp);
+typedef struct { const float *gamma, *beta, *means, *vars; float *snap; } mid_bn_res;
+int mid_bn_fwd_rbn_t(mid_stream s, float *stats_ws, const mid_bn_parts *parts, const float *x, const float *gamma, const float *beta,
+                     const float *residual_raw, const mid_bn_res *rb, float *means, float *vars, float *y, int N, int C, int P, float eps);
 int mid_bn_stats_t(mid_stream s, float *stats_ws, const void *x, int x_dt, float *means, float *vars, int N, int C, int P);
 int mid_bn_apply_t(mid_stream s, const void *x, int x_dt, const float *gamma, const float *beta, const void *residual,
                    const float *means, const float *vars, void *y, int a_dt, int N, int C, int P, float eps, int relu, void *ycl, int Hcl);
diff --git a/resnet_amd/csrc/mi_host.h b/resnet_amd/csrc/mi_host.h
--- a/resnet_amd/csrc/mi_host.h
+++ b/resnet_amd/csrc/mi_host.h
@@ -62,6 +62,7 @@
     void *dye;
     void *par; size_t par_bytes; int par_valid;
     void *xp; size_t xp_bytes; float *scratch; size_t scratch_floats;
+    int bn_folded, bn_owed; float *bn_snap;
 } MiLayer;
 typedef struct { MiLayer red, spa, exp, proj; } MiBlockLayers;
 
diff --git a/resnet_amd/csrc/ops.c b/resnet_amd/csrc/ops.c
--- a/resnet_amd/csrc/ops.c
+++ b/resnet_amd/csrc/ops.c
@@ -281,6 +281,14 @@
                      const float *vars, void *y, int a_dt, int N, int C, int H, float eps, int relu) {
     return finish(mid_bn_apply_t(mi_global()->compute, x, x_dt, gamma, beta, residual, means, vars, y, a_dt, N, C, H * H, eps, relu, NULL, 0));
 }
+int mi_op_bn_fwd_rbn(const float *x, const float *gamma, const float *beta, const float *r, const float *rgamma, const float *rbeta,
+                     const float *rmeans, const float *rvars, float *snap, float *means, float *vars, float *y, int N, int C, int H, float eps) {
+    float *ws = (float *)mid_malloc(mid_bn_ws_floats(C) * sizeof(float));
+    const mid_bn_res rb = {rgamma, rbeta, rmeans, rvars, snap};
+    int rc = finish(mid_bn_fwd_rbn_t(mi_global()->compute, ws, NULL, x, gamma, beta, r, &rb, means, vars, y, N, C, H * H, eps));
+    mid_free(ws);
+    return rc;
+}
 int mi_op_maxpool_fwd_t(const void *x, void *y, int dt, int *max_inds, int N, int C, int H, int k, int stride) {
     return finish(mid_maxpool_fwd_t(mi_global()->compute, x, y, dt, max_inds, N, C, H, k, stride));
 }
diff --git a/resnet_amd/csrc/trainer.c b/resnet_amd/csrc/trainer.c
--- a/resnet_amd/csrc/trainer.c
+++ b/resnet_amd/csrc/trainer.c
@@ -379,6 +379,10 @@
             layer_init(&B->proj, b->projection, b->incoming_filters, H, b->expanded_depth, s == 2 ? 3 : 1, s);
             plan_conv(c, &B->proj, N, 0);
             if (B->proj.cl) B->proj.cl_by_bn = i > 0 && !(H & 1);
+            if (c->dtype == MID_F32 && c->policy != MI_STORE_FULL) {
+                B->proj.bn_folded = 1;
+                B->proj.bn_snap = falloc(c, (size_t)2 * B->proj.K);
+            }
         }
         MiLayer *Ls[4] = {&B->red, &B->spa, &B->exp, &B->proj};
         for (int j = 0; j < 4; j++) {
@@ -723,7 +727,7 @@
 
 static int conv_out_dt(const MiCtx *c, const MiLayer *L) { return L == &c->stem ? (c->stem_bf16 ? MID_BF16 : MID_F32) : c->dtype; }
 static void unit_fwd(Train_ResNet *t, MiLayer *L, const float *in, const BatchNorm *bn, Cache_BatchNorm *cache, float *conv_out,
-                     float *act_out, const float *residual, int relu, const MiLayer *cl_reader) {
+                     float *act_out, const float *residual, int relu, const MiLayer *cl_reader, const mid_bn_res *rb) {
     MiCtx *c = ctx_of(t);
     const int N = t->batch_size, C = L->C, H = L->H, K = L->K, Ho = H / L->stride;
     const int bf_ops = L->fwd == MI_FWD_BF16 || L->fwd == MI_FWD_CL || L->fwd == MI_FWD_STEM_BF16;
@@ -753,6 +757,12 @@
     c->ws.pre_fwd = NULL;
     void *ycl = cl_reader && cl_reader->cl_by_bn ? cl_reader->cl : NULL;
     const int Hcl = ycl ? (cl_reader->stride == 2 ? -cl_reader->H : cl_reader->H) : 0;
+    if (rb) {
+        if (ycl || relu || cache->normalized_temp || cache->normalized) { ck(-2, "batch norm forward with a normalised residual: unsupported form"); return; }
+        ck(mid_bn_fwd_rbn_t(G.compute, c->bn_ws, parts, conv_out, bn->gamma, bn->beta, residual, rb, cache->means, cache->vars, act_out,
+                            N, K, Ho * Ho, t->eps), "batch norm forward (+ projection batch norm, add, ReLU)");
+        return;
+    }
     ck(mid_bn_fwd_t(G.compute, c->bn_ws, parts, conv_out, conv_out_dt(c, L), bn->gamma, bn->beta, residual, cache->means, cache->vars,
                     act_out, c->dtype, cache->normalized_temp, cache->normalized, N, K, Ho * Ho, t->eps, relu, ycl, Hcl), "batch norm forward");
 }
@@ -772,7 +782,7 @@
     bind_sync_bn(c);
     relayout_weights(c);
     unit_fwd(t, &c->stem, t->cur_batch->images, p->norm_init_conv, a->norm_init_conv, a->init_conv_applied, a->init_conv_activated,
-             NULL, 1, NULL);
+             NULL, 1, NULL, NULL);
     const int Hs = d->input / d->init_conv_stride;
     ck(mid_maxpool_fwd_t(G.compute, a->init_conv_activated, a->init_convblock_input, c->dtype, a->max_inds, N, f, Hs, d->init_maxpool_dim,
                          d->init_maxpool_stride), "max-pool forward");
@@ -782,21 +792,30 @@
         MiBlockLayers *B = &c->blk[i];
         Activation_ConvBlock *k = a->activation_conv_blocks[i];
         const int Ho = b->incoming_spatial_dim / b->stride;
-        unit_fwd(t, &B->red, bin, b->norm_depth_reduction, k->norm_post_reduced, k->post_reduced, k->post_reduced_activated, NULL, 1, &B->spa);
+        unit_fwd(t, &B->red, bin, b->norm_depth_reduction, k->norm_post_reduced, k->post_reduced, k->post_reduced_activated, NULL, 1, &B->spa,
+                 NULL);
         unit_fwd(t, &B->spa, k->post_reduced_activated, b->norm_spatial, k->norm_post_spatial, k->post_spatial, k->post_spatial_activated,
-                 NULL, 1, NULL);
+                 NULL, 1, NULL, NULL);
         const float *res = bin;
+        mid_bn_res rb = {NULL, NULL, NULL, NULL, NULL};
+        const int fold = b->projection && B->proj.bn_folded;
         if (b->projection) {
-            unit_fwd(t, &B->proj, bin, b->norm_projection, k->norm_post_projection, k->transformed_residual, k->post_projection_norm_vals,
-                     NULL, 0, NULL);
+            unit_fwd(t, &B->proj, bin, b->norm_projection, k->norm_post_projection, k->transformed_residual,
+                     fold ? NULL : k->post_projection_norm_vals, NULL, 0, NULL, NULL);
             res = k->post_projection_norm_vals;
+            if (fold) {
+                rb = (mid_bn_res){b->norm_projection->gamma, b->norm_projection->beta, k->norm_post_projection->means,
+                                  k->norm_post_projection->vars, B->proj.bn_snap};
+                res = k->transformed_residual;
+                B->proj.bn_owed = c->policy == MI_STORE_FAST;
+            }
         }
         if (!c->full_store) {
             unit_fwd(t, &B->exp, k->post_spatial_activated, b->norm_expansion, k->norm_post_expanded, k->post_expanded, k->output_activated,
-                     res, 0, i + 1 < d->n_conv_blocks ? &c->blk[i + 1].proj : NULL);
+                     res, 0, i + 1 < d->n_conv_blocks ? &c->blk[i + 1].proj : NULL, fold ? &rb : NULL);
         } else {
             unit_fwd(t, &B->exp, k->post_spatial_activated, b->norm_expansion, k->norm_post_expanded, k->post_expanded,
-                     k->post_expanded_norm_vals, NULL, 0, NULL);
+                     k->post_expanded_norm_vals, NULL, 0, NULL, NULL);
             ck(mid_add_relu(G.compute, k->post_expanded_norm_vals, res, k->output, k->output_activated,
                             (size_t)N * b->expanded_depth * Ho * Ho), "add + ReLU");
         }
@@ -811,6 +830,24 @@
     mid_memcpy_d2h(t->forward_buffer->pred_cpu, t->forward_buffer->pred, (size_t)N * d->output * sizeof(float), G.compute);
     mid_stream_sync(G.compute);
     poll_nan_flag(t);
+}
+
+void mi_trainer_materialize_activations(Train_ResNet *t) {
+    MiCtx *c = ctx_of(t);
+    const Dims *d = t->model->dims;
+    const Params *p = t->model->params;
+    Activations *a = t->forward_buffer->activations;
+    if (!c->blk || !a) return;
+    for (int i = 0; i < d->n_conv_blocks; i++) {
+        MiLayer *L = &c->blk[i].proj;
+        if (!L->bn_owed) continue;
+        const Activation_ConvBlock *k = a->activation_conv_blocks[i];
+        const int Ho = p->conv_blocks[i]->incoming_spatial_dim / p->conv_blocks[i]->stride;
+        ck(mid_bn_apply_t(G.compute, k->transformed_residual, MID_F32, L->bn_snap, L->bn_snap + L->K, NULL, k->norm_post_projection->means,
+                          k->norm_post_projection->vars, k->post_projection_norm_vals, MID_F32, t->batch_size, L->K, Ho * Ho, t->eps, 0,
+                          NULL, 0), "projection batch norm (materialised)");
+        L->bn_owed = 0;
+    }
 }
 
 float mi_host_loss(Train_ResNet *t, int *n_wrong) {
diff --git a/resnet_amd/ops.py b/resnet_amd/ops.py
--- a/resnet_amd/ops.py
+++ b/resnet_amd/ops.py
@@ -346,6 +346,15 @@
                                           int(relu)), "bn_apply_t")
         return self.get_t(dy, a_dt)
 
+    def bn_fwd_rbn(self, x, gamma, beta, r, rgamma, rbeta, rmeans, rvars, eps):
+        N, Cc, H, _ = x.shape
+        dx, dg, db, dr = self.dev(x), self.dev(gamma), self.dev(beta), self.dev(r)
+        drg, drb, drm, drv = (self.dev(a) for a in (rgamma, rbeta, rmeans, rvars))
+        dm, dv, dy, ds = self.dev(shape=(Cc,)), self.dev(shape=(Cc,)), self.dev(shape=x.shape), self.dev(shape=(2, Cc))
+        self._chk(self.L.mi_op_bn_fwd_rbn(dx.ptr, dg.ptr, db.ptr, dr.ptr, drg.ptr, drb.ptr, drm.ptr, drv.ptr, ds.ptr, dm.ptr, dv.ptr, dy.ptr,
+                                          N, Cc, H, eps), "bn_fwd_rbn")
+        return dm.get(), dv.get(), dy.get(), ds.get()
+
     def bn_bwd_t(self, x, gamma, beta, means, vars_, dy, eps, mask_mode, x_dt, a_dt, mask_src=None):
         N, Cc, H, _ = x.shape
         dx, ddy = self.dev_t(x, x_dt), self.dev_t(dy, a_dt)
diff --git a/resnet_amd/trainer.py b/resnet_amd/trainer.py
--- a/resnet_amd/trainer.py
+++ b/resnet_amd/trainer.py
@@ -173,6 +173,8 @@
         return list(out)
 
     def activation(self, name, deriv=False):
+        if not deriv:
+            self.L.mi_trainer_materialize_activations(self.t)
         t = self.t.contents
         a = (t.backprop_buffer.contents.activation_derivs if deriv else t.forward_buffer.contents.activations).contents
         d, N = self.dims, self.batch
```

Result: no change. 2462, median of 6 (+0.4%).
